# Tikai7/DiTTO-TTS

Hardware: NVIDIA B200
Metric: latent frames/sec per denoising step (higher is better)
Workload: dtype bf16

## Files before the change

ditto_tts_b200/csrc/cross_fused.cu:

```cuda
#include <algorithm>
#include <cstdlib>

#include "common.cuh"
#include "kernels.cuh"

namespace ditto {
namespace {

constexpr int XF_THREADS = 640;
constexpr int XF_EPI_WARP0 = 4;
constexpr int XF_EPI_WARPS = 16;
constexpr int XF_SM_WARPS = 8;
constexpr int XF_REGS_LAUNCH = 96, XF_REGS_CTRL = 56, XF_REGS_EPI = 104;
static_assert(128 * XF_REGS_CTRL + 32 * XF_EPI_WARPS * XF_REGS_EPI <= XF_THREADS * XF_REGS_LAUNCH, "register re-distribution exceeds the CTA pool");
constexpr int XF_BM = 128;
constexpr int XF_BK = 64;
constexpr int XF_NS = 64;
constexpr int XF_CH = 128;
constexpr int XF_HC = 64;
constexpr int XF_STAGES = 2;
constexpr int XF_A_BYTES = XF_BM * XF_BK * 2;
constexpr int XF_B_BYTES = XF_NS * XF_BK * 2;
constexpr int XF_STAGE_BYTES = XF_A_BYTES + XF_B_BYTES;
constexpr int XF_MAX_H = 768;
constexpr int XF_P_BYTES = XF_BM * XF_NS * 2;
constexpr int XF_VF_BOX = XF_NS * 64 * 2;
constexpr int XF_VF_RING = 3;
constexpr int XF_VF_BYTES = XF_VF_RING * XF_VF_BOX;
constexpr int XF_NB = 4;
constexpr int XF_SLAB_BYTES = XF_BM * 32 * 4;
constexpr int XF_HBUF_BYTES = 2 * XF_SLAB_BYTES;
constexpr int XF_OFF_P = XF_STAGES * XF_STAGE_BYTES;
constexpr int XF_OFF_VF = XF_OFF_P + XF_P_BYTES;
constexpr int XF_OFF_HB = XF_OFF_VF + XF_VF_BYTES;
constexpr int XF_OFF_BAR = XF_OFF_HB + XF_NB * XF_HBUF_BYTES;
constexpr int XF_BAR_BYTES = 512;
constexpr int XF_OFF_STAT = XF_OFF_BAR + XF_BAR_BYTES;
constexpr int XF_STAT_BYTES = 2 * XF_BM * 4 * 8;
constexpr int XF_SMEM_BYTES = XF_OFF_STAT + XF_STAT_BYTES + 1024 ;
static_assert(XF_SMEM_BYTES <= 232448, "exceeds the 227 KiB shared memory of an sm_100 CTA");
static_assert(XF_OFF_P % 1024 == 0 && XF_OFF_VF % 1024 == 0 && XF_OFF_HB % 1024 == 0 && XF_STAGE_BYTES % 1024 == 0,
              "swizzled operands need 1024-B alignment");
constexpr int XF_TMEM_COLS = 512;
constexpr int XF_O_BUFS = 3;
constexpr int XF_S_COL0 = XF_O_BUFS * XF_CH;

struct XfDev {
  int n_seq, T, S, H;
  int rt;
  int m_tiles, num_tiles, num_kb, num_ch, num_hc;
  int pf_dist;
  float alpha2;
  const float* sbias; long long sb_seq;
  const float* out_bias;
  const float* gamma; const float* beta;
  float inv_h;
  const float2* ln_stat; int ln_parts; const float* ln_c;
};

__device__ __forceinline__ void epi_bar_sync() { asm volatile("bar.sync 1, %0;" ::"n"(32 * XF_EPI_WARPS) : "memory"); }
__device__ __forceinline__ void quarter_bar_sync(int quarter) { asm volatile("bar.sync %0, 128;" ::"r"(2 + quarter) : "memory"); }
__device__ __forceinline__ void xf_regs_ctrl() { asm volatile("setmaxnreg.dec.sync.aligned.u32 %0;" ::"n"(XF_REGS_CTRL)); }
__device__ __forceinline__ void xf_regs_epi() { asm volatile("setmaxnreg.inc.sync.aligned.u32 %0;" ::"n"(XF_REGS_EPI)); }
__device__ __forceinline__ void tmem_ld_16x16(uint32_t taddr, uint32_t (&r)[8]) {
  asm volatile("tcgen05.ld.sync.aligned.16x256b.x2.b32 {%0, %1, %2, %3, %4, %5, %6, %7}, [%8];"
               : "=r"(r[0]), "=r"(r[1]), "=r"(r[2]), "=r"(r[3]), "=r"(r[4]), "=r"(r[5]), "=r"(r[6]), "=r"(r[7])
               : "r"(taddr)
               : "memory");
}
__device__ __forceinline__ void tma_store_4d(const CUtensorMap* m, const void* smem, int c0, int c1, int c2, int c3) {
  asm volatile("cp.async.bulk.tensor.4d.global.shared::cta.bulk_group [%0, {%2, %3, %4, %5}], [%1];" ::"l"(reinterpret_cast<uint64_t>(m)),
               "r"(smem_u32(smem)), "r"(c0), "r"(c1), "r"(c2), "r"(c3)
               : "memory");
}
__device__ __forceinline__ void tma_prefetch_4d(const CUtensorMap* m, int c0, int c1, int c2, int c3) {
  asm volatile("cp.async.bulk.prefetch.tensor.4d.L2.global.tile [%0, {%1, %2, %3, %4}];" ::"l"(reinterpret_cast<uint64_t>(m)), "r"(c0),
               "r"(c1), "r"(c2), "r"(c3)
               : "memory");
}
__device__ __forceinline__ void bulk_commit() { asm volatile("cp.async.bulk.commit_group;" ::: "memory"); }
template <int N>
__device__ __forceinline__ void bulk_wait() { asm volatile("cp.async.bulk.wait_group %0;" ::"n"(N) : "memory"); }
template <int N>
__device__ __forceinline__ void bulk_wait_read() { asm volatile("cp.async.bulk.wait_group.read %0;" ::"n"(N) : "memory"); }

__global__ void __launch_bounds__(XF_THREADS, 1)
    cross_fused_kernel(const __grid_constant__ CUtensorMap tmap_u, const __grid_constant__ CUtensorMap tmap_kf,
                       const __grid_constant__ CUtensorMap tmap_vf, const __grid_constant__ CUtensorMap tmap_h,
                       const __grid_constant__ CUtensorMap tmap_uo, const XfDev p) {
  extern __shared__ uint8_t smem_raw[];
  const uint32_t raw_addr = smem_u32(smem_raw);
  uint8_t* smem = smem_raw + ((1024u - (raw_addr & 1023u)) & 1023u);
  uint8_t* p_smem = smem + XF_OFF_P;
  uint8_t* vf_smem = smem + XF_OFF_VF;
  uint8_t* hbuf = smem + XF_OFF_HB;
  uint64_t* full_bar = reinterpret_cast<uint64_t*>(smem + XF_OFF_BAR);
  uint64_t* empty_bar = full_bar + XF_STAGES;
  uint64_t* s_full = empty_bar + XF_STAGES;
  uint64_t* s_empty = s_full + 2;
  uint64_t* p_full = s_empty + 2;
  uint64_t* vf_full = p_full + 1;
  uint64_t* vf_empty = vf_full + XF_VF_RING;
  uint64_t* o_full = vf_empty + XF_VF_RING;
  uint64_t* o_empty = o_full + XF_O_BUFS;
  uint64_t* hin_full = o_empty + XF_O_BUFS;
  uint64_t* hout_full = hin_full + XF_NB;
  uint64_t* hfree = hout_full + XF_NB;
  uint32_t* tmem_ptr = reinterpret_cast<uint32_t*>(hfree + XF_NB);
  float2* stat = reinterpret_cast<float2*>(smem + XF_OFF_STAT);
  static_assert((2 * XF_STAGES + 2 + 2 + 1 + 2 * XF_VF_RING + 2 * XF_O_BUFS + 3 * XF_NB) * 8 + 4 <= XF_BAR_BYTES, "barrier block too small");

  const int warp = warp_id_uniform();
  const int lane = threadIdx.x & 31;

  if (warp == 0 && lane == 0) {
    tma_prefetch_desc(&tmap_u);
    tma_prefetch_desc(&tmap_kf);
    tma_prefetch_desc(&tmap_vf);
    tma_prefetch_desc(&tmap_h);
    tma_prefetch_desc(&tmap_uo);
  }
  if (warp == 1 && lane == 0) {
    for (int s = 0; s < XF_STAGES; ++s) {
      mbar_init(&full_bar[s], 1);
      mbar_init(&empty_bar[s], 1);
    }
    for (int s = 0; s < 2; ++s) {
      mbar_init(&s_full[s], 1);
      mbar_init(&s_empty[s], XF_SM_WARPS);
    }
    mbar_init(p_full, XF_SM_WARPS);
    for (int s = 0; s < XF_VF_RING; ++s) {
      mbar_init(&vf_full[s], 1);
      mbar_init(&vf_empty[s], 1);
    }
    for (int s = 0; s < XF_O_BUFS; ++s) {
      mbar_init(&o_full[s], 1);
      mbar_init(&o_empty[s], XF_EPI_WARPS);
    }
    for (int s = 0; s < XF_NB; ++s) {
      mbar_init(&hin_full[s], 1);
      mbar_init(&hout_full[s], XF_EPI_WARPS);
      mbar_init(&hfree[s], 1);
    }
    fence_barrier_init();
  }
  if (warp == 2) tmem_alloc<XF_TMEM_COLS>(tmem_ptr);
  tcgen05_fence_before();
  __syncthreads();
  tcgen05_fence_after();
  const uint32_t tmem_base = *tmem_ptr;
  const int first = blockIdx.x, step = gridDim.x;

  if (warp == 0) {
    xf_regs_ctrl();
    {
      const bool leader = elect_one();
      int stage = 0;
      uint32_t phase = 0;
      uint32_t vc = 0;
      const uint32_t stage_tx = static_cast<uint32_t>(p.rt) * (XF_BK * 2) + XF_B_BYTES;
      auto load_scores_operands = [&](int tile) {
        const int seq = tile / p.m_tiles, mb = tile - seq * p.m_tiles;
        for (int kb = 0; kb < p.num_kb; ++kb) {
          mbar_wait(&empty_bar[stage], phase ^ 1u);
          if (leader) {
            uint8_t* sa = smem + stage * XF_STAGE_BYTES;
            mbar_expect_tx(&full_bar[stage], stage_tx);
            tma_load_4d(&tmap_u, &full_bar[stage], sa, kb * XF_BK, mb * p.rt, 0, seq);
            tma_load_4d(&tmap_kf, &full_bar[stage], sa + XF_A_BYTES, kb * XF_BK, 0, 0, seq);
          }
          __syncwarp();
          if (++stage == XF_STAGES) { stage = 0; phase ^= 1u; }
        }
      };
      if (first < p.num_tiles) load_scores_operands(first);
      for (int tile = first; tile < p.num_tiles; tile += step) {
        const int seq = tile / p.m_tiles;
        for (int hc = 0; hc < p.num_hc; ++hc, ++vc) {
          const uint32_t vs = vc % XF_VF_RING;
          mbar_wait(&vf_empty[vs], ((vc / XF_VF_RING) & 1u) ^ 1u);
          if (leader) {
            mbar_expect_tx(&vf_full[vs], XF_VF_BOX);
            tma_load_4d(&tmap_vf, &vf_full[vs], vf_smem + vs * XF_VF_BOX, hc * XF_HC, 0, 0, seq);
          }
          __syncwarp();
        }
        if (tile + step < p.num_tiles) load_scores_operands(tile + step);
      }
    }
  } else if (warp == 1) {
    xf_regs_ctrl();
    {
      const bool leader = elect_one();
      constexpr uint32_t idesc_s = umma_idesc_bf16(XF_BM, XF_NS, false, false);
      constexpr uint32_t idesc_o = umma_idesc_bf16(XF_BM, XF_HC, false, true);
      const uint64_t ds0 = umma_smem_desc(smem_u32(smem), 16, 1024);
      const uint64_t dp0 = umma_smem_desc(smem_u32(p_smem), 16, 1024);
      const uint64_t dv0 = umma_smem_desc(smem_u32(vf_smem), XF_VF_BOX, 1024);
      int stage = 0;
      uint32_t phase = 0;
      auto issue_scores = [&](uint32_t j) {
        const uint32_t sb = j & 1u;
        mbar_wait(&s_empty[sb], ((j >> 1) & 1u) ^ 1u);
        tcgen05_fence_after();
        const uint32_t d_tmem = tmem_base + XF_S_COL0 + sb * XF_NS;
        for (int kb = 0; kb < p.num_kb; ++kb) {
          mbar_wait(&full_bar[stage], phase);
          tcgen05_fence_after();
          if (leader) {
            const uint64_t da = ds0 + static_cast<uint64_t>((stage * XF_STAGE_BYTES) >> 4);
#pragma unroll
            for (int k = 0; k < XF_BK / 16; ++k)
              umma_bf16(d_tmem, da + ((k * 32) >> 4), da + ((XF_A_BYTES + k * 32) >> 4), idesc_s, (kb | k) != 0 ? 1u : 0u);
            umma_commit(&empty_bar[stage]);
          }
          __syncwarp();
          if (++stage == XF_STAGES) { stage = 0; phase ^= 1u; }
        }
        if (leader) umma_commit(&s_full[sb]);
        __syncwarp();
      };
      uint32_t it = 0, oc = 0, vc = 0;
      if (first < p.num_tiles) issue_scores(0);
      for (int tile = first; tile < p.num_tiles; tile += step, ++it) {
        mbar_wait(p_full, it & 1u);
        for (int hc = 0; hc < p.num_hc; ++hc, ++vc) {
          const uint32_t ob = oc % XF_O_BUFS, vs = vc % XF_VF_RING;
          mbar_wait(&vf_full[vs], (vc / XF_VF_RING) & 1u);
          if ((hc & 1) == 0) mbar_wait(&o_empty[ob], ((oc / XF_O_BUFS) & 1u) ^ 1u);
          tcgen05_fence_after();
          if (leader) {
            const uint32_t d_tmem = tmem_base + ob * XF_CH + (hc & 1) * XF_HC;
            const uint64_t dv = dv0 + static_cast<uint64_t>((vs * XF_VF_BOX) >> 4);
#pragma unroll
            for (int k = 0; k < XF_NS / 16; ++k)
              umma_bf16(d_tmem, dp0 + ((k * 32) >> 4), dv + ((k * (16 * 128)) >> 4), idesc_o, k != 0 ? 1u : 0u);
            umma_commit(&vf_empty[vs]);
            if (hc & 1) umma_commit(&o_full[ob]);
          }
          __syncwarp();
          if (hc & 1) ++oc;
        }
        if (tile + step < p.num_tiles) issue_scores(it + 1);
      }
    }
  } else if (warp == 2 || warp == 3) {
    xf_regs_ctrl();
    {
      const bool leader = elect_one();
      const int my_tiles = first < p.num_tiles ? (p.num_tiles - 1 - first) / step + 1 : 0;
      const int jobs_per_tile = 2 * p.num_hc;
      const int J = my_tiles * jobs_per_tile;
      auto job_coords = [&](int j, int& seq, int& row, int& pass, int& hc) {
        const int ti = j / jobs_per_tile, r = j - ti * jobs_per_tile;
        const int tile = first + ti * step;
        seq = tile / p.m_tiles;
        row = (tile - seq * p.m_tiles) * p.rt;
        pass = r / p.num_hc;
        hc = r - pass * p.num_hc;
      };
      if (warp == 2) {
        const int P0 = my_tiles * p.num_hc;
        int pf_next = 0;
        auto prefetch_upto = [&](int limit) {
          if (p.pf_dist <= 0) return;
          limit = limit < P0 ? limit : P0;
          for (; pf_next < limit; ++pf_next) {
            const int ti = pf_next / p.num_hc, hc = pf_next - ti * p.num_hc;
            const int tile = first + ti * step, seq = tile / p.m_tiles, row = (tile - seq * p.m_tiles) * p.rt;
            if (leader && pf_next >= XF_NB) {
              tma_prefetch_4d(&tmap_h, hc * XF_HC, row, 0, seq);
              tma_prefetch_4d(&tmap_h, hc * XF_HC + 32, row, 0, seq);
            }
          }
        };
        for (int j = 0; j < J; ++j) {
          int seq, row, pass, hc;
          job_coords(j, seq, row, pass, hc);
          const int b = j % XF_NB;
          const int ti = j / jobs_per_tile;
          prefetch_upto(pass == 0 ? ti * p.num_hc + hc + p.pf_dist + 1 : (ti + 1) * p.num_hc + p.pf_dist + (hc + 1) / 2 + 1);
          mbar_wait(&hfree[b], ((j / XF_NB) & 1u) ^ 1u);
          if (leader) {
            uint8_t* buf = hbuf + b * XF_HBUF_BYTES;
            mbar_expect_tx(&hin_full[b], static_cast<uint32_t>(p.rt) * 256);
            tma_load_4d(&tmap_h, &hin_full[b], buf, hc * XF_HC, row, 0, seq);
            tma_load_4d(&tmap_h, &hin_full[b], buf + XF_SLAB_BYTES, hc * XF_HC + 32, row, 0, seq);
          }
          __syncwarp();
        }
      } else {
        for (int j = 0; j < J; ++j) {
          const int b = j % XF_NB;
          mbar_wait(&hout_full[b], (j / XF_NB) & 1u);
          int seq, row, pass, hc;
          job_coords(j, seq, row, pass, hc);
          if (leader) {
            const uint8_t* buf = hbuf + b * XF_HBUF_BYTES;
            if (pass == 0) {
              tma_store_4d(&tmap_h, buf, hc * XF_HC, row, 0, seq);
              tma_store_4d(&tmap_h, buf + XF_SLAB_BYTES, hc * XF_HC + 32, row, 0, seq);
            } else {
              tma_store_4d(&tmap_uo, buf, hc * XF_HC, row, 0, seq);
            }
            bulk_commit();
            const int jn = j - 1 + XF_NB;
            if (j >= 1 && jn < J) {
              bulk_wait_read<1>();
              if ((jn % jobs_per_tile) >= p.num_hc) {
                if (p.num_hc - XF_NB + 1 > 8) bulk_wait<8>();
                else bulk_wait<1>();
              }
              mbar_arrive(&hfree[(j - 1) % XF_NB]);
            }
          }
          __syncwarp();
        }
        if (leader) bulk_wait<0>();
        __syncwarp();
      }
    }
  } else if (warp >= XF_EPI_WARP0) {
    xf_regs_epi();
    const int ew = warp - XF_EPI_WARP0;
    const int quarter = warp & 3;
    const int sub = ew >> 2;
    const int g = lane >> 2, q = lane & 3, q2 = q * 2;
    const bool writer = q == 0;
    uint32_t it = 0, oc = 0, job = 0;
    for (int tile = first; tile < p.num_tiles; tile += step, ++it) {
      const int seq = tile / p.m_tiles;
      const uint32_t sb = it & 1u;
      if (sub < 2) {
        const int trow = quarter * 32 + sub * 16;
        const float* bias = p.sbias + seq * p.sb_seq;
        float2 bb[8];
#pragma unroll
        for (int kb = 0; kb < 8; ++kb) {
          const int c = kb * 8 + q2;
          bb[kb].x = c < p.S ? __ldg(bias + c) * 1.4426950408889634f : 0.f;
          bb[kb].y = c + 1 < p.S ? __ldg(bias + c + 1) * 1.4426950408889634f : 0.f;
        }
        float aA = p.alpha2, nA = 0.f, aB = p.alpha2, nB = 0.f;
        float2 cc[8];
#pragma unroll
        for (int kb = 0; kb < 8; ++kb) cc[kb] = make_float2(0.f, 0.f);
        if (p.ln_stat != nullptr) {
          const float* lnc = p.ln_c + seq * p.sb_seq;
#pragma unroll
          for (int kb = 0; kb < 8; ++kb) {
            const int c = kb * 8 + q2;
            cc[kb].x = c < p.S ? __ldg(lnc + c) : 0.f;
            cc[kb].y = c + 1 < p.S ? __ldg(lnc + c + 1) : 0.f;
          }
          const int mbt = tile - seq * p.m_tiles;
          const int lrA = mbt * p.rt + trow + g;
#pragma unroll
          for (int half = 0; half < 2; ++half) {
            const int lr = lrA + half * 8;
            float sm = 0.f, sq = 0.f;
            if (lr < p.T) {
              const float2* sp2 = p.ln_stat + (static_cast<long long>(seq) * p.T + lr) * p.ln_parts;
              for (int c = 0; c < p.ln_parts; ++c) {
                const float2 v = __ldg(sp2 + c);
                sm += v.x; sq += v.y;
              }
            }
            const float mean = sm * p.inv_h;
            const float rstd = rsqrtf(fmaxf(fmaf(-mean, mean, sq * p.inv_h), 0.f) + 1e-5f);
            if (half == 0) { aA = rstd * p.alpha2; nA = -mean * aA; }
            else { aB = rstd * p.alpha2; nB = -mean * aB; }
          }
        }
        mbar_wait(&s_full[sb], (it >> 1) & 1u);
        tcgen05_fence_after();
        uint32_t r[32];
        tmem_ld_16x64(tmem_base + (static_cast<uint32_t>(trow) << 16) + XF_S_COL0 + sb * XF_NS, r);
        tmem_ld_wait();
        tcgen05_fence_before();
        __syncwarp();
        if (lane == 0) mbar_arrive(&s_empty[sb]);
        float mA = -INFINITY, mB = -INFINITY;
#pragma unroll
// ... 213 lines not shown
  }
  return 0;
}

}

bool cross_fused_supported(int64_t T, int64_t S, int H, int heads) {
  return heads == 1 && S >= 1 && S <= XF_NS && H % XF_CH == 0 && H >= XF_NB * XF_HC && H <= XF_MAX_H && T >= 1;
}

int launch_cross_fused(const CrossFusedParams& q, cudaStream_t st) {
  DITTO_TRY(tc_gemm_init());
  DITTO_REQUIRE(cross_fused_supported(q.T, q.S, q.H, 1), DITTO_E_UNSUPPORTED, "cross_fused: unsupported shape");
  DITTO_REQUIRE(q.u && q.kfold && q.vfold && q.sbias && q.out_bias && q.h && q.gamma && q.beta && q.u_out, DITTO_E_BADARG,
                "cross_fused: null argument");
  DITTO_REQUIRE(q.n_seq >= 1 && q.Sp >= q.S && q.Sp % 8 == 0, DITTO_E_BADARG, "cross_fused: bad sizes");
  DeviceState* ds = device_state();
  if (ds == nullptr) return DITTO_E_CUDA;
  if (!ds->xf_attr) {
    DITTO_CUDA(cudaFuncSetAttribute(cross_fused_kernel, cudaFuncAttributeMaxDynamicSharedMemorySize, XF_SMEM_BYTES));
    ds->xf_attr = true;
  }
  TcOperand U, Kf, Vf, Uo;
  U.ptr = q.u; U.rows = q.T; U.cols = q.H; U.ld = q.H; U.s_outer = q.T * q.H;
  Kf.ptr = q.kfold; Kf.rows = q.S; Kf.cols = q.H; Kf.ld = q.H; Kf.s_outer = q.kf_seq;
  Vf.ptr = q.vfold; Vf.rows = q.Sp; Vf.cols = q.H; Vf.ld = q.H; Vf.s_outer = q.vf_seq;
  Uo.ptr = q.u_out; Uo.rows = q.T; Uo.cols = q.H; Uo.ld = q.H; Uo.s_outer = q.T * q.H;
  const int sms = tc_num_sms();
  int rt = XF_BM;
  if (g_opt.xf_rows >= 8 && g_opt.xf_rows <= XF_BM && g_opt.xf_rows % 8 == 0) rt = g_opt.xf_rows;
  CUtensorMap mu, mk, mv, mh, mo;
  DITTO_TRY(tc_make_map(&mu, U, 1, q.n_seq, XF_BK, rt));
  DITTO_TRY(tc_make_map(&mk, Kf, 1, q.n_seq, XF_BK, XF_NS));
  DITTO_TRY(tc_make_map(&mv, Vf, 1, q.n_seq, 64, XF_NS));
  DITTO_TRY(tc_make_map(&mo, Uo, 1, q.n_seq, XF_HC, rt));
  DITTO_TRY(make_map_h(&mh, q.h, q.n_seq, q.T, q.H, rt));
  XfDev p;
  p.n_seq = static_cast<int>(q.n_seq); p.T = static_cast<int>(q.T); p.S = static_cast<int>(q.S); p.H = q.H;
  p.rt = rt;
  p.m_tiles = static_cast<int>(ceil_div(q.T, rt));
  const int64_t tiles = static_cast<int64_t>(p.m_tiles) * q.n_seq;
  DITTO_REQUIRE(tiles < (1ll << 31), DITTO_E_UNSUPPORTED, "cross_fused: too many tiles");
  p.num_tiles = static_cast<int>(tiles);
  p.num_kb = q.H / XF_BK;
  p.num_ch = q.H / XF_CH;
  p.num_hc = q.H / XF_HC;
  p.alpha2 = q.alpha * 1.4426950408889634f;
  p.sbias = q.sbias; p.sb_seq = q.sb_seq;
  p.out_bias = q.out_bias;
  p.gamma = q.gamma; p.beta = q.beta;
  p.inv_h = 1.0f / static_cast<float>(q.H);
  p.pf_dist = g_opt.xf_prefetch > 0 ? std::min(g_opt.xf_prefetch, 2 * p.num_hc) : 0;
  p.ln_stat = q.ln_stat; p.ln_parts = q.ln_parts; p.ln_c = q.ln_c;
  if (q.ln_stat != nullptr) DITTO_REQUIRE(q.ln_parts > 0 && q.ln_c != nullptr, DITTO_E_BADARG, "cross_fused: deferred LayerNorm arguments");
  const double rows = static_cast<double>(q.n_seq) * q.T;
  ProfScope prof(q.tag, st, 4.0 * rows * q.S * q.H, rows * q.H * 12.0);
  const int grid = static_cast<int>(std::min<int64_t>(sms, tiles));
  cross_fused_kernel<<<grid, XF_THREADS, XF_SMEM_BYTES, st>>>(mu, mk, mv, mh, mo, p);
  DITTO_LAUNCH_CHECK();
  return 0;
}

}
```

ditto_tts_b200/csrc/elementwise.cu:

```cuda
#include <vector>

#include "kernels.cuh"

namespace ditto {

__global__ void cast_bf16_kernel(const float* __restrict__ x, bf16* __restrict__ y, int64_t n) {
  int64_t i = (static_cast<int64_t>(blockIdx.x) * blockDim.x + threadIdx.x) * 4;
  const int64_t stride = static_cast<int64_t>(gridDim.x) * blockDim.x * 4;
  for (; i + 3 < n; i += stride) {
    float4 v = *reinterpret_cast<const float4*>(x + i);
    uint2 o;
    o.x = pack_bf16x2(v.x, v.y);
    o.y = pack_bf16x2(v.z, v.w);
    *reinterpret_cast<uint2*>(y + i) = o;
  }
  if (i < n) {
    for (int64_t j = i; j < n && j < i + 4; ++j) y[j] = __float2bfloat16_rn(x[j]);
  }
}

int launch_cast_bf16(const float* x, bf16* y, int64_t n, cudaStream_t st) {
  if (n <= 0) return 0;
  DITTO_REQUIRE((reinterpret_cast<uintptr_t>(x) & 15) == 0 && (reinterpret_cast<uintptr_t>(y) & 7) == 0,
                DITTO_E_BADARG, "cast_bf16: misaligned pointer");
// ... 456 lines not shown
  return 0;
}

__global__ void silu_kernel(float* __restrict__ x, int64_t n) {
  for (int64_t i = static_cast<int64_t>(blockIdx.x) * blockDim.x + threadIdx.x; i < n;
       i += static_cast<int64_t>(gridDim.x) * blockDim.x) {
    const float v = x[i];
    x[i] = v / (1.0f + expf(-v));
  }
}
int launch_silu(float* x, int64_t n, cudaStream_t st) {
  silu_kernel<<<static_cast<unsigned>(std::min<int64_t>(ceil_div(n, 256), 148 * 8)), 256, 0, st>>>(x, n);
  DITTO_LAUNCH_CHECK();
  return 0;
}

__global__ void mean_silu_kernel(const float* __restrict__ text, float* __restrict__ out, int S, int D) {
  const int seq = blockIdx.y;
  const int c = blockIdx.x * blockDim.x + threadIdx.x;
  if (c >= D) return;
  const float* p = text + static_cast<int64_t>(seq) * S * D + c;
  float acc = 0.f;
  for (int s = 0; s < S; ++s) acc += p[static_cast<int64_t>(s) * D];
  const float m = acc / static_cast<float>(S);
  out[static_cast<int64_t>(seq) * D + c] = m / (1.0f + expf(-m));
}
int launch_mean_silu(const float* text, float* out, int64_t n, int S, int D, cudaStream_t st) {
  dim3 grid(static_cast<unsigned>(ceil_div(D, 128)), static_cast<unsigned>(n));
  mean_silu_kernel<<<grid, 128, 0, st>>>(text, out, S, D);
  DITTO_LAUNCH_CHECK();
  return 0;
}

__global__ void fold_bias_kernel(const bf16* __restrict__ kv, int64_t ld, const float* __restrict__ bq, float* __restrict__ sb,
                                 int64_t total, int S, int Sp, int heads, int d, float scale) {
  const int lane = threadIdx.x & 31;
  const int64_t o = static_cast<int64_t>(blockIdx.x) * (blockDim.x >> 5) + (threadIdx.x >> 5);
  if (o >= total) return;
  const int s_idx = static_cast<int>(o % Sp);
  const int head = static_cast<int>((o / Sp) % heads);
  const int64_t seq = o / (static_cast<int64_t>(Sp) * heads);
  float acc = 0.f;
  if (s_idx < S) {
    const bf16* row = kv + (seq * S + s_idx) * ld + head * d;
    for (int i = lane; i < d; i += 32) acc += __bfloat162float(row[i]) * bq[head * d + i];
  }
  acc = warp_sum(acc);
  if (lane == 0) sb[o] = s_idx < S ? scale * acc : 0.f;
}
int launch_fold_bias(const bf16* kv, int64_t ld, const float* bq, float* sb, int64_t n, int S, int Sp, int heads, int d, float scale,
                     cudaStream_t st) {
  const int64_t total = n * heads * Sp;
  fold_bias_kernel<<<static_cast<unsigned>(ceil_div(total, 8)), 256, 0, st>>>(kv, ld, bq, sb, total, S, Sp, heads, d, scale);
  DITTO_LAUNCH_CHECK();
  return 0;
}

__global__ void transpose_v_kernel(const bf16* __restrict__ v, int64_t ld, bf16* __restrict__ vt, int T, int Tp, int heads,
                                   int d) {
  __shared__ bf16 tile[32][33];
  const int b = blockIdx.z;
  const int seq = b / heads, head = b % heads;
  const bf16* src = v + (static_cast<int64_t>(seq) * T) * ld + head * d;
  bf16* dst = vt + static_cast<int64_t>(b) * d * Tp;
  const int t0 = blockIdx.x * 32, c0 = blockIdx.y * 32;
  for (int i = threadIdx.y; i < 32; i += blockDim.y) {
    const int tt = t0 + i, c = c0 + threadIdx.x;
    tile[i][threadIdx.x] = (tt < T && c < d) ? src[static_cast<int64_t>(tt) * ld + c] : __float2bfloat16(0.f);
  }
  __syncthreads();
  for (int i = threadIdx.y; i < 32; i += blockDim.y) {
    const int c = c0 + i, tt = t0 + threadIdx.x;
    if (c < d && tt < Tp) dst[static_cast<int64_t>(c) * Tp + tt] = tile[threadIdx.x][i];
  }
}
int launch_transpose_v(const bf16* v, int64_t ld, bf16* vt, int64_t n_seq, int T, int Tp, int heads, int d, cudaStream_t st) {
  dim3 grid(static_cast<unsigned>(ceil_div(Tp, 32)), static_cast<unsigned>(ceil_div(d, 32)), static_cast<unsigned>(n_seq * heads));
  transpose_v_kernel<<<grid, dim3(32, 8), 0, st>>>(v, ld, vt, T, Tp, heads, d);
  DITTO_LAUNCH_CHECK();
  return 0;
}

__device__ __forceinline__ float cfg_combine(float ec, float eu, float w) { return __fmaf_rn(w, __fsub_rn(ec, eu), eu); }
__device__ __forceinline__ float ddpm_update(float x, float e, float z, float c1, float c2, float c3) {
  return __fmaf_rn(c3, z, __fmul_rn(c1, __fmaf_rn(-c2, e, x)));
}

__global__ void __launch_bounds__(256)
    cfg_ddpm_update_kernel(const float4* __restrict__ eps_c, const float4* __restrict__ eps_u, const float4* __restrict__ x,
                           const float4* __restrict__ z, const int64_t* __restrict__ t, const float* __restrict__ coef,
                           int steps, float w, float4* __restrict__ out, int64_t vec_per_seq, int64_t total_vec) {
  for (int64_t i = static_cast<int64_t>(blockIdx.x) * blockDim.x + threadIdx.x; i < total_vec;
       i += static_cast<int64_t>(gridDim.x) * blockDim.x) {
    const int64_t seq = i / vec_per_seq;
    int64_t tt = t[seq];
    tt = tt < 0 ? 0 : (tt >= steps ? steps - 1 : tt);
    const float c1 = coef[tt * 3 + 0], c2 = coef[tt * 3 + 1], c3 = coef[tt * 3 + 2];
    float4 e = eps_c[i];
    if (eps_u != nullptr) {
      const float4 u = eps_u[i];
      e = make_float4(cfg_combine(e.x, u.x, w), cfg_combine(e.y, u.y, w), cfg_combine(e.z, u.z, w), cfg_combine(e.w, u.w, w));
    }
    const float4 xv = x[i];
    const float4 zv = z != nullptr ? z[i] : make_float4(0.f, 0.f, 0.f, 0.f);
    out[i] = make_float4(ddpm_update(xv.x, e.x, zv.x, c1, c2, c3), ddpm_update(xv.y, e.y, zv.y, c1, c2, c3),
                         ddpm_update(xv.z, e.z, zv.z, c1, c2, c3), ddpm_update(xv.w, e.w, zv.w, c1, c2, c3));
// ... 208 lines not shown
__global__ void __launch_bounds__(256)
    cfg_update_known_kernel(const float4* __restrict__ eps_c, const float4* __restrict__ eps_u, const float4* __restrict__ x,
                            const float4* __restrict__ z, unsigned long long* rng, int64_t* t, int64_t n_t,
                            const float* __restrict__ coef, const float* __restrict__ coef_known, int steps, float w,
                            float4* __restrict__ out, float4* __restrict__ hist, const float4* __restrict__ known,
                            const uint8_t* __restrict__ mask, int64_t vec_per_seq, int64_t vec_per_frame, int64_t total_vec,
                            int64_t vec_offset, int advance) {
  unsigned long long seed = 0ull, draw = 0ull;
  if (RNG) {
    seed = rng[0];
    draw = rng[1];
  }
  for (int64_t i = static_cast<int64_t>(blockIdx.x) * blockDim.x + threadIdx.x; i < total_vec;
       i += static_cast<int64_t>(gridDim.x) * blockDim.x) {
    const int64_t seq = i / vec_per_seq;
    if (mask[i / vec_per_frame] != 0) {
      int64_t tt = t[seq];
      tt = tt < 0 ? 0 : (tt >= steps ? steps - 1 : tt);
      const float a = coef_known[tt * 2 + 0], s = coef_known[tt * 2 + 1];
      const float4 pv = known[i];
      const float4 zv = RNG ? philox_normal4(seed, draw, static_cast<unsigned long long>(vec_offset + i)) : z[i];
      out[i] = make_float4(known_value(pv.x, zv.x, a, s), known_value(pv.y, zv.y, a, s), known_value(pv.z, zv.z, a, s),
                           known_value(pv.w, zv.w, a, s));
      continue;
    }
    if (MULTISTEP) {
      const MultistepRow c = multistep_row(coef, t, seq, steps);
      float4 e = eps_c[i];
      if (eps_u != nullptr) {
        const float4 u = eps_u[i];
        e = make_float4(cfg_combine(e.x, u.x, w), cfg_combine(e.y, u.y, w), cfg_combine(e.z, u.z, w), cfg_combine(e.w, u.w, w));
      }
      const float4 xv = x[i];
      float4 zv = RNG ? make_float4(0.f, 0.f, 0.f, 0.f) : z[i];
      const float4 h = multistep_hist(hist, i, c.c4);
      if (RNG) zv = philox_normal4(seed, draw, static_cast<unsigned long long>(vec_offset + i));
      multistep_store(c, xv, e, zv, h, out, hist, i);
    } else {
      int64_t tt = t[seq];
      tt = tt < 0 ? 0 : (tt >= steps ? steps - 1 : tt);
      const float c1 = coef[tt * 3 + 0], c2 = coef[tt * 3 + 1], c3 = coef[tt * 3 + 2];
      float4 e = eps_c[i];
      if (eps_u != nullptr) {
        const float4 u = eps_u[i];
        e = make_float4(cfg_combine(e.x, u.x, w), cfg_combine(e.y, u.y, w), cfg_combine(e.z, u.z, w), cfg_combine(e.w, u.w, w));
      }
      const float4 xv = x[i];
      const float4 zv = RNG ? philox_normal4(seed, draw, static_cast<unsigned long long>(vec_offset + i)) : z[i];
      out[i] = make_float4(ddpm_update(xv.x, e.x, zv.x, c1, c2, c3), ddpm_update(xv.y, e.y, zv.y, c1, c2, c3),
                           ddpm_update(xv.z, e.z, zv.z, c1, c2, c3), ddpm_update(xv.w, e.w, zv.w, c1, c2, c3));
    }
  }
  if (RNG && advance) last_block_advances(rng, t, n_t, draw);
}

static int64_t profiled_known_frames(const uint8_t* mask, int64_t n, cudaStream_t st) {
  cudaStreamCaptureStatus cs = cudaStreamCaptureStatusNone;
  if (!g_prof_enabled || cudaStreamIsCapturing(st, &cs) != cudaSuccess || cs != cudaStreamCaptureStatusNone) return 0;
  std::vector<uint8_t> h(static_cast<size_t>(n));
  if (cudaMemcpyAsync(h.data(), mask, static_cast<size_t>(n), cudaMemcpyDeviceToHost, st) != cudaSuccess ||
      cudaStreamSynchronize(st) != cudaSuccess)
    return 0;
  int64_t k = 0;
  for (uint8_t v : h) k += v != 0;
  return k;
}

int launch_cfg_update_known(const float* eps_c, const float* eps_u, const float* x, const float* z, unsigned long long* rng, int64_t* t,
                            int64_t n_t, const float* coef, const float* coef_known, int steps, float w, float* out, float* hist,
                            const float* known, const uint8_t* mask, int64_t B, int64_t T, int64_t H, int64_t elem_offset, bool advance,
                            cudaStream_t st) {
  DITTO_REQUIRE(H % 4 == 0 && elem_offset % 4 == 0, DITTO_E_UNSUPPORTED, "cfg_update_known: H % 4 and element offset % 4");
  const bool draw = rng != nullptr, ms = hist != nullptr;
  const int64_t vec_per_frame = H / 4, total_vec = B * T * vec_per_frame;
  if (total_vec == 0) return (draw && advance) ? launch_step_advance(rng, t, n_t, st) : 0;
  const int64_t want = ceil_div(total_vec, 256 * 4);
  const unsigned blocks = static_cast<unsigned>(std::min<int64_t>(round_up(want, 148), 148 * 32));
  const int64_t known_vec = profiled_known_frames(mask, B * T, st) * vec_per_frame;
  const double unknown_streams = (ms ? 5 : 3) + (eps_u ? 1 : 0) + (draw ? 0 : 1), known_streams = 2 + (draw ? 0 : 1);
  ProfScope prof(PC_CFG_UPDATE, st, 0.0,
                 16.0 * (static_cast<double>(total_vec - known_vec) * unknown_streams + static_cast<double>(known_vec) * known_streams) +
                     static_cast<double>(B * T));
  const float4 *ec = reinterpret_cast<const float4*>(eps_c), *eu = reinterpret_cast<const float4*>(eps_u);
  const float4 *xv = reinterpret_cast<const float4*>(x), *zv = reinterpret_cast<const float4*>(z);
  const float4* kv = reinterpret_cast<const float4*>(known);
  float4 *o = reinterpret_cast<float4*>(out), *h = reinterpret_cast<float4*>(hist);
  const int64_t vps = T * vec_per_frame, voff = elem_offset / 4;
  const int adv = advance ? 1 : 0;
  if (ms && draw)
    cfg_update_known_kernel<true, true><<<blocks, 256, 0, st>>>(ec, eu, xv, zv, rng, t, n_t, coef, coef_known, steps, w, o, h, kv, mask,
                                                                vps, vec_per_frame, total_vec, voff, adv);
  else if (ms)
    cfg_update_known_kernel<true, false><<<blocks, 256, 0, st>>>(ec, eu, xv, zv, rng, t, n_t, coef, coef_known, steps, w, o, h, kv, mask,
                                                                 vps, vec_per_frame, total_vec, voff, adv);
  else if (draw)
    cfg_update_known_kernel<false, true><<<blocks, 256, 0, st>>>(ec, eu, xv, zv, rng, t, n_t, coef, coef_known, steps, w, o, h, kv, mask,
                                                                 vps, vec_per_frame, total_vec, voff, adv);
  else
    cfg_update_known_kernel<false, false><<<blocks, 256, 0, st>>>(ec, eu, xv, zv, rng, t, n_t, coef, coef_known, steps, w, o, h, kv,
                                                                  mask, vps, vec_per_frame, total_vec, voff, adv);
  DITTO_LAUNCH_CHECK();
  return 0;
}

__global__ void step_advance_kernel(unsigned long long* rng, int64_t* t, int64_t n_t) {
  for (int64_t i = threadIdx.x; i < n_t; i += blockDim.x) t[i] -= 1;
// ... 94 lines not shown
```

ditto_tts_b200/csrc/engine.cu:

```cuda
#include <cmath>
#include <cstdio>
#include <cstdlib>
#include <cstring>
#include <map>
#include <mutex>
#include <vector>

#include "kernels.cuh"

namespace ditto {

static thread_local std::string t_last_error;
std::atomic<long long> g_launches{0};
DebugOptions g_opt;
void set_error(const std::string& msg) { t_last_error = msg; }
int cuda_fail(cudaError_t err, const char* what, const char* file, int line) {
  t_last_error = std::string("CUDA error ") + std::to_string(static_cast<int>(err)) + " (" + cudaGetErrorString(err) + ") at " +
                 what + " [" + file + ":" + std::to_string(line) + "]";
  return DITTO_E_CUDA;
}

bool g_prof_enabled = false;
namespace {
struct ProfRec { int cls; cudaEvent_t a, b; double flops, bytes; };
// ... 13 lines not shown
  if (cudaEventCreate(&r.a) != cudaSuccess || cudaEventCreate(&r.b) != cudaSuccess) return;
  cudaEventRecord(r.a, st);
  g_prof_recs.push_back(r);
  slot = static_cast<int>(g_prof_recs.size()) - 1;
}
ProfScope::~ProfScope() {
  if (slot >= 0) cudaEventRecord(g_prof_recs[slot].b, st);
}

struct Arena {
  char* base;
  size_t off = 0;
  explicit Arena(void* b) : base(static_cast<char*>(b)) {}
  template <typename T>
  T* take(int64_t n) {
    off = (off + 255) & ~static_cast<size_t>(255);
    T* p = base ? reinterpret_cast<T*>(base + off) : nullptr;
    off += static_cast<size_t>(n) * sizeof(T);
    return p;
  }
};

struct LayerPack {
  bf16 *w_qkv = nullptr, *wc_in = nullptr, *wc_o = nullptr, *w_glu = nullptr, *w_fc2 = nullptr;
  bf16* wc_o_p4 = nullptr;
  float *b_qkv = nullptr, *b_glu = nullptr;
  float *c_qkv = nullptr, *c_glu = nullptr, *bq_g = nullptr;
  bf16* wq_g = nullptr;
};

}

using namespace ditto;

struct ditto_engine {
  ditto_config_t cfg;
  int H = 0, L = 0, heads = 0, d = 0, half = 0, Td = 0, Xd = 0, steps = 0, maxT = 0;
  bool bf16_mode = false, fused_rope = false, finalized = false, have_schedule = false;
  bool blocks_only = false;
  int device = -1;
  int rope_pd = 0;
  bool glu_perm16 = false;
  bool pv_perm4 = false;
  bool qkv_perm16 = false;
  bool cross_flash = false;
  bool fc2_ln = false;
  bool flash768 = false;
  bool flash_attn = true;
  bool defer_ln2 = false;
  bool fused_cross = true;
  bool fused_attn = false;
  bool fold_cross = false;
  bool defer_ln = false;
  int pv_transpose = 0;
  bool rope_table_in_epilogue = false;
  std::map<std::string, int64_t> expected;
  std::map<std::string, float*> w;
  std::vector<void*> owned;
  float *time_table = nullptr, *rope_cos = nullptr, *rope_sin = nullptr, *rope_freq = nullptr, *coef = nullptr, *qs_buf = nullptr;
  float* coef_ms = nullptr;
  float* coef_known = nullptr;
  bf16 *w_in16 = nullptr, *w_out16 = nullptr;
  bf16* w_out_p4 = nullptr;
  std::vector<LayerPack> layers;
  static constexpr int kSide = 8;
  cudaStream_t side[kSide] = {};
  cudaEvent_t ev_fork = nullptr, ev_join[kSide] = {};
  int n_side = 0;
  std::recursive_mutex fork_mutex;

  const float* W(const std::string& k) const {
    auto it = w.find(k);
    return it == w.end() ? nullptr : it->second;
  }
  const float* LW(int i, const char* name) const { return W("blocks." + std::to_string(i) + "." + name); }
};

namespace ditto {

static int dev_alloc(ditto_engine* e, void** p, size_t bytes) {
  DITTO_CUDA(cudaMalloc(p, bytes ? bytes : 16));
  e->owned.push_back(*p);
  return 0;
}

static void build_expected(ditto_engine* e) {
  const int64_t H = e->H, Td = e->Td, Xd = e->Xd, St = e->steps;
  auto& m = e->expected;
  if (!e->blocks_only) {
    m["t_embedding.weight"] = St * Td;
    m["time_embed.0.weight"] = Td * Td; m["time_embed.0.bias"] = Td;
    m["time_embed.2.weight"] = Td * Td; m["time_embed.2.bias"] = Td;
    m["ada_ln.time_mlp.1.weight"] = 2 * H * Td; m["ada_ln.time_mlp.1.bias"] = 2 * H;
    m["ada_ln.text_mlp.1.weight"] = 2 * H * Xd; m["ada_ln.text_mlp.1.bias"] = 2 * H;
    m["proj_in.weight"] = H * H; m["proj_in.bias"] = H;
    m["proj_out.weight"] = H * H; m["proj_out.bias"] = H;
  }
  for (int i = 0; i < e->L; ++i) {
    const std::string p = "blocks." + std::to_string(i) + ".";
    for (const char* n : {"norm1", "norm2", "norm3"}) { m[p + n + ".weight"] = H; m[p + n + ".bias"] = H; }
    m[p + "attn.in_proj_weight"] = 3 * H * H; m[p + "attn.in_proj_bias"] = 3 * H;
    m[p + "cross_attn.in_proj_weight"] = 3 * H * H; m[p + "cross_attn.in_proj_bias"] = 3 * H;
    m[p + "cross_attn.out_proj.weight"] = H * H; m[p + "cross_attn.out_proj.bias"] = H;
    m[p + "mlp_fc1.weight"] = 4 * H * H; m[p + "mlp_fc1.bias"] = 4 * H;
    m[p + "gate.weight"] = 4 * H * H; m[p + "gate.bias"] = 4 * H;
    m[p + "mlp_fc2.weight"] = 4 * H * H; m[p + "mlp_fc2.bias"] = H;
  }
  m["rotary.inv_freq"] = e->half;
}

static bool ignorable_key(const std::string& k) {
  if (k.rfind("nac.", 0) == 0) return true;
  if (k == "alphas_cumprod") return true;
  if (k.size() > 9 && k.compare(k.size() - 9, 9, ".inv_freq") == 0 && k != "rotary.inv_freq") return true;
  if (k.find(".attn.out_proj.") != std::string::npos) return true;
  return false;
}

static int sgemm_nt(const float* A, int64_t lda, const float* Wt, int64_t ldw, float* C, int64_t ldc, const float* bias,
                    const float* resid, int64_t ldr, float alpha, int M, int N, int K, cudaStream_t st) {
  SgemmParams p;
  p.A = A; p.lda = lda; p.B = Wt; p.ldb = ldw; p.C = C; p.ldc = ldc; p.bias = bias; p.resid = resid; p.ldr = ldr;
  p.alpha = alpha; p.M = M; p.N = N; p.K = K; p.b_is_nk = true;
  return launch_sgemm(p, st);
}

static int tc_nt(const bf16* A, int64_t lda, const bf16* Wt, int64_t ldw, void* out, bool out_bf16, int64_t ldo,
                 const float* bias, const float* resid, int64_t ldr, int64_t resid_row_mod, bf16* out2, int64_t ldo2,
                 int M, int N, int K, cudaStream_t st, int tag = PC_TC_OTHER, float2* stat_out = nullptr, int stat_parts = 0) {
  TcGemmParams p;
  p.tag = tag;
  p.stat_out = stat_out; p.stat_parts = stat_parts;
  p.A.ptr = A; p.A.rows = M; p.A.cols = K; p.A.ld = lda;
  p.B.ptr = Wt; p.B.rows = N; p.B.cols = K; p.B.ld = ldw;
  p.M = M; p.N = N; p.K = K;
  p.bias = bias; p.out = out; p.out_bf16 = out_bf16; p.ldo = ldo;
  p.resid = resid; p.ldr = ldr; p.resid_row_mod = resid_row_mod; p.out2 = out2; p.ldo2 = ldo2;
  return launch_tc_gemm(p, st);
}

struct CtxLayout {
  float* text_mod = nullptr;
  void* kv0 = nullptr;
  size_t kv_stride = 0;
  bf16 *kfold0 = nullptr, *vfold0 = nullptr;
  float *sbias0 = nullptr, *cvec0 = nullptr;
  size_t kfold_stride = 0, vfold_stride = 0, sbias_stride = 0;
  size_t total = 0;
};
static bool fold_active(const ditto_engine* e, int64_t S) {
  return e->bf16_mode && e->fold_cross && e->heads * round_up(S, 8) * 2 <= e->H;
}
static bool fold_ln_active(const ditto_engine* e, int64_t S) {
  const bool want = e->defer_ln || (e->defer_ln2 && cross_fused_supported(1, S, e->H, e->heads));
  return want && fold_active(e, S) && tc_scores_softmax_csize(static_cast<int>(S)) == 1;
}
static bool cross_flash_active(const ditto_engine* e, int64_t S) {
  return e->cross_flash && e->fused_cross && e->heads == 1 && S <= 256 && fold_active(e, S) && !cross_fused_supported(1, S, e->H, e->heads);
}
static CtxLayout ctx_layout(const ditto_engine* e, void* base, int64_t n, int64_t S) {
  Arena a(base);
  CtxLayout c;
  c.text_mod = a.take<float>(n * 2 * e->H);
  const int64_t kv_elems = n * S * 2 * e->H;
  a.take<char>(0);
  const size_t kv_bytes = ((static_cast<size_t>(kv_elems) * (e->bf16_mode ? 2 : 4)) + 255) & ~static_cast<size_t>(255);
  c.kv0 = a.take<char>(static_cast<int64_t>(kv_bytes) * e->L);
  c.kv_stride = kv_bytes;
  if (fold_active(e, S)) {
    const int64_t Sp = round_up(S, 8);
    c.kfold_stride = static_cast<size_t>(n * e->heads * S * e->H);
    c.vfold_stride = static_cast<size_t>(n * e->heads * Sp * e->H);
    c.sbias_stride = static_cast<size_t>(n * e->heads * Sp);
    c.kfold0 = a.take<bf16>(static_cast<int64_t>(c.kfold_stride) * e->L);
    c.vfold0 = a.take<bf16>(static_cast<int64_t>(c.vfold_stride) * e->L);
    c.sbias0 = a.take<float>(static_cast<int64_t>(c.sbias_stride) * e->L);
    if (e->defer_ln || e->defer_ln2) c.cvec0 = a.take<float>(static_cast<int64_t>(c.sbias_stride) * e->L);
  }
  c.total = a.off + 256;
  return c;
}

struct SeqGroup {
  int64_t n = 0, n_x = 0, T = 0, S = 0;
  const void* ctx = nullptr;
  int64_t row0 = 0;
  int64_t xrow0 = 0;
  int64_t seq0 = 0;
  int64_t p_off = 0;
  int64_t l_off = 0;
  int64_t vt_off = 0;
};

struct Workspace {
  float *h = nullptr, *xskip = nullptr, *scores = nullptr;
  void *u = nullptr, *qkv = nullptr, *P = nullptr, *qc = nullptr, *oc = nullptr, *hid = nullptr, *xb16 = nullptr;
  float *fc1 = nullptr, *gate = nullptr;
  bf16* vt = nullptr;
  float* lpart = nullptr;
  float2* lnstat = nullptr;
  int ln_parts_h = 0, ln_parts_attn = 0;
  float* tmp_small = nullptr;
  bf16* text16 = nullptr;
  int* row_pos = nullptr;
  int64_t M = 0;
  size_t total = 0;
};
static Workspace ws_layout(const ditto_engine* e, void* base, SeqGroup* gs, int ng) {
  Arena a(base);
  Workspace w;
  const int64_t H = e->H;
  const int es = e->bf16_mode ? 2 : 4;
  int64_t M = 0, Mx = 0, seqs = 0, p_el = 0, l_el = 0, vt_el = 0, n_tot = 0, text_el = 0;
  for (int i = 0; i < ng; ++i) {
    SeqGroup& g = gs[i];
    const int64_t ldp = std::max(round_up(g.T, 8), round_up(g.S, 8));
    g.row0 = M; g.xrow0 = Mx; g.seq0 = seqs; g.p_off = p_el; g.l_off = l_el; g.vt_off = vt_el;
    M += g.n * g.T; Mx += g.n_x * g.T; seqs += g.n;
    p_el += round_up(g.n * e->heads * g.T * ldp, 128);
    l_el += round_up(g.n * e->heads * g.T * ceil_div(ldp, 256), 64);
    vt_el += round_up(g.n * e->heads * e->d * ldp, 128);
    n_tot = std::max(n_tot, g.n);
    text_el = std::max(text_el, g.n * g.S);
  }
  w.M = M;
  w.h = a.take<float>(M * H);
  w.xskip = a.take<float>(M * H);
  w.u = a.take<char>(M * H * es);
  w.xb16 = a.take<char>(M * H * 2);
  w.qkv = a.take<char>(M * 3 * H * es);
// ... 193 lines not shown
  if (block_only) {
  } else if (b16) {
    const int Mp = static_cast<int>(ragged ? M : g0.n_x * g0.T);
    DITTO_TRY(tc_nt(static_cast<bf16*>(w.xb16), H, e->w_in16, H, w.xskip, false, H, e->W("proj_in.bias"), nullptr, 0, 0, nullptr, 0, Mp, H,
                    H, st, PC_TC_PROJ_IN));
  } else {
    for (int gi = 0; gi < ng; ++gi)
      DITTO_TRY(sgemm_nt(x + gs[gi].xrow0 * H, H, e->W("proj_in.weight"), H, w.xskip + gs[gi].xrow0 * H, H, e->W("proj_in.bias"), nullptr, 0,
                         1.f, static_cast<int>(gs[gi].n_x * gs[gi].T), H, H, st));
  }

  const bool fuse_cross_any = b16 && e->fused_cross && !dln;
  auto fuse_cross_group = [&](const SeqGroup& g) {
    return fuse_cross_any && fold_active(e, g.S) && cross_fused_supported(g.T, g.S, H, e->heads);
  };
  for (int i = l_begin; i < l_end; ++i) {
    const LayerPack& lp = e->layers[i];
    const bool last = (i == l_end - 1);
    if (b16) {
      bf16* u = static_cast<bf16*>(w.u);
      bf16* qkv = static_cast<bf16*>(w.qkv);
      if (do_self) {
        TcGemmParams g;
        g.A.ptr = u; g.A.rows = M; g.A.cols = H; g.A.ld = H;
        g.B.ptr = lp.w_qkv; g.B.rows = 3 * H; g.B.cols = H; g.B.ld = H;
        g.M = static_cast<int>(M); g.N = 3 * H; g.K = H; g.bias = lp.b_qkv; g.out = qkv; g.out_bf16 = true; g.ldo = 3 * H;
        g.tag = PC_TC_QKV;
        if (e->fused_rope) {
          g.epilogue = TC_EPI_QKV_ROPE; g.rope_cos = e->rope_cos; g.rope_sin = e->rope_sin; g.rope_half = e->half;
          g.rope_freq = e->rope_table_in_epilogue ? nullptr : e->rope_freq;
          g.rope_pd = e->rope_pd; g.seq_T = static_cast<int>(g0.T); g.hidden = H;
          g.rope_pos = ragged ? w.row_pos : nullptr;
          g.rope_perm16 = e->qkv_perm16;
        }
        if (dln) { g.ln_stat = w.lnstat; g.ln_parts = ln1_parts; g.ln_width = H; g.ln_c = lp.c_qkv; }
        DITTO_TRY(launch_tc_gemm(g, st));
        if (!e->fused_rope)
          for (int gi = 0; gi < ng; ++gi)
            DITTO_TRY(launch_rope(qkv + gs[gi].row0 * 3 * H, true, 3 * H, e->rope_cos, e->rope_sin, gs[gi].n * gs[gi].T,
                                  static_cast<int>(gs[gi].T), H, d, st));
      }
      DITTO_TRY(fork.begin(ng));
      for (int gi = 0; gi < ng; ++gi) {
        const SeqGroup& grp = gs[gi];
        const Workspace wg = group_view(e, w, grp);
        const CtxLayout c = ctx_layout(e, const_cast<void*>(grp.ctx), grp.n, grp.S);
        const int64_t n = grp.n, T = grp.T, S = grp.S, Mg = n * T;
        cudaStream_t st = fork.stream(gi);
        bf16* q = qkv + grp.row0 * 3 * H;
        bf16* ug = u + grp.row0 * H;
        float* hg = w.h + grp.row0 * H;
        const bool dln2 = dln ? dln2_all : fold_ln_active(e, S) && do_self;
        float2* lnstat_g = w.lnstat ? w.lnstat + grp.row0 * std::max(w.ln_parts_h, w.ln_parts_attn) : nullptr;
        if (!do_self) {
        } else if (e->flash768 && !dln2 && flash768_supported(H, e->heads, static_cast<int>(T))) {
          Flash768Params f;
          f.qkv = q; f.ld = 3 * H; f.n_seq = n; f.T = static_cast<int>(T); f.H = H; f.alpha = inv_sqrt_d; f.h = hg;
          f.gamma = e->LW(i, "norm2.weight"); f.beta = e->LW(i, "norm2.bias"); f.u_out = ug; f.tag = PC_FLASH768;
          DITTO_TRY(launch_flash768(f, st));
        } else {
          DITTO_TRY(attention_bf16(e, wg, q, 3 * H, T * 3 * H, q + H, 3 * H, T * 3 * H, q + 2 * H, 3 * H, T * 3 * H, n, static_cast<int>(T),
                                   static_cast<int>(T), inv_sqrt_d, hg, false, H, T * H, hg, st, false, dln2 ? ug : nullptr,
                                   dln2 ? lnstat_g : nullptr));
          if (!dln2) DITTO_TRY(launch_layernorm(hg, e->LW(i, "norm2.weight"), e->LW(i, "norm2.bias"), ug, true, Mg, H, st));
        }
        if (!do_cross) continue;
        void* kv = static_cast<char*>(c.kv0) + c.kv_stride * i;
        bool norm3_done = false;
        if (fold_active(e, S)) {
          const int heads = e->heads;
          const int64_t Sp = round_up(S, 8);
          if (!dln && cross_flash_active(e, S)) {
            Flash768Params f;
            f.qkv = ug; f.ld = H; f.n_seq = n; f.T = static_cast<int>(T); f.H = H; f.alpha = sqrt_inv_d; f.h = hg;
            f.kfold = c.kfold0 + c.kfold_stride * i; f.kf_seq = S * H; f.vfold = c.vfold0 + c.vfold_stride * i; f.vf_seq = Sp * H;
            f.vf_rows = static_cast<int>(Sp); f.Tk = static_cast<int>(S); f.kbias = c.sbias0 + c.sbias_stride * i; f.kb_seq = Sp;
            f.out_bias = e->LW(i, "cross_attn.out_proj.bias");
            f.gamma = e->LW(i, "norm3.weight"); f.beta = e->LW(i, "norm3.bias"); f.u_out = ug; f.tag = PC_CROSS_FLASH;
            DITTO_TRY(launch_flash768_quad(f, st));
            continue;
          }
          if (fuse_cross_group(grp)) {
            CrossFusedParams f;
            f.u = ug; f.kfold = c.kfold0 + c.kfold_stride * i; f.kf_seq = S * H; f.vfold = c.vfold0 + c.vfold_stride * i; f.vf_seq = Sp * H;
            f.sbias = c.sbias0 + c.sbias_stride * i; f.sb_seq = Sp; f.out_bias = e->LW(i, "cross_attn.out_proj.bias");
            f.h = hg; f.gamma = e->LW(i, "norm3.weight"); f.beta = e->LW(i, "norm3.bias"); f.u_out = ug;
            f.n_seq = n; f.T = T; f.S = S; f.Sp = Sp; f.H = H; f.alpha = sqrt_inv_d; f.tag = PC_TC_CROSS_FUSED;
            if (dln2) { f.ln_stat = lnstat_g; f.ln_parts = w.ln_parts_attn; f.ln_c = c.cvec0 + c.sbias_stride * i; }
            DITTO_TRY(launch_cross_fused(f, st));
            continue;
          }
          if (e->fused_attn && tc_scores_softmax_csize(static_cast<int>(S)) == 1) {
            TcScoresSoftmaxParams f;
            f.Q.ptr = ug; f.Q.rows = T; f.Q.cols = H; f.Q.ld = H; f.Q.s_inner = 0; f.Q.s_outer = T * H;
            f.Km.ptr = c.kfold0 + c.kfold_stride * i; f.Km.rows = S; f.Km.cols = H; f.Km.ld = H; f.Km.s_inner = S * H;
            f.Km.s_outer = static_cast<int64_t>(heads) * S * H;
            f.M = static_cast<int>(T); f.N = static_cast<int>(S); f.K = H; f.batch_inner = heads; f.batch_outer = static_cast<int>(n);
            f.alpha = sqrt_inv_d; f.bias = c.sbias0 + c.sbias_stride * i; f.sb_inner = Sp; f.sb_outer = heads * Sp;
            f.P = static_cast<bf16*>(wg.P); f.ldp = heads * Sp; f.sp_inner = Sp; f.sp_outer = T * heads * Sp; f.npad = static_cast<int>(Sp);
            f.tag = PC_TC_CROSS_SCORES;
            if (dln2) { f.ln_stat = lnstat_g; f.ln_parts = w.ln_parts_attn; f.ln_width = H; f.ln_c = c.cvec0 + c.sbias_stride * i; }
            DITTO_TRY(launch_tc_scores_softmax(f, st));
          } else {
            DITTO_REQUIRE(!dln2, DITTO_E_UNSUPPORTED, "forward: deferred LayerNorm needs the fused scores kernel on the folded cross path");
            TcGemmParams g;
            g.A.ptr = ug; g.A.rows = T; g.A.cols = H; g.A.ld = H; g.A.s_inner = 0; g.A.s_outer = T * H;
            g.B.ptr = c.kfold0 + c.kfold_stride * i; g.B.rows = S; g.B.cols = H; g.B.ld = H; g.B.s_inner = S * H;
            g.B.s_outer = static_cast<int64_t>(heads) * S * H;
            g.M = static_cast<int>(T); g.N = static_cast<int>(S); g.K = H; g.batch_inner = heads; g.batch_outer = static_cast<int>(n);
            g.alpha = sqrt_inv_d; g.bias = c.sbias0 + c.sbias_stride * i; g.sb_inner = Sp; g.sb_outer = heads * Sp;
            g.out = wg.scores; g.out_bf16 = false; g.ldo = heads * Sp; g.so_inner = Sp; g.so_outer = T * heads * Sp;
            g.tag = PC_TC_CROSS_SCORES;
            DITTO_TRY(launch_tc_gemm(g, st));
            DITTO_TRY(launch_softmax(wg.scores, Sp, wg.P, true, Sp, n * T * heads, static_cast<int>(S), st));
          }
          TcGemmParams o;
          o.A.ptr = static_cast<const bf16*>(wg.P); o.A.rows = T; o.A.cols = heads * Sp; o.A.ld = heads * Sp; o.A.s_outer = T * heads * Sp;
          o.B.ptr = c.vfold0 + c.vfold_stride * i; o.B.rows = heads * Sp; o.B.cols = H; o.B.ld = H; o.B.s_outer = heads * Sp * H;
          o.b_kn = true;
          o.M = static_cast<int>(T); o.N = H; o.K = static_cast<int>(heads * Sp); o.batch_inner = 1; o.batch_outer = static_cast<int>(n);
          o.bias = e->LW(i, "cross_attn.out_proj.bias");
          o.out = hg; o.out_bf16 = false; o.ldo = H; o.so_outer = T * H; o.resid = hg; o.ldr = H; o.sr_outer = T * H;
          o.tag = PC_TC_CROSS_PV;
          if (dln) { o.out2 = u; o.ldo2 = H; o.stat_out = w.lnstat; o.stat_parts = w.ln_parts_h; o.stat_rows_outer = T; }
          DITTO_TRY(launch_tc_gemm(o, st));
        } else {
          bf16* qc = static_cast<bf16*>(w.qc) + grp.row0 * H;
          bf16* oc = static_cast<bf16*>(w.oc) + grp.row0 * H;
          DITTO_TRY(tc_nt(ug, H, lp.wc_in, H, qc, true, H, e->LW(i, "cross_attn.in_proj_bias"), nullptr, 0, 0, nullptr, 0, static_cast<int>(Mg),
                          H, H, st, PC_TC_CROSS_Q));
          const bf16* kc = static_cast<const bf16*>(kv);
          DITTO_TRY(attention_bf16(e, wg, qc, H, T * H, kc, 2 * H, S * 2 * H, kc + H, 2 * H, S * 2 * H, n, static_cast<int>(T),
                                   static_cast<int>(S), sqrt_inv_d, oc, true, H, T * H, nullptr, st, true));
          if (e->fc2_ln && !dln) {
            GemmResidLnParams f;
            f.A = oc; f.lda = H; f.W = lp.wc_o_p4; f.ldw = H; f.bias = e->LW(i, "cross_attn.out_proj.bias"); f.h = hg; f.ldh = H;
            f.gamma = e->LW(i, "norm3.weight"); f.beta = e->LW(i, "norm3.bias"); f.u = ug; f.ldu = H;
            f.M = static_cast<int>(Mg); f.N = H; f.K = H; f.tag = PC_TC_CROSS_OUT;
            DITTO_TRY(launch_gemm_resid_ln(f, st));
            norm3_done = true;
          } else {
// ... 146 lines not shown
int32_t ditto_profile_get(int32_t i, int64_t* launches, double* total_ms, double* flops, double* bytes) {
  DITTO_REQUIRE(i >= 0 && i < PC_COUNT && launches && total_ms && flops && bytes, DITTO_E_BADARG, "profile_get: bad argument");
  *launches = g_prof_acc[i].launches; *total_ms = g_prof_acc[i].ms; *flops = g_prof_acc[i].flops; *bytes = g_prof_acc[i].bytes;
  return 0;
}

int32_t ditto_debug_set_counters(uint64_t* counters) {
  tc_gemm_set_debug_counters(reinterpret_cast<unsigned long long*>(counters));
  return 0;
}

int32_t ditto_engine_create(const ditto_config_t* cfg, ditto_engine_t** out) {
  DITTO_REQUIRE(cfg && out, DITTO_E_BADARG, "engine_create: null argument");
  DITTO_REQUIRE(cfg->hidden_dim > 0 && cfg->num_layers > 0 && cfg->num_heads > 0 && cfg->time_dim > 0 && cfg->diffusion_steps > 0,
                DITTO_E_BADARG, "engine_create: non-positive dimension");
  DITTO_REQUIRE(cfg->hidden_dim % cfg->num_heads == 0 && (cfg->hidden_dim / cfg->num_heads) % 2 == 0, DITTO_E_BADARG,
                "engine_create: hidden_dim must split into heads of even size");
  DITTO_REQUIRE(cfg->text_dim == cfg->hidden_dim, DITTO_E_UNSUPPORTED,
                "engine_create: text_dim must equal hidden_dim (nn.MultiheadAttention without kdim, DiT.py:90-91)");
  DITTO_REQUIRE(cfg->hidden_dim % 8 == 0 && cfg->hidden_dim <= 1024 && cfg->time_dim % 4 == 0, DITTO_E_UNSUPPORTED,
                "engine_create: need hidden_dim % 8 == 0, hidden_dim <= 1024, time_dim % 4 == 0");
  DITTO_REQUIRE(cfg->precision == DITTO_PREC_FP32 || cfg->precision == DITTO_PREC_BF16, DITTO_E_BADARG, "engine_create: precision");
  int ndev = 0;
  DITTO_CUDA(cudaGetDeviceCount(&ndev));
  DITTO_REQUIRE(ndev > 0, DITTO_E_CUDA, "engine_create: no CUDA device (there is no CPU fallback)");
  ditto_engine* e = new ditto_engine();
  e->cfg = *cfg;
  e->H = cfg->hidden_dim; e->L = cfg->num_layers; e->heads = cfg->num_heads; e->d = e->H / e->heads; e->half = e->d / 2;
  e->Td = cfg->time_dim; e->Xd = cfg->text_dim; e->steps = cfg->diffusion_steps;
  e->maxT = cfg->max_seq_len > 0 ? cfg->max_seq_len : 4096;
  e->bf16_mode = cfg->precision == DITTO_PREC_BF16;
  e->blocks_only = (cfg->flags & DITTO_F_BLOCKS_ONLY) != 0;
  if (cudaGetDevice(&e->device) != cudaSuccess) e->device = -1;
  if (e->bf16_mode) {
    if (e->bf16_mode && e->d % 8 != 0) {
      delete e;
      set_error("engine_create: bf16 path needs head_dim % 8 == 0 (16-byte TMA rows)");
      return DITTO_E_UNSUPPORTED;
    }
    int rc = tc_gemm_init();
    if (rc != 0) { delete e; return rc; }
    for (int pd : {128, 64, 32})
      if (e->half % pd == 0 && e->H % (2 * pd) == 0) { e->rope_pd = pd; break; }
    e->fused_rope = (cfg->flags & DITTO_F_FUSED_ROPE) && e->rope_pd != 0;
    e->fold_cross = (cfg->flags & DITTO_F_FOLD_CROSS) != 0;
    e->fused_attn = (cfg->flags & DITTO_F_FUSED_ATTN) != 0;
    e->defer_ln = (cfg->flags & DITTO_F_DEFER_LN) != 0 && e->fused_rope && e->fused_attn;
    if (g_opt.no_defer_ln) e->defer_ln = false;
    if (g_opt.no_fused_attn) e->fused_attn = false;
    e->fused_cross = e->fused_attn;
    e->flash_attn = e->fused_attn;
    if (g_opt.no_flash) e->flash_attn = false;
    if (g_opt.no_fused_cross) e->fused_cross = false;
    e->defer_ln2 = !e->defer_ln && e->fused_cross && e->bf16_mode && e->heads == 1 && g_opt.defer_ln2 != 0;
    e->pv_transpose = g_opt.pv_transpose != 0;
    e->rope_table_in_epilogue = g_opt.rope_table != 0;
    e->glu_perm16 = !e->defer_ln && e->H % 32 == 0 && !g_opt.glu_generic;
    const bool pd_ok = e->rope_pd == 128 || (e->rope_pd == 32 && !g_opt.no_rope_fast32);
    e->qkv_perm16 = e->fused_rope && pd_ok && !e->defer_ln && !e->rope_table_in_epilogue && e->H % 256 == 0 && !g_opt.rope_generic;
    e->pv_perm4 = e->qkv_perm16 && !e->pv_transpose && !e->defer_ln2 && e->d % 128 == 0 && !g_opt.no_pv_perm4;
    e->flash768 = e->fused_attn && e->pv_perm4 && !e->defer_ln && flash768_supported(e->H, e->heads, 1) && !g_opt.no_flash768;
    e->fc2_ln = !e->defer_ln && gemm_resid_ln_supported(e->H, 4 * e->H) && !g_opt.no_fc2_ln && gemm_resid_ln_schedulable(e->H);
    e->cross_flash = e->flash768 && e->fc2_ln && e->fold_cross && !e->defer_ln2 && !g_opt.no_cross_flash && flash768_quad_schedulable();
  }
  build_expected(e);
  e->layers.resize(e->L);
  int want_side = ditto_engine::kSide;
  if (g_opt.side_streams >= 0) want_side = std::min(ditto_engine::kSide, g_opt.side_streams);
  if (want_side > 0 && cudaEventCreateWithFlags(&e->ev_fork, cudaEventDisableTiming) == cudaSuccess) {
    for (int k = 0; k < want_side; ++k) {
      if (cudaStreamCreateWithFlags(&e->side[k], cudaStreamNonBlocking) != cudaSuccess ||
          cudaEventCreateWithFlags(&e->ev_join[k], cudaEventDisableTiming) != cudaSuccess)
        break;
      e->n_side = k + 1;
    }
  }
  *out = e;
  return 0;
}

int32_t ditto_engine_destroy(ditto_engine_t* e) {
  if (!e) return 0;
  for (int k = 0; k < ditto_engine::kSide; ++k) {
    if (e->side[k]) cudaStreamDestroy(e->side[k]);
    if (e->ev_join[k]) cudaEventDestroy(e->ev_join[k]);
  }
  if (e->ev_fork) cudaEventDestroy(e->ev_fork);
  for (auto& kv : e->w) cudaFree(kv.second);
  for (void* p : e->owned) cudaFree(p);
  delete e;
  return 0;
}

int32_t ditto_engine_load_weight(ditto_engine_t* e, const char* key, const float* data, int64_t numel, void* stream) {
  DITTO_REQUIRE(e && key && data, DITTO_E_BADARG, "load_weight: null argument");
  const std::string k(key);
  if (ignorable_key(k)) return 0;
  auto it = e->expected.find(k);
  if (it == e->expected.end()) {
    set_error("load_weight: unknown state_dict key '" + k + "'");
    return DITTO_E_BADARG;
  }
  if (it->second != numel) {
    set_error("load_weight: '" + k + "' has " + std::to_string(numel) + " elements, expected " + std::to_string(it->second));
    return DITTO_E_BADARG;
  }
// ... 222 lines not shown

int32_t ditto_text_context(ditto_engine_t* e, const float* text_emb, int64_t n, int64_t S, void* ctx, void* workspace,
                           int64_t workspace_bytes, void* stream) {
  DITTO_REQUIRE(e && text_emb && ctx && workspace, DITTO_E_BADARG, "text_context: null argument");
  DITTO_REQUIRE(e->finalized, DITTO_E_STATE, "text_context: engine not finalized");
  DITTO_REQUIRE(n > 0 && S > 0, DITTO_E_BADARG, "text_context: empty input");
  cudaStream_t st = static_cast<cudaStream_t>(stream);
  const int H = e->H, Xd = e->Xd;
  Workspace w = ws_layout(e, workspace, n, 1, S);
  DITTO_REQUIRE(static_cast<int64_t>(w.total) <= workspace_bytes, DITTO_E_WORKSPACE, "text_context: workspace too small");
  CtxLayout c = ctx_layout(e, ctx, n, S);
  if (!e->blocks_only) {
    DITTO_TRY(launch_mean_silu(text_emb, w.tmp_small, n, static_cast<int>(S), Xd, st));
    DITTO_TRY(sgemm_nt(w.tmp_small, Xd, e->W("ada_ln.text_mlp.1.weight"), Xd, c.text_mod, 2 * H, e->W("ada_ln.text_mlp.1.bias"), nullptr,
                       0, 1.f, static_cast<int>(n), 2 * H, Xd, st));
  }
  if (e->bf16_mode) DITTO_TRY(launch_cast_bf16(text_emb, w.text16, n * S * Xd, st));
  for (int i = 0; i < e->L; ++i) {
    void* kv = static_cast<char*>(c.kv0) + c.kv_stride * i;
    const float* bias = e->LW(i, "cross_attn.in_proj_bias") + H;
    if (e->bf16_mode) {
      DITTO_TRY(tc_nt(w.text16, Xd, e->layers[i].wc_in + static_cast<int64_t>(H) * H, H, kv, true, 2 * H, bias, nullptr, 0, 0, nullptr, 0,
                      static_cast<int>(n * S), 2 * H, Xd, st, PC_TC_TEXT_KV));
      if (fold_active(e, S)) {
        const int d = e->d, heads = e->heads;
        const int64_t Sp = round_up(S, 8);
        const bf16* kvb = static_cast<const bf16*>(kv);
        bf16* kf = c.kfold0 + c.kfold_stride * i;
        bf16* vf = c.vfold0 + c.vfold_stride * i;
        float* sb = c.sbias0 + c.sbias_stride * i;
        DITTO_CUDA(cudaMemsetAsync(vf, 0, c.vfold_stride * sizeof(bf16), st));
        TcGemmParams g;
        g.A.ptr = kvb; g.A.rows = S; g.A.cols = d; g.A.ld = 2 * H; g.A.s_inner = d; g.A.s_outer = S * 2 * H;
        const bool fln = fold_ln_active(e, S);
        g.B.ptr = fln ? e->layers[i].wq_g : e->layers[i].wc_in;
        g.B.rows = d; g.B.cols = H; g.B.ld = H; g.B.s_inner = static_cast<int64_t>(d) * H; g.B.s_outer = 0;
        g.b_kn = true;
        g.M = static_cast<int>(S); g.N = H; g.K = d; g.batch_inner = heads; g.batch_outer = static_cast<int>(n);
        g.out = kf; g.out_bf16 = true; g.ldo = H; g.so_inner = S * H; g.so_outer = static_cast<int64_t>(heads) * S * H;
        g.tag = PC_TC_TEXT_KV;
        DITTO_TRY(launch_tc_gemm(g, st));
        TcGemmParams v;
        v.A.ptr = kvb + H; v.A.rows = S; v.A.cols = d; v.A.ld = 2 * H; v.A.s_inner = d; v.A.s_outer = S * 2 * H;
        v.B.ptr = cross_flash_active(e, S) ? e->layers[i].wc_o_p4 : e->layers[i].wc_o;
        v.B.rows = H; v.B.cols = d; v.B.ld = H; v.B.s_inner = d; v.B.s_outer = 0;
        v.M = static_cast<int>(S); v.N = H; v.K = d; v.batch_inner = heads; v.batch_outer = static_cast<int>(n);
        v.out = vf; v.out_bf16 = true; v.ldo = H; v.so_inner = Sp * H; v.so_outer = static_cast<int64_t>(heads) * Sp * H;
        v.tag = PC_TC_TEXT_KV;
        DITTO_TRY(launch_tc_gemm(v, st));
        DITTO_TRY(launch_fold_bias(kvb, 2 * H, fln ? e->layers[i].bq_g : e->LW(i, "cross_attn.in_proj_bias"), sb, n,
                                   static_cast<int>(S), static_cast<int>(Sp), heads, d, sqrtf(1.0f / static_cast<float>(d)), st));
        if (fln)
          DITTO_TRY(launch_rowsum_bf16(kf, c.cvec0 + c.sbias_stride * i, n * heads, static_cast<int>(S), static_cast<int>(Sp), H, st));
      }
    } else {
      DITTO_TRY(sgemm_nt(text_emb, Xd, e->LW(i, "cross_attn.in_proj_weight") + static_cast<int64_t>(H) * H, H, static_cast<float*>(kv),
                         2 * H, bias, nullptr, 0, 1.f, static_cast<int>(n * S), 2 * H, Xd, st));
    }
  }
  return 0;
}

int32_t ditto_forward(ditto_engine_t* e, const float* x, int64_t n_x, const void* ctx, const int64_t* t, int64_t n_seq, int64_t T,
                      int64_t S, float* out, void* workspace, int64_t workspace_bytes, void* stream) {
  DITTO_REQUIRE(e && x && ctx && t && out && workspace, DITTO_E_BADARG, "forward: null argument");
  DITTO_REQUIRE(e->finalized && !e->blocks_only, DITTO_E_STATE, "forward: engine not finalized (or a blocks-only engine)");
  DITTO_REQUIRE(n_seq > 0 && T > 0 && S > 0 && n_x > 0 && n_seq % n_x == 0, DITTO_E_BADARG, "forward: bad batch sizes");
  DITTO_REQUIRE(T <= e->maxT, DITTO_E_UNSUPPORTED, "forward: T exceeds max_seq_len of the engine");
  return forward_impl(e, x, n_x, ctx, t, n_seq, T, S, out, workspace, workspace_bytes, static_cast<cudaStream_t>(stream));
}

int32_t ditto_cfg_ddpm_update(ditto_engine_t* e, const float* eps_c, const float* eps_u, const float* x, const float* z,
                              const int64_t* t, float guidance_scale, float* x_out, int64_t B, int64_t elems_per_seq, void* stream) {
  DITTO_REQUIRE(e && eps_c && x && t && x_out, DITTO_E_BADARG, "cfg_ddpm_update: null argument");
  DITTO_REQUIRE(e->have_schedule, DITTO_E_STATE, "cfg_ddpm_update: schedule not loaded");
  DITTO_REQUIRE(B >= 0 && elems_per_seq >= 0, DITTO_E_BADARG, "cfg_ddpm_update: negative size");
  return launch_cfg_ddpm_update(eps_c, eps_u, x, z, t, e->coef, e->steps, guidance_scale, x_out, B, elems_per_seq,
                                static_cast<cudaStream_t>(stream));
}

static int launch_update(const ditto_engine* e, const float* eps_c, const float* eps_u, const float* x, const float* z, const int64_t* t,
                         float w, float* x_out, float* hist, int64_t B, int64_t per, cudaStream_t st) {
  if (hist) return launch_cfg_multistep_update(eps_c, eps_u, x, z, t, e->coef_ms, e->steps, w, x_out, hist, B, per, st);
  return launch_cfg_ddpm_update(eps_c, eps_u, x, z, t, e->coef, e->steps, w, x_out, B, per, st);
}
static int launch_update_rng(const ditto_engine* e, const float* eps_c, const float* eps_u, const float* x, uint64_t* rng, int64_t* t,
                             int64_t n_t, float w, float* x_out, float* hist, int64_t B, int64_t per, int64_t elem_offset, bool advance,
                             cudaStream_t st) {
  unsigned long long* r = reinterpret_cast<unsigned long long*>(rng);
  if (hist)
    return launch_cfg_multistep_update_rng(eps_c, eps_u, x, r, t, n_t, e->coef_ms, e->steps, w, x_out, hist, B, per, elem_offset, advance, st);
  return launch_cfg_ddpm_update_rng(eps_c, eps_u, x, r, t, n_t, e->coef, e->steps, w, x_out, B, per, elem_offset, advance, st);
}
static int require_multistep(const ditto_engine* e, const float* hist, const char* what) {
  DITTO_REQUIRE(e && hist, DITTO_E_BADARG, std::string(what) + ": null argument (hist)");
  DITTO_REQUIRE(e->coef_ms, DITTO_E_STATE, std::string(what) + ": no multistep table loaded (ditto_engine_load_multistep_table)");
  return 0;
}

static int32_t p_sample_impl(ditto_engine_t* e, const float* x, const void* ctx, const int64_t* t, const float* z, int32_t guided,
                             float guidance_scale, int64_t B, int64_t T, int64_t S, float* eps_scratch, float* x_out, float* hist,
                             void* workspace, int64_t workspace_bytes, void* stream) {
  DITTO_REQUIRE(e && x && ctx && t && eps_scratch && x_out && workspace, DITTO_E_BADARG, "p_sample: null argument");
  DITTO_REQUIRE(e->finalized && e->have_schedule && !e->blocks_only, DITTO_E_STATE, "p_sample: engine not finalized / schedule not loaded");
  DITTO_REQUIRE(B > 0 && T > 0 && S > 0 && T <= e->maxT, DITTO_E_BADARG, "p_sample: bad sizes");
  const int64_t n = guided ? 2 * B : B;
// ... 327 lines not shown
  return static_cast<int64_t>(a.off + 256);
}

int32_t ditto_adaln(const float* x, const float* time_emb, const float* text_emb, const float* w_time, const float* b_time,
                    const float* w_text, const float* b_text, float* out, int64_t n_seq, int64_t T, int64_t S, int64_t H, int64_t time_dim,
                    int64_t text_dim, void* workspace, int64_t workspace_bytes, void* stream) {
  DITTO_REQUIRE(x && time_emb && text_emb && w_time && b_time && w_text && b_text && out && workspace, DITTO_E_BADARG, "adaln: null argument");
  DITTO_REQUIRE(n_seq > 0 && T > 0 && S > 0 && H > 0 && H % 4 == 0 && H <= 1024 && time_dim % 4 == 0 && text_dim > 0, DITTO_E_UNSUPPORTED,
                "adaln: need H % 4 == 0, H <= 1024, time_dim % 4 == 0");
  DITTO_REQUIRE(ditto_adaln_workspace_bytes(n_seq, H, time_dim, text_dim) <= workspace_bytes, DITTO_E_WORKSPACE, "adaln: workspace too small");
  cudaStream_t st = static_cast<cudaStream_t>(stream);
  Arena a(workspace);
  float* ts = a.take<float>(n_seq * time_dim);
  float* tm = a.take<float>(n_seq * 2 * H);
  float* pooled = a.take<float>(n_seq * text_dim);
  float* xm = a.take<float>(n_seq * 2 * H);
  DITTO_CUDA(cudaMemcpyAsync(ts, time_emb, sizeof(float) * n_seq * time_dim, cudaMemcpyDeviceToDevice, st));
  DITTO_TRY(launch_silu(ts, n_seq * time_dim, st));
  DITTO_TRY(sgemm_nt(ts, time_dim, w_time, time_dim, tm, 2 * H, b_time, nullptr, 0, 1.f, static_cast<int>(n_seq), static_cast<int>(2 * H),
                     static_cast<int>(time_dim), st));
  DITTO_TRY(launch_mean_silu(text_emb, pooled, n_seq, static_cast<int>(S), static_cast<int>(text_dim), st));
  DITTO_TRY(sgemm_nt(pooled, text_dim, w_text, text_dim, xm, 2 * H, b_text, nullptr, 0, 1.f, static_cast<int>(n_seq), static_cast<int>(2 * H),
                     static_cast<int>(text_dim), st));
  return launch_adaln_ln(x, n_seq, tm, xm, nullptr, static_cast<int>(n_seq), nullptr, nullptr, out, nullptr, false, nullptr, n_seq,
                         static_cast<int>(T), static_cast<int>(H), st);
}

int32_t ditto_rope(const float* t, const float* pos, float* out, int64_t batch, int64_t T, int64_t heads, int64_t head_dim, void* stream) {
  DITTO_REQUIRE(t && pos && out, DITTO_E_BADARG, "rope: null argument");
  DITTO_REQUIRE(batch >= 0 && T > 0 && heads > 0 && head_dim > 0 && head_dim % 2 == 0, DITTO_E_BADARG, "rope: bad sizes (head_dim must be even)");
  return launch_rope_angles(t, pos, out, batch, static_cast<int>(T), static_cast<int>(heads), static_cast<int>(head_dim),
                            static_cast<cudaStream_t>(stream));
}

int32_t ditto_attn_self768(const void* qkv, int64_t ld, int64_t n_seq, int64_t T, float alpha, float* h, const float* gamma,
                           const float* beta, void* u_out, int32_t flags, void* stream) {
  DITTO_REQUIRE(qkv && h && n_seq > 0 && T > 0 && T < (1ll << 30), DITTO_E_BADARG, "attn_self768: bad argument");
  Flash768Params f;
  f.qkv = static_cast<const bf16*>(qkv); f.ld = ld; f.n_seq = n_seq; f.T = static_cast<int>(T); f.H = 768; f.alpha = alpha; f.h = h;
  f.gamma = gamma; f.beta = beta; f.u_out = static_cast<bf16*>(u_out); f.force_rescale = (flags & 1) != 0; f.dbg = flags >> 8; f.tag = PC_FLASH768;
  return launch_flash768(f, static_cast<cudaStream_t>(stream));
}

int32_t ditto_debug_option(const char* name, int32_t value) {
  DITTO_REQUIRE(name != nullptr, DITTO_E_BADARG, "debug_option: null name");
  struct Opt { const char* n; int* p; };
  const Opt opts[] = {
      {"no_pair", &g_opt.no_pair}, {"cluster_m", &g_opt.cluster_m}, {"cluster_n", &g_opt.cluster_n}, {"generic_epi", &g_opt.generic_epi},
      {"stages_1cta", &g_opt.stages_1cta}, {"stages_pair", &g_opt.stages_pair}, {"no_mcast", &g_opt.no_mcast}, {"xf_rows", &g_opt.xf_rows}, {"xf_prefetch", &g_opt.xf_prefetch},
      {"no_defer_ln", &g_opt.no_defer_ln}, {"no_fused_attn", &g_opt.no_fused_attn}, {"no_flash", &g_opt.no_flash},
      {"no_flash768", &g_opt.no_flash768}, {"no_fused_cross", &g_opt.no_fused_cross}, {"defer_ln2", &g_opt.defer_ln2},
      {"pv_transpose", &g_opt.pv_transpose}, {"rope_table", &g_opt.rope_table}, {"rope_generic", &g_opt.rope_generic},
      {"glu_generic", &g_opt.glu_generic}, {"no_rope_fast32", &g_opt.no_rope_fast32}, {"no_pv_perm4", &g_opt.no_pv_perm4},
      {"side_streams", &g_opt.side_streams}, {"no_fused_ln", &g_opt.no_fused_ln}, {"flash768_quad", &g_opt.flash768_quad},
      {"no_fc2_ln", &g_opt.no_fc2_ln}, {"no_cross_flash", &g_opt.no_cross_flash}, {"dbg_nostore", &g_opt.dbg_nostore}};
  if (strcmp(name, "reset") == 0) { g_opt = DebugOptions(); return 0; }
  for (const Opt& o : opts)
    if (strcmp(name, o.n) == 0) { *o.p = value; return 0; }
  set_error(std::string("debug_option: unknown option '") + name + "'");
  return DITTO_E_BADARG;
}

int32_t ditto_layernorm(const float* x, const float* gamma, const float* beta, void* y, int32_t out_bf16, int64_t rows, int64_t H,
                        void* stream) {
  DITTO_REQUIRE(x && y && rows >= 0 && H > 0, DITTO_E_BADARG, "layernorm: bad argument");
  return launch_layernorm(x, gamma, beta, y, out_bf16 != 0, rows, static_cast<int>(H), static_cast<cudaStream_t>(stream));
}

int32_t ditto_gemm_f32(const float* A, int64_t lda, int64_t strideA, const float* B, int64_t ldb, int64_t strideB, int32_t b_is_nk,
                       float* C, int64_t ldc, int64_t strideC, const float* bias, const float* resid, float alpha, int64_t M, int64_t N,
                       int64_t K, int64_t batch, void* stream) {
  DITTO_REQUIRE(A && B && C && batch >= 1, DITTO_E_BADARG, "gemm_f32: bad argument");
  SgemmParams p;
  p.A = A; p.lda = lda; p.sA_outer = strideA; p.B = B; p.ldb = ldb; p.sB_outer = strideB; p.b_is_nk = b_is_nk != 0;
  p.C = C; p.ldc = ldc; p.sC_outer = strideC; p.bias = bias; p.resid = resid; p.ldr = ldc; p.sR_outer = strideC; p.alpha = alpha;
  p.M = static_cast<int>(M); p.N = static_cast<int>(N); p.K = static_cast<int>(K); p.batch_outer = static_cast<int>(batch);
  return launch_sgemm(p, static_cast<cudaStream_t>(stream));
}

int32_t ditto_gemm_resid_ln_weight_row(int32_t packed_row) { return packed_row >= 0 ? gemm_resid_ln_weight_row(packed_row) : -1; }
int32_t ditto_gemm_resid_ln(const void* A, int64_t lda, const void* W, int64_t ldw, const float* bias, float* h, int64_t ldh,
                            const float* gamma, const float* beta, void* u, int64_t ldu, int64_t M, int64_t N, int64_t K, void* stream) {
  DITTO_REQUIRE(A && W && bias && h && M > 0 && M < (1ll << 31) && N > 0 && K > 0 && N < (1 << 20) && K < (1 << 24), DITTO_E_BADARG,
                "gemm_resid_ln: bad argument");
  GemmResidLnParams f;
  f.A = static_cast<const bf16*>(A); f.lda = lda; f.W = static_cast<const bf16*>(W); f.ldw = ldw; f.bias = bias;
  f.h = h; f.ldh = ldh; f.gamma = gamma; f.beta = beta; f.u = static_cast<bf16*>(u); f.ldu = ldu;
  f.M = static_cast<int>(M); f.N = static_cast<int>(N); f.K = static_cast<int>(K);
  return launch_gemm_resid_ln(f, static_cast<cudaStream_t>(stream));
}

int32_t ditto_gemm_bf16(const void* A, int64_t lda, const void* W, int64_t ldw, void* C, int64_t ldc, int32_t out_bf16,
                        const float* bias, const float* resid, int64_t ldr, float alpha, int64_t M, int64_t N, int64_t K, void* stream) {
  DITTO_REQUIRE(A && W && C, DITTO_E_BADARG, "gemm_bf16: null argument");
  TcGemmParams p;
  p.A.ptr = static_cast<const bf16*>(A); p.A.rows = M; p.A.cols = K; p.A.ld = lda;
  p.B.ptr = static_cast<const bf16*>(W); p.B.rows = N; p.B.cols = K; p.B.ld = ldw;
  p.M = static_cast<int>(M); p.N = static_cast<int>(N); p.K = static_cast<int>(K);
  p.alpha = alpha; p.bias = bias; p.out = C; p.out_bf16 = out_bf16 != 0; p.ldo = ldc; p.resid = resid; p.ldr = ldr;
  return launch_tc_gemm(p, static_cast<cudaStream_t>(stream));
}

int32_t ditto_cast_bf16(const float* x, void* y, int64_t n, void* stream) {
  DITTO_REQUIRE(x && y && n >= 0, DITTO_E_BADARG, "cast_bf16: bad argument");
  return launch_cast_bf16(x, static_cast<bf16*>(y), n, static_cast<cudaStream_t>(stream));
}

// ... 3 lines not shown
```

ditto_tts_b200/csrc/flash_attn768.cu:

```cuda
#include <algorithm>

#include "common.cuh"
#include "kernels.cuh"

namespace ditto {
namespace {

constexpr int F7_THREADS = 384;
constexpr int F7_EPI_WARP0 = 4;
constexpr int F7_EPI_WARPS = 8;
constexpr int F7_BM = 128, F7_BN = 128, F7_BK = 64;
constexpr int F7_D = 768;
constexpr int F7_DH = F7_D / 2;
constexpr int F7_KCH = F7_D / F7_BK;
constexpr int F7_VKEYS = 32;
constexpr int F7_VST = F7_BN / F7_VKEYS;
constexpr int F7_VBOX = F7_VKEYS * 128;
constexpr int F7_STAGES = 4;
constexpr int F7_STAGE_BYTES = 32768;
constexpr int F7_QK_BYTES = F7_BM * F7_BK * 2;
constexpr int F7_V_BYTES = (F7_DH / 64) * F7_VBOX;
constexpr int F7_P_BYTES = F7_BM * F7_BN * 2;
constexpr int F7_OFF_POWN = F7_STAGES * F7_STAGE_BYTES;
constexpr int F7_OFF_PLAND = F7_OFF_POWN + F7_P_BYTES;
constexpr int F7_OFF_BAR = F7_OFF_PLAND + F7_P_BYTES;
constexpr int F7_BAR_BYTES = 256;
constexpr int F7_OFF_XCH = F7_OFF_BAR + F7_BAR_BYTES;
constexpr int F7_XCH_HDR = 0, F7_XCH_L = 2 * F7_BM * 4, F7_XCH_STAT = 4 * F7_BM * 4;
constexpr int F7_XCH_BYTES = 4 * F7_BM * 4 + 2 * F7_BM * 8;
constexpr int F7_SMEM_BYTES = F7_OFF_XCH + F7_XCH_BYTES + 1024;
static_assert(F7_SMEM_BYTES <= 232448, "exceeds the 227 KiB shared memory of an sm_100 CTA");
static_assert(F7_V_BYTES <= F7_STAGE_BYTES && 2 * F7_QK_BYTES == F7_STAGE_BYTES, "ring slot too small");
static_assert(F7_KCH % F7_STAGES == 0 && F7_VST == F7_STAGES, "every tile must start at ring slot 0");
constexpr int F7_TMEM_COLS = 512;
constexpr int F7_S_COL = F7_DH;
constexpr float F7_TAU = 8.0f;

#ifndef DITTO_F7_TRACE
#define DITTO_F7_TRACE 0
#endif
constexpr int F7_TR_MAX = 512;
constexpr int F7_TR_ROLES = 3;
struct F7Tr {
  unsigned long long* b; int n; long long t0;
  __device__ __forceinline__ void init(unsigned long long* buf, int rank, int role, bool on, long long t_sync) {
    b = (DITTO_F7_TRACE && buf != nullptr && on) ? buf + (rank * F7_TR_ROLES + role) * F7_TR_MAX : nullptr; n = 0; t0 = t_sync;
  }
  __device__ __forceinline__ void ev(int kind, int j) {
    if (DITTO_F7_TRACE && b != nullptr && n < F7_TR_MAX)
      b[n++] = (static_cast<unsigned long long>(kind * 256 + (j & 255)) << 40) | (static_cast<unsigned long long>(clock64() - t0) & 0xFFFFFFFFFFull);
  }
  __device__ __forceinline__ void val(int kind, int j, long long v) {
    if (DITTO_F7_TRACE && b != nullptr && n < F7_TR_MAX)
      b[n++] = (static_cast<unsigned long long>(kind * 256 + (j & 255)) << 40) | (static_cast<unsigned long long>(v) & 0xFFFFFFFFFFull);
  }
};

struct F7Dev {
  unsigned long long* trace;
  int n_seq, T;
  int m_tiles, k_tiles, num_items;
  float alpha2;
  float* h;
  const float* gamma; const float* beta;
  bf16* u_out;
  int force_rescale;
  int dbg;
};

__device__ __forceinline__ void tmem_st_16x64(uint32_t taddr, const uint32_t (&r)[32]) {
  asm volatile(
      "tcgen05.st.sync.aligned.16x256b.x8.b32 [%0], "
      "{%1, %2, %3, %4, %5, %6, %7, %8, %9, %10, %11, %12, %13, %14, %15, %16, "
      "%17, %18, %19, %20, %21, %22, %23, %24, %25, %26, %27, %28, %29, %30, %31, %32};"
      ::"r"(taddr), "r"(r[0]), "r"(r[1]), "r"(r[2]), "r"(r[3]), "r"(r[4]), "r"(r[5]), "r"(r[6]), "r"(r[7]), "r"(r[8]), "r"(r[9]),
        "r"(r[10]), "r"(r[11]), "r"(r[12]), "r"(r[13]), "r"(r[14]), "r"(r[15]), "r"(r[16]), "r"(r[17]), "r"(r[18]), "r"(r[19]),
        "r"(r[20]), "r"(r[21]), "r"(r[22]), "r"(r[23]), "r"(r[24]), "r"(r[25]), "r"(r[26]), "r"(r[27]), "r"(r[28]), "r"(r[29]),
        "r"(r[30]), "r"(r[31])
      : "memory");
}
__device__ __forceinline__ void tmem_st_wait() { asm volatile("tcgen05.wait::st.sync.aligned;" ::: "memory"); }
__device__ __forceinline__ uint32_t f7_ctarank() {
  uint32_t r;
  asm volatile("mov.u32 %0, %%cluster_ctarank;" : "=r"(r));
  return r;
}
__device__ __forceinline__ void f7_cluster_sync() {
  asm volatile("barrier.cluster.arrive.release.aligned;\n\tbarrier.cluster.wait.acquire.aligned;" ::: "memory");
}
__device__ __forceinline__ uint32_t f7_mapa(uint32_t addr, uint32_t rank) {
  uint32_t r;
  asm volatile("mapa.shared::cluster.u32 %0, %1, %2;" : "=r"(r) : "r"(addr), "r"(rank));
  return r;
}
__device__ __forceinline__ void f7_st_async(uint32_t remote_addr, float v, uint32_t remote_bar) {
  asm volatile("st.async.weak.shared::cluster.mbarrier::complete_tx::bytes.b32 [%0], %1, [%2];" ::"r"(remote_addr),
               "r"(__float_as_uint(v)), "r"(remote_bar)
               : "memory");
}
__device__ __forceinline__ void f7_bulk_copy_to_peer(uint32_t remote_dst, uint32_t local_src, uint32_t bytes, uint32_t remote_bar) {
  asm volatile("cp.async.bulk.shared::cluster.shared::cta.mbarrier::complete_tx::bytes [%0], [%1], %2, [%3];" ::"r"(remote_dst),
               "r"(local_src), "r"(bytes), "r"(remote_bar)
               : "memory");
}
__device__ __forceinline__ void f7_commit_mc(uint64_t* bar, uint16_t mask) {
  asm volatile("tcgen05.commit.cta_group::1.mbarrier::arrive::one.shared::cluster.multicast::cluster.b64 [%0], %1;" ::"r"(smem_u32(bar)),
               "h"(mask)
               : "memory");
}
__device__ __forceinline__ void f7_prefetch_l2(const void* p) { asm volatile("prefetch.global.L2 [%0];" ::"l"(p)); }

__global__ void __cluster_dims__(2, 1, 1) __launch_bounds__(F7_THREADS, 1)
    flash_attn768_kernel(const __grid_constant__ CUtensorMap tmap_q, const __grid_constant__ CUtensorMap tmap_k,
                         const __grid_constant__ CUtensorMap tmap_v, const F7Dev p) {
  extern __shared__ uint8_t smem_raw[];
  const uint32_t raw_addr = smem_u32(smem_raw);
  uint8_t* smem = smem_raw + ((1024u - (raw_addr & 1023u)) & 1023u);
  uint8_t* p_own = smem + F7_OFF_POWN;
// ... 386 lines not shown
#pragma unroll
        for (int jj = 0; jj < 4; ++jj) {
          f[jj] = (okA && !(p.dbg & 2)) ? *reinterpret_cast<const float4*>(hA + cb * 64 + jj * 16) : make_float4(0.f, 0.f, 0.f, 0.f);
          f[4 + jj] = (okB && !(p.dbg & 2)) ? *reinterpret_cast<const float4*>(hB + cb * 64 + jj * 16) : make_float4(0.f, 0.f, 0.f, 0.f);
        }
      };
      load_res(0, f0);
      load_res(1, f1);
      mbar_wait(&l_bar[par], (it >> 1) & 1u);
      tr.ev(15, it);
      lA += l_x[par * F7_BM + rA];
      lB += l_x[par * F7_BM + rB];
      const float iA = 1.0f / lA, iB = 1.0f / lB;
      mbar_wait(o_full, it & 1u);
      tcgen05_fence_after();
      tr.ev(16, it);
      float smA = 0.f, sqA = 0.f, smB = 0.f, sqB = 0.f;
      auto sweep1 = [&](int cb, const float4(&f)[8]) {
        uint32_t o[32];
        tmem_ld_16x64(t_lane + cb * 64, o);
        tmem_ld_wait();
#pragma unroll
        for (int jj = 0; jj < 4; ++jj) {
          const int k0 = 2 * jj, k1 = 2 * jj + 1;
          float4 vA, vB;
          vA.x = fmaf(iA, __uint_as_float(o[4 * k0]), f[jj].x);
          vA.y = fmaf(iA, __uint_as_float(o[4 * k0 + 1]), f[jj].y);
          vA.z = fmaf(iA, __uint_as_float(o[4 * k1]), f[jj].z);
          vA.w = fmaf(iA, __uint_as_float(o[4 * k1 + 1]), f[jj].w);
          vB.x = fmaf(iB, __uint_as_float(o[4 * k0 + 2]), f[4 + jj].x);
          vB.y = fmaf(iB, __uint_as_float(o[4 * k0 + 3]), f[4 + jj].y);
          vB.z = fmaf(iB, __uint_as_float(o[4 * k1 + 2]), f[4 + jj].z);
          vB.w = fmaf(iB, __uint_as_float(o[4 * k1 + 3]), f[4 + jj].w);
          if (okA && !(p.dbg & 4)) *reinterpret_cast<float4*>(hA + cb * 64 + jj * 16) = vA;
          if (okB && !(p.dbg & 4)) *reinterpret_cast<float4*>(hB + cb * 64 + jj * 16) = vB;
          smA += (vA.x + vA.y) + (vA.z + vA.w);
          sqA = fmaf(vA.x, vA.x, fmaf(vA.y, vA.y, fmaf(vA.z, vA.z, fmaf(vA.w, vA.w, sqA))));
          smB += (vB.x + vB.y) + (vB.z + vB.w);
          sqB = fmaf(vB.x, vB.x, fmaf(vB.y, vB.y, fmaf(vB.z, vB.z, fmaf(vB.w, vB.w, sqB))));
          o[4 * k0] = __float_as_uint(vA.x); o[4 * k0 + 1] = __float_as_uint(vA.y);
          o[4 * k1] = __float_as_uint(vA.z); o[4 * k1 + 1] = __float_as_uint(vA.w);
          o[4 * k0 + 2] = __float_as_uint(vB.x); o[4 * k0 + 3] = __float_as_uint(vB.y);
          o[4 * k1 + 2] = __float_as_uint(vB.z); o[4 * k1 + 3] = __float_as_uint(vB.w);
        }
        if (p.u_out != nullptr) tmem_st_16x64(t_lane + cb * 64, o);
      };
#pragma unroll 1
      for (int cb = 0; cb < F7_DH / 64; cb += 2) {
        sweep1(cb, f0);
        if (cb + 2 < F7_DH / 64) load_res(cb + 2, f0);
        sweep1(cb + 1, f1);
        if (cb + 3 < F7_DH / 64) load_res(cb + 3, f1);
      }
      tr.ev(17, it);
      if (p.u_out != nullptr) {
        tmem_st_wait();
        smA = quad_sum(smA); sqA = quad_sum(sqA); smB = quad_sum(smB); sqB = quad_sum(sqB);
        if (ew == 0 && lane == 0) mbar_expect_tx(&stat_bar[par], F7_BM * 8);
        if (writer) {
          const uint32_t slot = f7_mapa(smem_u32(stat_x + (par * F7_BM + rA) * 2), peer);
          const uint32_t bar = f7_mapa(smem_u32(&stat_bar[par]), peer);
          f7_st_async(slot, smA, bar);
          f7_st_async(slot + 4, sqA, bar);
          f7_st_async(slot + 8 * 8, smB, bar);
          f7_st_async(slot + 8 * 8 + 4, sqB, bar);
        }
        mbar_wait(&stat_bar[par], (it >> 1) & 1u);
        tr.ev(18, it);
        const float2 xA = *reinterpret_cast<const float2*>(stat_x + (par * F7_BM + rA) * 2);
        const float2 xB = *reinterpret_cast<const float2*>(stat_x + (par * F7_BM + rB) * 2);
        const float inv_h = 1.0f / static_cast<float>(F7_D);
        const float meanA = (smA + xA.x) * inv_h, meanB = (smB + xB.x) * inv_h;
        const float rsA = rsqrtf(fmaxf(fmaf(-meanA, meanA, (sqA + xA.y) * inv_h), 0.f) + 1e-5f);
        const float rsB = rsqrtf(fmaxf(fmaf(-meanB, meanB, (sqB + xB.y) * inv_h), 0.f) + 1e-5f);
        bf16* uA = p.u_out + growA * F7_D + col_half + q * 4;
        bf16* uB = uA + 8 * F7_D;
        const float* gp = p.gamma + col_half + q * 4;
        const float* bp = p.beta + col_half + q * 4;
#pragma unroll 1
        for (int cb = 0; cb < F7_DH / 64; ++cb) {
          uint32_t o[32];
          tmem_ld_16x64(t_lane + cb * 64, o);
          float4 gm[4], bt[4];
#pragma unroll
          for (int jj = 0; jj < 4; ++jj) {
            gm[jj] = __ldg(reinterpret_cast<const float4*>(gp + cb * 64 + jj * 16));
            bt[jj] = __ldg(reinterpret_cast<const float4*>(bp + cb * 64 + jj * 16));
          }
          tmem_ld_wait();
#pragma unroll
          for (int jj = 0; jj < 4; ++jj) {
            const int k0 = 2 * jj, k1 = 2 * jj + 1;
            uint2 wA, wB;
            wA.x = pack_bf16x2(fmaf((__uint_as_float(o[4 * k0]) - meanA) * rsA, gm[jj].x, bt[jj].x),
                               fmaf((__uint_as_float(o[4 * k0 + 1]) - meanA) * rsA, gm[jj].y, bt[jj].y));
            wA.y = pack_bf16x2(fmaf((__uint_as_float(o[4 * k1]) - meanA) * rsA, gm[jj].z, bt[jj].z),
                               fmaf((__uint_as_float(o[4 * k1 + 1]) - meanA) * rsA, gm[jj].w, bt[jj].w));
            wB.x = pack_bf16x2(fmaf((__uint_as_float(o[4 * k0 + 2]) - meanB) * rsB, gm[jj].x, bt[jj].x),
                               fmaf((__uint_as_float(o[4 * k0 + 3]) - meanB) * rsB, gm[jj].y, bt[jj].y));
            wB.y = pack_bf16x2(fmaf((__uint_as_float(o[4 * k1 + 2]) - meanB) * rsB, gm[jj].z, bt[jj].z),
                               fmaf((__uint_as_float(o[4 * k1 + 3]) - meanB) * rsB, gm[jj].w, bt[jj].w));
            if (okA && !(p.dbg & 8)) *reinterpret_cast<uint2*>(uA + cb * 64 + jj * 16) = wA;
            if (okB && !(p.dbg & 8)) *reinterpret_cast<uint2*>(uB + cb * 64 + jj * 16) = wB;
          }
        }
      }
      tcgen05_fence_before();
      __syncwarp();
      if (lane == 0) mbar_arrive(o_empty);
      tr.ev(19, it);
    }
  } else {
    regs_shrink_ctrl();
  }

  __syncwarp();
  tcgen05_fence_before();
  __syncthreads();
  f7_cluster_sync();
  if (warp == 2) {
    tcgen05_fence_after();
    tmem_dealloc<F7_TMEM_COLS>(tmem_base);
  }
}

}

bool flash768_supported(int H, int heads, int T) { return heads == 1 && H == F7_D && T >= 1; }

int launch_flash768(const Flash768Params& q, cudaStream_t st) {
  if (g_opt.flash768_quad != 1 && q.T >= 1 && (g_opt.flash768_quad == 2 || flash768_quad_preferred(q.T)) && flash768_quad_schedulable())
    return launch_flash768_quad(q, st);
  DITTO_TRY(tc_gemm_init());
  DITTO_REQUIRE(flash768_supported(q.H, 1, q.T), DITTO_E_UNSUPPORTED, "flash768: single head of 768 only");
  DITTO_REQUIRE(q.qkv && q.h && q.n_seq >= 1 && q.ld % 8 == 0 && q.ld >= 3 * F7_D, DITTO_E_BADARG, "flash768: bad argument");
  DITTO_REQUIRE(q.u_out == nullptr || (q.gamma && q.beta), DITTO_E_BADARG, "flash768: LayerNorm output needs gamma and beta");
  DITTO_REQUIRE((reinterpret_cast<uintptr_t>(q.h) & 15) == 0 && (reinterpret_cast<uintptr_t>(q.u_out) & 7) == 0, DITTO_E_BADARG,
                "flash768: h must be 16-byte, u 8-byte aligned");
  DeviceState* ds = device_state();
  if (ds == nullptr) return DITTO_E_CUDA;
  DITTO_REQUIRE(ds->num_sms >= 2, DITTO_E_UNSUPPORTED, "flash768: needs an SM pair");
  if (!ds->f768_attr) {
    DITTO_CUDA(cudaFuncSetAttribute(flash_attn768_kernel, cudaFuncAttributeMaxDynamicSharedMemorySize, F7_SMEM_BYTES));
    ds->f768_attr = true;
  }
  TcOperand Q, K, V;
  Q.ptr = q.qkv; Q.rows = q.T; Q.cols = F7_D; Q.ld = q.ld; Q.s_outer = static_cast<int64_t>(q.T) * q.ld;
  K = Q; K.ptr = q.qkv + F7_D;
  V = Q; V.ptr = q.qkv + 2 * F7_D;
  CUtensorMap mq, mk, mv;
  DITTO_TRY(tc_make_map(&mq, Q, 1, q.n_seq, F7_BK, F7_BM));
  DITTO_TRY(tc_make_map(&mk, K, 1, q.n_seq, F7_BK, F7_BN));
  DITTO_TRY(tc_make_map(&mv, V, 1, q.n_seq, 64, F7_VKEYS));
  F7Dev p;
  p.n_seq = static_cast<int>(q.n_seq); p.T = q.T;
  p.m_tiles = static_cast<int>(ceil_div(q.T, F7_BM));
  p.k_tiles = static_cast<int>(ceil_div(q.T, F7_BN));
  const int64_t items = static_cast<int64_t>(p.m_tiles) * q.n_seq;
  DITTO_REQUIRE(items < (1ll << 31), DITTO_E_UNSUPPORTED, "flash768: too many work items");
  p.num_items = static_cast<int>(items);
  p.alpha2 = q.alpha * 1.4426950408889634f;
  p.h = q.h; p.gamma = q.gamma; p.beta = q.beta; p.u_out = q.u_out;
  p.force_rescale = q.force_rescale ? 1 : 0;
  p.dbg = q.dbg;
  p.trace = DITTO_F7_TRACE ? tc_gemm_debug_counters() : nullptr;
  const double rows = static_cast<double>(q.n_seq) * q.T;
  ProfScope prof(q.tag, st, 4.0 * q.T * static_cast<double>(q.T) * F7_D * q.n_seq, rows * F7_D * (6.0 + 8.0 + (q.u_out ? 2.0 : 0.0)));
  const int clusters = static_cast<int>(std::min<int64_t>(ds->num_sms / 2, items));
  flash_attn768_kernel<<<2 * clusters, F7_THREADS, F7_SMEM_BYTES, st>>>(mq, mk, mv, p);
  DITTO_LAUNCH_CHECK();
  return 0;
}

}
```

ditto_tts_b200/csrc/flash_attn768q.cu:

```cuda
#include <algorithm>
#include <mutex>

#include "common.cuh"
#include "kernels.cuh"

namespace ditto {
namespace {

constexpr int Q7_THREADS = 384;
constexpr int Q7_EPI_WARP0 = 4;
constexpr int Q7_EPI_WARPS = 8;
constexpr int Q7_BM = 128, Q7_BN = 128, Q7_BK = 64;
constexpr int Q7_D = 768;
constexpr int Q7_DH = Q7_D / 2;
constexpr int Q7_KCH = Q7_D / Q7_BK;
constexpr int Q7_VKEYS = 64;
constexpr int Q7_VST = Q7_BN / Q7_VKEYS;
constexpr int Q7_VBOX = Q7_VKEYS * 128;
constexpr int Q7_STAGES = 6;
constexpr int Q7_Q_BYTES = Q7_BM * Q7_BK * 2;
constexpr int Q7_K_BYTES = (Q7_BN / 2) * Q7_BK * 2;
constexpr int Q7_V_BYTES = 3 * Q7_VBOX;
constexpr int Q7_STAGE_BYTES = 24576;
static_assert(Q7_Q_BYTES + Q7_K_BYTES == Q7_STAGE_BYTES && Q7_V_BYTES == Q7_STAGE_BYTES, "both stage kinds fill a ring slot");
constexpr int Q7_P_BYTES = Q7_BM * Q7_BN * 2;
constexpr int Q7_OFF_POWN = Q7_STAGES * Q7_STAGE_BYTES;
constexpr int Q7_OFF_PLAND = Q7_OFF_POWN + Q7_P_BYTES;
constexpr int Q7_OFF_BAR = Q7_OFF_PLAND + Q7_P_BYTES;
constexpr int Q7_BAR_BYTES = 512;
constexpr int Q7_OFF_XCH = Q7_OFF_BAR + Q7_BAR_BYTES;
constexpr int Q7_XCH_HDR = 0, Q7_XCH_L = 2 * Q7_BM * 4, Q7_XCH_STAT = 4 * Q7_BM * 4;
constexpr int Q7_XCH_BYTES = 4 * Q7_BM * 4 + 2 * Q7_BM * 8;
constexpr int Q7_SMEM_BYTES = Q7_OFF_XCH + Q7_XCH_BYTES + 1024;
static_assert(Q7_SMEM_BYTES <= 232448, "exceeds the 227 KiB shared memory of an sm_100 CTA");
static_assert(Q7_OFF_POWN % 1024 == 0, "operand buffers must be 1024-byte aligned (128-B swizzle atoms)");
constexpr int Q7_TMEM_COLS = 512;
constexpr int Q7_S_COL = Q7_DH;
constexpr float Q7_TAU = 8.0f;

#ifndef DITTO_F7_TRACE
#define DITTO_F7_TRACE 0
#endif
constexpr int Q7_TR_MAX = 512, Q7_TR_ROLES = 3;
struct Q7Tr {
  unsigned long long* b; int n; long long t0;
  __device__ __forceinline__ void init(unsigned long long* buf, int rank, int role, bool on, long long t_sync) {
    b = (DITTO_F7_TRACE && buf != nullptr && on) ? buf + (rank * Q7_TR_ROLES + role) * Q7_TR_MAX : nullptr; n = 0; t0 = t_sync;
  }
  __device__ __forceinline__ void ev(int kind, int j) {
    if (DITTO_F7_TRACE && b != nullptr && n < Q7_TR_MAX)
      b[n++] = (static_cast<unsigned long long>(kind * 256 + (j & 255)) << 40) | (static_cast<unsigned long long>(clock64() - t0) & 0xFFFFFFFFFFull);
  }
  __device__ __forceinline__ void val(int kind, int j, long long v) {
    if (DITTO_F7_TRACE && b != nullptr && n < Q7_TR_MAX)
      b[n++] = (static_cast<unsigned long long>(kind * 256 + (j & 255)) << 40) | (static_cast<unsigned long long>(v) & 0xFFFFFFFFFFull);
  }
};

struct Q7Dev {
  unsigned long long* trace;
  int n_seq, T;
  int Tk;
  int m_tiles, k_tiles, num_items;
  const float* kbias; long long kb_seq;
  const float* obias;
  float alpha2;
  float* h;
  const float* gamma; const float* beta;
  bf16* u_out;
  int force_rescale;
  int dbg;
};

__device__ __forceinline__ void q7_tmem_st_16x64(uint32_t taddr, const uint32_t (&r)[32]) {
  asm volatile(
      "tcgen05.st.sync.aligned.16x256b.x8.b32 [%0], "
      "{%1, %2, %3, %4, %5, %6, %7, %8, %9, %10, %11, %12, %13, %14, %15, %16, "
      "%17, %18, %19, %20, %21, %22, %23, %24, %25, %26, %27, %28, %29, %30, %31, %32};"
      ::"r"(taddr), "r"(r[0]), "r"(r[1]), "r"(r[2]), "r"(r[3]), "r"(r[4]), "r"(r[5]), "r"(r[6]), "r"(r[7]), "r"(r[8]), "r"(r[9]),
        "r"(r[10]), "r"(r[11]), "r"(r[12]), "r"(r[13]), "r"(r[14]), "r"(r[15]), "r"(r[16]), "r"(r[17]), "r"(r[18]), "r"(r[19]),
        "r"(r[20]), "r"(r[21]), "r"(r[22]), "r"(r[23]), "r"(r[24]), "r"(r[25]), "r"(r[26]), "r"(r[27]), "r"(r[28]), "r"(r[29]),
        "r"(r[30]), "r"(r[31])
      : "memory");
}
__device__ __forceinline__ void q7_tmem_st_wait() { asm volatile("tcgen05.wait::st.sync.aligned;" ::: "memory"); }
__device__ __forceinline__ uint32_t q7_mapa(uint32_t addr, uint32_t rank) {
  uint32_t r;
  asm volatile("mapa.shared::cluster.u32 %0, %1, %2;" : "=r"(r) : "r"(addr), "r"(rank));
  return r;
}
__device__ __forceinline__ void q7_st_async(uint32_t remote_addr, float v, uint32_t remote_bar) {
  asm volatile("st.async.weak.shared::cluster.mbarrier::complete_tx::bytes.b32 [%0], %1, [%2];" ::"r"(remote_addr),
               "r"(__float_as_uint(v)), "r"(remote_bar)
               : "memory");
}
__device__ __forceinline__ void q7_bulk_copy_to_peer(uint32_t remote_dst, uint32_t local_src, uint32_t bytes, uint32_t remote_bar) {
  asm volatile("cp.async.bulk.shared::cluster.shared::cta.mbarrier::complete_tx::bytes [%0], [%1], %2, [%3];" ::"r"(remote_dst),
               "r"(local_src), "r"(bytes), "r"(remote_bar)
               : "memory");
}
__device__ __forceinline__ void q7_prefetch_l2(const void* p) { asm volatile("prefetch.global.L2 [%0];" ::"l"(p)); }

template <bool CROSS>
__global__ void __launch_bounds__(Q7_THREADS, 1)
    flash_attn768q_kernel(const __grid_constant__ CUtensorMap tmap_q, const __grid_constant__ CUtensorMap tmap_k,
                          const __grid_constant__ CUtensorMap tmap_v, const Q7Dev p) {
  extern __shared__ uint8_t smem_raw[];
  const uint32_t raw_addr = smem_u32(smem_raw);
  uint8_t* smem = smem_raw + ((1024u - (raw_addr & 1023u)) & 1023u);
  uint8_t* p_own = smem + Q7_OFF_POWN;
  uint8_t* p_land = smem + Q7_OFF_PLAND;
  uint64_t* ring_full = reinterpret_cast<uint64_t*>(smem + Q7_OFF_BAR);
  uint64_t* ring_empty = ring_full + Q7_STAGES;
  uint64_t* s_full = ring_empty + Q7_STAGES;
  uint64_t* s_empty = s_full + 1;
  uint64_t* p_full = s_empty + 1;
  uint64_t* p_ready = p_full + 1;
  uint64_t* p_free = p_ready + 1;
  uint64_t* land_full = p_free + 1;
  uint64_t* land_ready = land_full + 1;
  uint64_t* accept = land_ready + 1;
  uint64_t* pv_done = accept + 2;
  uint64_t* o_full = pv_done + 4;
  uint64_t* o_empty = o_full + 1;
  uint64_t* hdr_bar = o_empty + 1;
  uint64_t* l_bar = hdr_bar + 2;
  uint64_t* stat_bar = l_bar + 2;
  uint32_t* tmem_ptr = reinterpret_cast<uint32_t*>(stat_bar + 2);
  static_assert((2 * Q7_STAGES + 21) * 8 + 4 <= Q7_BAR_BYTES, "barrier block too small");
  float* hdr_x = reinterpret_cast<float*>(smem + Q7_OFF_XCH + Q7_XCH_HDR);
  float* l_x = reinterpret_cast<float*>(smem + Q7_OFF_XCH + Q7_XCH_L);
  float* stat_x = reinterpret_cast<float*>(smem + Q7_OFF_XCH + Q7_XCH_STAT);

  const int warp = warp_id_uniform();
  const int lane = threadIdx.x & 31;
  const uint32_t rank = __shfl_sync(0xffffffffu, cluster_ctarank(), 0);
  const int a = static_cast<int>(rank & 1u);
  const int c = static_cast<int>(rank >> 1);
  const uint32_t peer = rank ^ 2u;
  const int num_clusters = gridDim.x >> 2;
  const int first = blockIdx.x >> 2;
  const int KT = p.k_tiles;

  if (warp == 0 && lane == 0) {
    tma_prefetch_desc(&tmap_q);
    tma_prefetch_desc(&tmap_k);
    tma_prefetch_desc(&tmap_v);
  }
  if (warp == 1 && lane == 0) {
    for (int s = 0; s < Q7_STAGES; ++s) { mbar_init(&ring_full[s], 1); mbar_init(&ring_empty[s], 1); }
    mbar_init(s_full, 1);
    mbar_init(s_empty, 2 * Q7_EPI_WARPS);
    mbar_init(p_full, 2 * Q7_EPI_WARPS);
    mbar_init(p_ready, Q7_EPI_WARPS);
    mbar_init(p_free, 2);
    mbar_init(land_full, 1);
    mbar_init(land_ready, 2);
    mbar_init(&accept[0], 2 * Q7_EPI_WARPS);
    mbar_init(&accept[1], 2 * Q7_EPI_WARPS);
    for (int s = 0; s < 4; ++s) mbar_init(&pv_done[s], 1);
    mbar_init(o_full, 1);
    mbar_init(o_empty, 2 * Q7_EPI_WARPS);
    for (int s = 0; s < 2; ++s) { mbar_init(&hdr_bar[s], 1); mbar_init(&l_bar[s], 1); mbar_init(&stat_bar[s], 1); }
    fence_barrier_init();
  }
  if (warp == 2) {
    asm volatile("tcgen05.alloc.cta_group::2.sync.aligned.shared::cta.b32 [%0], %1;" ::"r"(smem_u32(tmem_ptr)), "n"(Q7_TMEM_COLS) : "memory");
    asm volatile("tcgen05.relinquish_alloc_permit.cta_group::2.sync.aligned;" ::: "memory");
  }
  __syncwarp();
  tcgen05_fence_before();
  __syncthreads();
  cluster_sync_all();
  tcgen05_fence_after();
  const uint32_t tmem_base = *tmem_ptr;
  if ((p.dbg >> 8) != 0 && (first & 1)) {
    const long long t_go = clock64() + (static_cast<long long>(p.dbg >> 8) << 11);
    while (clock64() < t_go) {}
  }
  const long long t_sync = DITTO_F7_TRACE ? clock64() : 0;

  if (warp == 0) {
    regs_shrink_ctrl();
    const bool leader = elect_one();
    Q7Tr tr; tr.init(p.trace, rank, 2, first == 0 && leader, t_sync);
    int stage = 0;
    uint32_t phase = 0;
    for (int item = first; item < p.num_items; item += num_clusters) {
      const int qt = item % p.m_tiles, seq = item / p.m_tiles;
      const int q_row0 = qt * (2 * Q7_BM) + a * Q7_BM;
      auto load_s = [&](int j) {
#pragma unroll 1
        for (int ch = 0; ch < Q7_KCH; ++ch) {
          mbar_wait(&ring_empty[stage], phase ^ 1u);
          if (leader) {
            uint8_t* sb = smem + stage * Q7_STAGE_BYTES;
            if (a == 0) mbar_expect_tx(&ring_full[stage], 2 * Q7_STAGE_BYTES);
            tma_load_4d_2sm(&tmap_q, &ring_full[stage], sb, ch * Q7_BK, q_row0, 0, seq);
            tma_load_4d_2sm(&tmap_k, &ring_full[stage], sb + Q7_Q_BYTES, ch * Q7_BK, j * Q7_BN + a * (Q7_BN / 2), 0, seq);
          }
          __syncwarp();
          if (++stage == Q7_STAGES) { stage = 0; phase ^= 1u; }
        }
        tr.ev(30, j);
      };
      auto load_v = [&](int j) {
#pragma unroll 1
        for (int s = 0; s < Q7_VST; ++s) {
          mbar_wait(&ring_empty[stage], phase ^ 1u);
          if (leader) {
            uint8_t* sb = smem + stage * Q7_STAGE_BYTES;
            const int key0 = j * Q7_BN + s * Q7_VKEYS;
            if (a == 0) mbar_expect_tx(&ring_full[stage], 2 * Q7_STAGE_BYTES);
            tma_load_4d_2sm(&tmap_v, &ring_full[stage], sb, c * Q7_DH + a * 128, key0, 0, seq);
            tma_load_4d_2sm(&tmap_v, &ring_full[stage], sb + Q7_VBOX, c * Q7_DH + a * 128 + 64, key0, 0, seq);
            tma_load_4d_2sm(&tmap_v, &ring_full[stage], sb + 2 * Q7_VBOX, c * Q7_DH + 256 + a * 64, key0, 0, seq);
          }
          __syncwarp();
          if (++stage == Q7_STAGES) { stage = 0; phase ^= 1u; }
        }
        tr.ev(31, j);
      };
      if (c < KT) load_s(c);
      for (int j = 0; j < KT; ++j) {
        if ((j & 1) == c && j + 2 < KT) load_s(j + 2);
        load_v(j);
      }
    }
  } else if (warp == 1) {
    regs_shrink_ctrl();
    if (a == 0) {
      const bool leader = elect_one();
      constexpr uint32_t idesc_s = umma_idesc_bf16(2 * Q7_BM, Q7_BN, false, false);
      constexpr uint32_t idesc_o256 = umma_idesc_bf16(2 * Q7_BM, 256, false, true);
      constexpr uint32_t idesc_o128 = umma_idesc_bf16(2 * Q7_BM, 128, false, true);
      const uint64_t dk0 = umma_smem_desc(smem_u32(smem), 16, 1024);
      const uint64_t dv0 = umma_smem_desc(smem_u32(smem), Q7_VBOX, 1024);
      constexpr uint64_t kToPOwn = Q7_OFF_POWN >> 4, kToPLand = Q7_OFF_PLAND >> 4;
      const uint16_t own_mask = static_cast<uint16_t>(3u << (2 * c)), peer_mask = static_cast<uint16_t>(3u << (2 * (c ^ 1)));
      int stage = 0;
      uint32_t phase = 0;
// ... 20 lines not shown
          __syncwarp();
          if (++stage == Q7_STAGES) { stage = 0; phase ^= 1u; }
        }
        if (leader) umma_commit_2sm_mc(s_full, own_mask);
        __syncwarp();
        tr.ev(2, sc);
        tr.val(6, sc, fw);
        ++sc;
      };
      auto issue_pv = [&](int j) {
        const bool own = (j & 1) == c;
        if (own) {
          mbar_wait(p_full, oc & 1u);
        } else {
          mbar_wait(land_ready, rc & 1u);
          mbar_wait(&accept[rc & 1u], (rc >> 1) & 1u);
        }
        if (j == 0) mbar_wait(o_empty, (it & 1u) ^ 1u);
        tcgen05_fence_after();
        tr.ev(3, j);
        long long fw = 0;
        const uint64_t dp = dk0 + (own ? kToPOwn : kToPLand);
#pragma unroll 1
        for (int s = 0; s < Q7_VST; ++s) {
          if (DITTO_F7_TRACE && tr.b) { const long long w0 = clock64(); mbar_wait(&ring_full[stage], phase); fw += clock64() - w0; }
          else mbar_wait(&ring_full[stage], phase);
          tcgen05_fence_after();
          if (leader) {
            const uint64_t so = static_cast<uint64_t>((stage * Q7_STAGE_BYTES) >> 4);
#pragma unroll
            for (int k = 0; k < Q7_VKEYS / 16; ++k) {
              const int key16 = s * (Q7_VKEYS / 16) + k;
              const uint64_t da = dp + (((key16 >> 2) * (Q7_BM * 128) + (key16 & 3) * 32) >> 4);
              const uint32_t acc = (j | s | k) != 0 ? 1u : 0u;
              umma_bf16_2sm(tmem_base, da, dv0 + so + ((k * (16 * 128)) >> 4), idesc_o256, acc);
              umma_bf16_2sm(tmem_base + 256, da, dv0 + so + ((2 * Q7_VBOX + k * (16 * 128)) >> 4), idesc_o128, acc);
            }
            umma_commit_2sm_mc(&ring_empty[stage], own_mask);
          }
          __syncwarp();
          tr.ev(8 + s, j);
          if (++stage == Q7_STAGES) { stage = 0; phase ^= 1u; }
        }
        if (leader) {
          umma_commit_2sm_mc(&pv_done[pvi & 3u], own_mask);
          umma_commit_2sm_mc(p_free, own ? own_mask : peer_mask);
        }
        __syncwarp();
        tr.ev(4, j);
        tr.val(7, j, fw);
        if (own) ++oc; else ++rc;
        ++pvi;
      };
      for (int item = first; item < p.num_items; item += num_clusters, ++it) {
        if (c < KT) issue_s();
        for (int j = 0; j < KT; ++j) {
          if ((j & 1) == c && j + 2 < KT) issue_s();
          issue_pv(j);
        }
        if (leader) umma_commit_2sm_mc(o_full, own_mask);
        __syncwarp();
        tr.ev(5, it);
      }
    }
  } else if (warp == 2) {
    regs_shrink_ctrl();
    const bool leader = elect_one();
    const uint32_t dst = q7_mapa(smem_u32(p_land), peer), src = smem_u32(p_own), bar = q7_mapa(smem_u32(land_full), peer);
    uint32_t oc = 0;
    for (int item = first; item < p.num_items; item += num_clusters)
      for (int j = c; j < KT; j += 2, ++oc) {
        mbar_wait(p_ready, oc & 1u);
        if (leader) q7_bulk_copy_to_peer(dst, src, Q7_P_BYTES, bar);
        __syncwarp();
      }
  } else if (warp == 3) {
    regs_shrink_ctrl();
    uint32_t rc = 0;
    for (int item = first; item < p.num_items; item += num_clusters)
      for (int j = c ^ 1; j < KT; j += 2, ++rc) {
        if (lane == 0) {
          mbar_expect_tx(land_full, Q7_P_BYTES);
          mbar_wait(land_full, rc & 1u);
          mbar_arrive_leader(land_ready);
        }
        __syncwarp();
      }
  } else {
    regs_grow_epi();
    const int ew = warp - Q7_EPI_WARP0;
    const int quarter = warp & 3, hsel = ew >> 2;
    const int g = lane >> 2, q = lane & 3, q2 = q * 2;
    const int trow = quarter * 32 + hsel * 16;
    const int rA = trow + g, rB = rA + 8;
    const uint32_t t_lane = tmem_base + (static_cast<uint32_t>(trow) << 16);
    const bool writer = q == 0;
    const int col_half = c * Q7_DH;
    uint32_t it = 0, sc = 0, oc = 0, rc = 0, pvc = 0;
    Q7Tr tr; tr.init(p.trace, rank, 1, first == 0 && ew == 0 && lane == 0, t_sync);
    auto rescale_o = [&](float fA, float fB) {
      tr.ev(25, static_cast<int>(pvc));
      mbar_wait(&pv_done[(pvc - 1) & 3u], ((pvc - 1) >> 2) & 1u);
      tcgen05_fence_after();
#pragma unroll 1
      for (int cb = 0; cb < Q7_DH / 64; ++cb) {
        uint32_t o[32];
        tmem_ld_16x64(t_lane + cb * 64, o);
        tmem_ld_wait();
#pragma unroll
        for (int kb = 0; kb < 8; ++kb) {
          o[4 * kb] = __float_as_uint(__uint_as_float(o[4 * kb]) * fA);
          o[4 * kb + 1] = __float_as_uint(__uint_as_float(o[4 * kb + 1]) * fA);
          o[4 * kb + 2] = __float_as_uint(__uint_as_float(o[4 * kb + 2]) * fB);
          o[4 * kb + 3] = __float_as_uint(__uint_as_float(o[4 * kb + 3]) * fB);
        }
        q7_tmem_st_16x64(t_lane + cb * 64, o);
      }
      q7_tmem_st_wait();
      tcgen05_fence_before();
    };
    for (int item = first; item < p.num_items; item += num_clusters, ++it) {
      const int qt = item % p.m_tiles, seq = item / p.m_tiles;
      const int row0 = qt * (2 * Q7_BM) + a * Q7_BM;
      const int lrowA = row0 + rA;
      const bool okA = lrowA < p.T, okB = lrowA + 8 < p.T;
      const long long growA = static_cast<long long>(seq) * p.T + lrowA;
      float* hA = p.h + growA * Q7_D + col_half + q * 4;
      float* hB = hA + 8 * Q7_D;
      auto prefetch_residual = [&]() {
        if (p.dbg & 16) return;
        for (int i = lane; i < 16 * (Q7_DH * 4 / 128); i += 32) {
          const int r = i / (Q7_DH * 4 / 128), l = i - r * (Q7_DH * 4 / 128);
          if (row0 + trow + r < p.T)
            q7_prefetch_l2(p.h + (static_cast<long long>(seq) * p.T + row0 + trow + r) * Q7_D + col_half + l * 32);
        }
      };
      if (c >= KT) prefetch_residual();
      tr.ev(24, it);
      float refA = 0.f, refB = 0.f;
      float2 lA2 = make_float2(0.f, 0.f), lB2 = make_float2(0.f, 0.f);
      uint32_t s0[32], s1[32];
      bool have_s = false;
      auto load_scores = [&]() {
        mbar_wait(s_full, sc & 1u);
        tcgen05_fence_after();
        tmem_ld_16x64(t_lane + Q7_S_COL, s0);
        tmem_ld_16x64(t_lane + Q7_S_COL + 64, s1);
        tmem_ld_wait();
        tcgen05_fence_before();
        __syncwarp();
        if (lane == 0) mbar_arrive_leader(s_empty);
        tr.ev(10, sc);
        ++sc;
        have_s = true;
      };
      for (int j = 0; j < KT; ++j, ++pvc) {
        if (pvc >= 4) mbar_wait(&pv_done[pvc & 3u], ((pvc >> 2) - 1) & 1u);
        tr.ev(20, j);
        if ((j & 1) != c) {
          if (j + 1 < KT && !have_s) load_scores();
          const uint32_t slot = rc & 1u;
          if (ew == 0 && lane == 0) mbar_expect_tx(&hdr_bar[slot], Q7_BM * 4);
          if (!(p.dbg & 1)) mbar_wait(&hdr_bar[slot], (rc >> 1) & 1u);
          tr.ev(11, j);
          const float nA = hdr_x[slot * Q7_BM + rA], nB = hdr_x[slot * Q7_BM + rB];
          if (j > 0) {
            const bool upA = nA != refA, upB = nB != refB;
            if (__any_sync(0xffffffffu, upA || upB)) {
              const float fA = upA ? ex2_approx(refA - nA) : 1.0f, fB = upB ? ex2_approx(refB - nB) : 1.0f;
              lA2.x *= fA; lA2.y *= fA; lB2.x *= fB; lB2.y *= fB;
              rescale_o(fA, fB);
            }
          }
          refA = nA; refB = nB;
// ... 126 lines not shown
      lB += l_x[par * Q7_BM + rB];
      const float iA = 1.0f / lA, iB = 1.0f / lB;
      mbar_wait(o_full, it & 1u);
      tcgen05_fence_after();
      tr.ev(16, it);
      float smA = 0.f, sqA = 0.f, smB = 0.f, sqB = 0.f;
      auto sweep1 = [&](int cb, const float4(&f)[8]) {
        uint32_t o[32];
        tmem_ld_16x64(t_lane + cb * 64, o);
        float4 ob[4];
        if (CROSS) {
#pragma unroll
          for (int jj = 0; jj < 4; ++jj) ob[jj] = __ldg(reinterpret_cast<const float4*>(p.obias + col_half + q * 4 + cb * 64 + jj * 16));
        }
        tmem_ld_wait();
        tr.ev(21, cb);
#pragma unroll
        for (int jj = 0; jj < 4; ++jj) {
          const int k0 = 2 * jj, k1 = 2 * jj + 1;
          float4 vA, vB;
          vA.x = fmaf(iA, __uint_as_float(o[4 * k0]), f[jj].x);
          vA.y = fmaf(iA, __uint_as_float(o[4 * k0 + 1]), f[jj].y);
          vA.z = fmaf(iA, __uint_as_float(o[4 * k1]), f[jj].z);
          vA.w = fmaf(iA, __uint_as_float(o[4 * k1 + 1]), f[jj].w);
          vB.x = fmaf(iB, __uint_as_float(o[4 * k0 + 2]), f[4 + jj].x);
          vB.y = fmaf(iB, __uint_as_float(o[4 * k0 + 3]), f[4 + jj].y);
          vB.z = fmaf(iB, __uint_as_float(o[4 * k1 + 2]), f[4 + jj].z);
          vB.w = fmaf(iB, __uint_as_float(o[4 * k1 + 3]), f[4 + jj].w);
          if (CROSS) {
            vA.x += ob[jj].x; vA.y += ob[jj].y; vA.z += ob[jj].z; vA.w += ob[jj].w;
            vB.x += ob[jj].x; vB.y += ob[jj].y; vB.z += ob[jj].z; vB.w += ob[jj].w;
          }
          if (okA && !(p.dbg & 4)) *reinterpret_cast<float4*>(hA + cb * 64 + jj * 16) = vA;
          if (okB && !(p.dbg & 4)) *reinterpret_cast<float4*>(hB + cb * 64 + jj * 16) = vB;
          smA += (vA.x + vA.y) + (vA.z + vA.w);
          sqA = fmaf(vA.x, vA.x, fmaf(vA.y, vA.y, fmaf(vA.z, vA.z, fmaf(vA.w, vA.w, sqA))));
          smB += (vB.x + vB.y) + (vB.z + vB.w);
          sqB = fmaf(vB.x, vB.x, fmaf(vB.y, vB.y, fmaf(vB.z, vB.z, fmaf(vB.w, vB.w, sqB))));
          o[4 * k0] = __float_as_uint(vA.x); o[4 * k0 + 1] = __float_as_uint(vA.y);
          o[4 * k1] = __float_as_uint(vA.z); o[4 * k1 + 1] = __float_as_uint(vA.w);
          o[4 * k0 + 2] = __float_as_uint(vB.x); o[4 * k0 + 3] = __float_as_uint(vB.y);
          o[4 * k1 + 2] = __float_as_uint(vB.z); o[4 * k1 + 3] = __float_as_uint(vB.w);
        }
        if (p.u_out != nullptr) q7_tmem_st_16x64(t_lane + cb * 64, o);
        tr.ev(22, cb);
      };
      static_assert(Q7_DH / 64 == 6, "two rounds of three chunks");
      sweep1(0, f0); load_res(3, f0);
      sweep1(1, f1); load_res(4, f1);
      sweep1(2, f2); load_res(5, f2);
      sweep1(3, f0);
      sweep1(4, f1);
      sweep1(5, f2);
      tr.ev(17, it);
      if (p.u_out != nullptr) {
        q7_tmem_st_wait();
        smA = quad_sum(smA); sqA = quad_sum(sqA); smB = quad_sum(smB); sqB = quad_sum(sqB);
        if (ew == 0 && lane == 0) mbar_expect_tx(&stat_bar[par], Q7_BM * 8);
        if (writer) {
          const uint32_t slot = q7_mapa(smem_u32(stat_x + (par * Q7_BM + rA) * 2), peer);
          const uint32_t bar = q7_mapa(smem_u32(&stat_bar[par]), peer);
          q7_st_async(slot, smA, bar);
          q7_st_async(slot + 4, sqA, bar);
          q7_st_async(slot + 8 * 8, smB, bar);
          q7_st_async(slot + 8 * 8 + 4, sqB, bar);
        }
        mbar_wait(&stat_bar[par], (it >> 1) & 1u);
        tr.ev(18, it);
        const float2 xA = *reinterpret_cast<const float2*>(stat_x + (par * Q7_BM + rA) * 2);
        const float2 xB = *reinterpret_cast<const float2*>(stat_x + (par * Q7_BM + rB) * 2);
        const float inv_h = 1.0f / static_cast<float>(Q7_D);
        const float meanA = (smA + xA.x) * inv_h, meanB = (smB + xB.x) * inv_h;
        const float rsA = rsqrtf(fmaxf(fmaf(-meanA, meanA, (sqA + xA.y) * inv_h), 0.f) + 1e-5f);
        const float rsB = rsqrtf(fmaxf(fmaf(-meanB, meanB, (sqB + xB.y) * inv_h), 0.f) + 1e-5f);
        const float2 aA2 = make_float2(rsA, rsA), cA2 = make_float2(-meanA * rsA, -meanA * rsA);
        const float2 aB2 = make_float2(rsB, rsB), cB2 = make_float2(-meanB * rsB, -meanB * rsB);
        bf16* uA = p.u_out + growA * Q7_D + col_half + q * 4;
        bf16* uB = uA + 8 * Q7_D;
        const float* gp = p.gamma + col_half + q * 4;
        const float* bp = p.beta + col_half + q * 4;
        auto sweep2 = [&](int cb, const uint32_t(&o)[32]) {
          float4 gm[4], bt[4];
#pragma unroll
          for (int jj = 0; jj < 4; ++jj) {
            gm[jj] = __ldg(reinterpret_cast<const float4*>(gp + cb * 64 + jj * 16));
            bt[jj] = __ldg(reinterpret_cast<const float4*>(bp + cb * 64 + jj * 16));
          }
          tr.ev(23, cb);
#pragma unroll
          for (int jj = 0; jj < 4; ++jj) {
            const int k0 = 2 * jj, k1 = 2 * jj + 1;
            const float2 g01 = make_float2(gm[jj].x, gm[jj].y), g23 = make_float2(gm[jj].z, gm[jj].w);
            const float2 b01 = make_float2(bt[jj].x, bt[jj].y), b23 = make_float2(bt[jj].z, bt[jj].w);
            const float2 yA0 = __ffma2_rn(__ffma2_rn(make_float2(__uint_as_float(o[4 * k0]), __uint_as_float(o[4 * k0 + 1])), aA2, cA2), g01, b01);
            const float2 yA1 = __ffma2_rn(__ffma2_rn(make_float2(__uint_as_float(o[4 * k1]), __uint_as_float(o[4 * k1 + 1])), aA2, cA2), g23, b23);
            const float2 yB0 = __ffma2_rn(__ffma2_rn(make_float2(__uint_as_float(o[4 * k0 + 2]), __uint_as_float(o[4 * k0 + 3])), aB2, cB2), g01, b01);
            const float2 yB1 = __ffma2_rn(__ffma2_rn(make_float2(__uint_as_float(o[4 * k1 + 2]), __uint_as_float(o[4 * k1 + 3])), aB2, cB2), g23, b23);
            uint2 wA, wB;
            wA.x = pack_bf16x2(yA0.x, yA0.y);
            wA.y = pack_bf16x2(yA1.x, yA1.y);
            wB.x = pack_bf16x2(yB0.x, yB0.y);
            wB.y = pack_bf16x2(yB1.x, yB1.y);
            if (okA && !(p.dbg & 8)) *reinterpret_cast<uint2*>(uA + cb * 64 + jj * 16) = wA;
            if (okB && !(p.dbg & 8)) *reinterpret_cast<uint2*>(uB + cb * 64 + jj * 16) = wB;
          }
        };
        {
          uint32_t o0[32], o1[32];
          tmem_ld_16x64(t_lane, o0);
          tmem_ld_wait();
#pragma unroll 1
          for (int cb = 0; cb < Q7_DH / 64; cb += 2) {
            tmem_ld_16x64(t_lane + (cb + 1) * 64, o1);
            sweep2(cb, o0);
            tmem_ld_wait();
            if (cb + 2 < Q7_DH / 64) tmem_ld_16x64(t_lane + (cb + 2) * 64, o0);
            sweep2(cb + 1, o1);
            tmem_ld_wait();
          }
        }
      }
      tcgen05_fence_before();
      __syncwarp();
      if (lane == 0) mbar_arrive_leader(o_empty);
      tr.ev(19, it);
    }
  }

  __syncwarp();
  tcgen05_fence_before();
  __syncthreads();
  cluster_sync_all();
  if (warp == 2) {
    tcgen05_fence_after();
    asm volatile("tcgen05.dealloc.cta_group::2.sync.aligned.b32 %0, %1;" ::"r"(tmem_base), "n"(Q7_TMEM_COLS) : "memory");
  }
}

std::mutex g_q7_mutex;

}

bool flash768_quad_preferred(int T) { return round_up(T, 2 * Q7_BM) * 100 <= round_up(T, Q7_BM) * 120; }

static int q7_clusters(DeviceState* ds) {
  std::lock_guard<std::mutex> lock(g_q7_mutex);
  if (ds->f768q_clusters == 0) {
    int n = 0;
    if (cudaFuncSetAttribute(flash_attn768q_kernel<false>, cudaFuncAttributeMaxDynamicSharedMemorySize, Q7_SMEM_BYTES) == cudaSuccess &&
        cudaFuncSetAttribute(flash_attn768q_kernel<true>, cudaFuncAttributeMaxDynamicSharedMemorySize, Q7_SMEM_BYTES) == cudaSuccess) {
      cudaLaunchConfig_t cfg = {};
      cudaLaunchAttribute attr[1];
      attr[0].id = cudaLaunchAttributeClusterDimension;
      attr[0].val.clusterDim.x = 4;
      attr[0].val.clusterDim.y = 1;
      attr[0].val.clusterDim.z = 1;
      cfg.blockDim = dim3(Q7_THREADS, 1, 1);
      cfg.dynamicSmemBytes = Q7_SMEM_BYTES;
      cfg.attrs = attr;
      cfg.numAttrs = 1;
      cfg.gridDim = dim3(static_cast<unsigned>(4 * std::max(ds->num_sms, 4)), 1, 1);
      if (cudaOccupancyMaxActiveClusters(&n, flash_attn768q_kernel<false>, &cfg) != cudaSuccess) n = 0;
    }
    (void)cudaGetLastError();
    ds->f768q_clusters = n > 0 ? n : -1;
  }
  return ds->f768q_clusters;
}

bool flash768_quad_schedulable() {
  if (tc_gemm_init() != 0) return false;
  DeviceState* ds = device_state();
  return ds != nullptr && q7_clusters(ds) > 0;
}

int launch_flash768_quad(const Flash768Params& q, cudaStream_t st) {
  DITTO_TRY(tc_gemm_init());
  DITTO_REQUIRE(flash768_supported(q.H, 1, q.T), DITTO_E_UNSUPPORTED, "flash768: single head of 768 only");
  const bool cross = q.kfold != nullptr;
  DITTO_REQUIRE(q.qkv && q.h && q.n_seq >= 1 && q.ld % 8 == 0 && q.ld >= (cross ? 1 : 3) * Q7_D, DITTO_E_BADARG, "flash768: bad argument");
  DITTO_REQUIRE(!cross || (q.vfold && q.kbias && q.out_bias && q.Tk >= 1 && q.Tk <= 256 && q.vf_rows >= q.Tk && q.kb_seq >= q.Tk &&
                           q.kf_seq % 8 == 0 && q.vf_seq % 8 == 0 && (reinterpret_cast<uintptr_t>(q.out_bias) & 15) == 0),
                DITTO_E_BADARG, "flash768 (cross-attention): folded keys / values, score bias and output bias for 1..256 text tokens");
  DITTO_REQUIRE(q.u_out == nullptr || (q.gamma && q.beta), DITTO_E_BADARG, "flash768: LayerNorm output needs gamma and beta");
  DITTO_REQUIRE((reinterpret_cast<uintptr_t>(q.h) & 15) == 0 && (reinterpret_cast<uintptr_t>(q.u_out) & 7) == 0, DITTO_E_BADARG,
                "flash768: h must be 16-byte, u 8-byte aligned");
  DeviceState* ds = device_state();
  if (ds == nullptr) return DITTO_E_CUDA;
  cudaLaunchConfig_t cfg = {};
  cudaLaunchAttribute attr[1];
  attr[0].id = cudaLaunchAttributeClusterDimension;
  attr[0].val.clusterDim.x = 4;
  attr[0].val.clusterDim.y = 1;
  attr[0].val.clusterDim.z = 1;
  cfg.blockDim = dim3(Q7_THREADS, 1, 1);
  cfg.dynamicSmemBytes = Q7_SMEM_BYTES;
  cfg.stream = st;
  cfg.attrs = attr;
  cfg.numAttrs = 1;
  const int max_clusters = q7_clusters(ds);
  DITTO_REQUIRE(max_clusters > 0, DITTO_E_UNSUPPORTED, "flash768: four-CTA clusters cannot be scheduled on this device");
  TcOperand Q, K, V;
  Q.ptr = q.qkv; Q.rows = q.T; Q.cols = Q7_D; Q.ld = q.ld; Q.s_outer = static_cast<int64_t>(q.T) * q.ld;
  K = Q; K.ptr = q.qkv + Q7_D;
  V = Q; V.ptr = q.qkv + 2 * Q7_D;
  if (cross) {
    K.ptr = q.kfold; K.rows = q.Tk; K.ld = Q7_D; K.s_outer = q.kf_seq;
    V.ptr = q.vfold; V.rows = q.Tk; V.ld = Q7_D; V.s_outer = q.vf_seq;
  }
  CUtensorMap mq, mk, mv;
  DITTO_TRY(tc_make_map(&mq, Q, 1, q.n_seq, Q7_BK, Q7_BM));
  DITTO_TRY(tc_make_map(&mk, K, 1, q.n_seq, Q7_BK, Q7_BN / 2));
  DITTO_TRY(tc_make_map(&mv, V, 1, q.n_seq, 64, Q7_VKEYS));
  Q7Dev p;
  p.n_seq = static_cast<int>(q.n_seq); p.T = q.T;
  p.Tk = cross ? q.Tk : q.T;
  p.kbias = q.kbias; p.kb_seq = q.kb_seq; p.obias = q.out_bias;
  p.m_tiles = static_cast<int>(ceil_div(q.T, 2 * Q7_BM));
  p.k_tiles = static_cast<int>(ceil_div(p.Tk, Q7_BN));
  const int64_t items = static_cast<int64_t>(p.m_tiles) * q.n_seq;
  DITTO_REQUIRE(items < (1ll << 31), DITTO_E_UNSUPPORTED, "flash768: too many work items");
  p.num_items = static_cast<int>(items);
  p.alpha2 = q.alpha * 1.4426950408889634f;
  p.h = q.h; p.gamma = q.gamma; p.beta = q.beta; p.u_out = q.u_out;
  p.force_rescale = q.force_rescale ? 1 : 0;
  p.dbg = q.dbg;
  p.trace = DITTO_F7_TRACE ? tc_gemm_debug_counters() : nullptr;
  const double rows = static_cast<double>(q.n_seq) * q.T;
  ProfScope prof(q.tag, st, 4.0 * q.T * static_cast<double>(p.Tk) * Q7_D * q.n_seq,
                 rows * Q7_D * ((cross ? 2.0 : 6.0) + 8.0 + (q.u_out ? 2.0 : 0.0)) + (cross ? 4.0 * q.n_seq * static_cast<double>(p.Tk) * Q7_D : 0.0));
  const int clusters = static_cast<int>(std::min<int64_t>(max_clusters, items));
  cfg.gridDim = dim3(static_cast<unsigned>(4 * clusters), 1, 1);
  void* args[4] = {&mq, &mk, &mv, &p};
  DITTO_CUDA(cudaLaunchKernelExC(&cfg, cross ? reinterpret_cast<const void*>(flash_attn768q_kernel<true>)
                                             : reinterpret_cast<const void*>(flash_attn768q_kernel<false>), args));
  count_launch();
  return 0;
}

}
```

ditto_tts_b200/csrc/kernels.cuh:

```cuda
#pragma once
#include <algorithm>

#include "common.cuh"

namespace ditto {

struct DebugOptions {
  int no_pair = 0, cluster_m = 0, cluster_n = 0, generic_epi = 0, stages_1cta = 0, stages_pair = 0, no_mcast = 0, dbg_nostore = 0;
  int xf_rows = 0;
  int xf_prefetch = 0;
  int no_defer_ln = 0, no_fused_attn = 0, no_flash = 0, no_flash768 = 0, no_fused_cross = 0, defer_ln2 = 0, pv_transpose = 0,
      rope_table = 0, rope_generic = 0, glu_generic = 0, no_rope_fast32 = 0, no_pv_perm4 = 0, side_streams = -1, no_fused_ln = 0;
  int flash768_quad = 0;
  int no_fc2_ln = 0;
  int no_cross_flash = 0;
};
extern DebugOptions g_opt;

struct DeviceState {
  bool tc_init = false, xf_attr = false, fa_attr = false, f768_attr = false;
  int num_sms = 0;
  int f768q_clusters = 0;
};
DeviceState* device_state();

int launch_cast_bf16(const float* x, bf16* y, int64_t n, cudaStream_t st);
int launch_pack_rows(const float* x, bf16* y, float* bias_out, const float* bias_in, const int* perm, int rows, int K,
                     cudaStream_t st, const float* gamma = nullptr, const float* beta = nullptr, float* csum = nullptr);
int launch_rowsum_bf16(const bf16* x, float* out, int64_t groups, int S, int Sp, int K, cudaStream_t st);
int launch_layernorm(const float* x, const float* gamma, const float* beta, void* y, bool out_bf16, int64_t rows, int H,
                     cudaStream_t st);
int launch_adaln_ln(const float* x, int64_t n_x, const float* time_table, const float* text_mod, const int64_t* t,
                    int steps, const float* gamma, const float* beta, float* h, void* u, bool u_bf16, bf16* xcast,
                    int64_t n_seq, int T, int H, cudaStream_t st, float2* stat = nullptr, bool xcast_all = false,
                    int* row_pos = nullptr);
int launch_rope_table(const float* inv_freq, float* cos_t, float* sin_t, float* freq_out, int max_T, int half, int head_dim,
                      cudaStream_t st);
int launch_rope(void* qkv, bool is_bf16, int64_t ld, const float* cos_t, const float* sin_t, int64_t rows, int seq_T,
                int H, int head_dim, cudaStream_t st);
int launch_softmax(const float* s, int64_t lds, void* p, bool p_bf16, int64_t ldp, int64_t rows, int cols, cudaStream_t st);
int launch_geglu_f32(const float* a, const float* g, float* out, int64_t n, cudaStream_t st);
int launch_silu(float* x, int64_t n, cudaStream_t st);
int launch_mean_silu(const float* text, float* out, int64_t n, int S, int D, cudaStream_t st);
int launch_fold_bias(const bf16* kv, int64_t ld, const float* bq, float* sb, int64_t n, int S, int Sp, int heads, int d, float scale,
                     cudaStream_t st);
int launch_transpose_v(const bf16* v, int64_t ld, bf16* vt, int64_t n_seq, int T, int Tp, int heads, int d, cudaStream_t st);
int launch_cfg_ddpm_update(const float* eps_c, const float* eps_u, const float* x, const float* z, const int64_t* t,
                           const float* coef, int steps, float w, float* out, int64_t B, int64_t elems_per_seq,
                           cudaStream_t st);
int launch_cfg_ddpm_update_rng(const float* eps_c, const float* eps_u, const float* x, unsigned long long* rng, int64_t* t, int64_t n_t,
                               const float* coef, int steps, float w, float* out, int64_t B, int64_t elems_per_seq,
                               int64_t elem_offset, bool advance, cudaStream_t st);
int launch_cfg_multistep_update(const float* eps_c, const float* eps_u, const float* x, const float* z, const int64_t* t,
                                const float* coef, int steps, float w, float* out, float* hist, int64_t B, int64_t elems_per_seq,
                                cudaStream_t st);
int launch_cfg_multistep_update_rng(const float* eps_c, const float* eps_u, const float* x, unsigned long long* rng, int64_t* t,
                                    int64_t n_t, const float* coef, int steps, float w, float* out, float* hist, int64_t B,
                                    int64_t elems_per_seq, int64_t elem_offset, bool advance, cudaStream_t st);
int launch_cfg_update_known(const float* eps_c, const float* eps_u, const float* x, const float* z, unsigned long long* rng, int64_t* t,
                            int64_t n_t, const float* coef, const float* coef_known, int steps, float w, float* out, float* hist,
                            const float* known, const uint8_t* mask, int64_t B, int64_t T, int64_t H, int64_t elem_offset, bool advance,
                            cudaStream_t st);
int launch_step_advance(unsigned long long* rng, int64_t* t, int64_t n_t, cudaStream_t st);
int launch_randn(const unsigned long long* rng, int64_t elem_offset, float* out, int64_t n, cudaStream_t st);
int launch_rope_angles(const float* t, const float* pos, float* out, int64_t batch, int T, int heads, int d, cudaStream_t st);
int launch_schedule_coef(const float* betas, const float* alphas, const float* acp, float* coef, int steps, cudaStream_t st);
int launch_q_sample(const float* x0, const float* noise, const int64_t* t, const float* buf, int steps, float* out, int64_t B,
                    int64_t elems_per_seq, cudaStream_t st);

struct SgemmParams {
  const float* A = nullptr; int64_t lda = 0, sA_inner = 0, sA_outer = 0;
  const float* B = nullptr; int64_t ldb = 0, sB_inner = 0, sB_outer = 0;
  float* C = nullptr;       int64_t ldc = 0, sC_inner = 0, sC_outer = 0;
  const float* resid = nullptr; int64_t ldr = 0, sR_inner = 0, sR_outer = 0;
  const float* bias = nullptr;
  float alpha = 1.f;
  int M = 0, N = 0, K = 0;
  int batch_inner = 1, batch_outer = 1;
  bool b_is_nk = true;
};
int launch_sgemm(const SgemmParams& p, cudaStream_t st);

enum TcEpilogue { TC_EPI_STORE = 0, TC_EPI_GEGLU = 1, TC_EPI_QKV_ROPE = 2 };

struct TcOperand {
  const bf16* ptr = nullptr;
  int64_t rows = 0, cols = 0, ld = 0;
  int64_t s_inner = 0, s_outer = 0;
};

struct TcGemmParams {
  TcOperand A, B;
  bool b_kn = false;
  int M = 0, N = 0, K = 0;
  int batch_inner = 1, batch_outer = 1;
  int epilogue = TC_EPI_STORE;
  int tag = PC_TC_OTHER;
  float alpha = 1.f;
  const float* bias = nullptr;
  int64_t sb_inner = 0, sb_outer = 0;
  void* out = nullptr; bool out_bf16 = false;
  int64_t ldo = 0, so_inner = 0, so_outer = 0;
  const float* resid = nullptr;
  int64_t ldr = 0, sr_inner = 0, sr_outer = 0;
  int64_t resid_row_mod = 0;
  bf16* out2 = nullptr; int64_t ldo2 = 0;
  const float* rope_cos = nullptr; const float* rope_sin = nullptr;
  const float* rope_freq = nullptr;
  int rope_half = 0, rope_pd = 0, seq_T = 0, hidden = 0;
  const int* rope_pos = nullptr;
  bool rope_perm16 = false;
  bool glu_perm16 = false;
  bool out_perm4 = false;
  const float* row_lsum = nullptr; int row_lparts = 0; int64_t sl_inner = 0, sl_outer = 0;
  int cluster_m = 0, cluster_n = 0;
  float2* stat_out = nullptr; int stat_parts = 0; int64_t stat_rows_outer = 0;
  const float2* ln_stat = nullptr; int ln_parts = 0; int ln_width = 0; const float* ln_c = nullptr;
};
int launch_tc_gemm(const TcGemmParams& p, cudaStream_t st);

struct TcScoresSoftmaxParams {
  TcOperand Q, Km;
  int M = 0, N = 0, K = 0;
  int batch_inner = 1, batch_outer = 1;
  float alpha = 1.f;
  const float* bias = nullptr; int64_t sb_inner = 0, sb_outer = 0;
  bf16* P = nullptr; int64_t ldp = 0, sp_inner = 0, sp_outer = 0;
  int npad = 0;
  float* lpart = nullptr; int64_t sl_inner = 0, sl_outer = 0;
  int cluster_m = 0;
  const float2* ln_stat = nullptr; int ln_parts = 0; int ln_width = 0; const float* ln_c = nullptr;
  int tag = PC_TC_OTHER;
};
int tc_scores_softmax_csize(int N);
int launch_tc_scores_softmax(const TcScoresSoftmaxParams& p, cudaStream_t st);
struct CrossFusedParams {
  const bf16* u = nullptr;
  const bf16* kfold = nullptr; int64_t kf_seq = 0;
  const bf16* vfold = nullptr; int64_t vf_seq = 0;
  const float* sbias = nullptr; int64_t sb_seq = 0;
  const float* out_bias = nullptr;
  float* h = nullptr;
  const float* gamma = nullptr; const float* beta = nullptr;
  bf16* u_out = nullptr;
  const float2* ln_stat = nullptr; int ln_parts = 0; const float* ln_c = nullptr;
  int64_t n_seq = 0, T = 0, S = 0, Sp = 0; int H = 0;
  float alpha = 1.f;
  int tag = PC_TC_OTHER;
};
bool cross_fused_supported(int64_t T, int64_t S, int H, int heads);
int launch_cross_fused(const CrossFusedParams& p, cudaStream_t st);

struct FlashAttnParams {
  TcOperand Q, Km, V;
  int64_t n_seq = 0; int heads = 0, d = 0, Tq = 0, Tk = 0;
  float alpha = 1.f;
  float* out = nullptr; const float* resid = nullptr;
  int64_t ldo = 0, o_seq = 0, ldr = 0, r_seq = 0;
  int tag = PC_TC_OTHER;
};
bool flash_attn_supported(int d, int Tq, int Tk);
int launch_flash_attn(const FlashAttnParams& p, cudaStream_t st);

struct Flash768Params {
  const bf16* qkv = nullptr; int64_t ld = 0;
  int64_t n_seq = 0; int T = 0; int H = 0;
  float alpha = 1.f;
  float* h = nullptr;
  const float* gamma = nullptr; const float* beta = nullptr;
  bf16* u_out = nullptr;
  const bf16* kfold = nullptr; int64_t kf_seq = 0;
  const bf16* vfold = nullptr; int64_t vf_seq = 0; int vf_rows = 0;
  int Tk = 0;
  const float* kbias = nullptr; int64_t kb_seq = 0;
  const float* out_bias = nullptr;
  bool force_rescale = false;
  int dbg = 0;
  int tag = PC_TC_OTHER;
};
bool flash768_supported(int H, int heads, int T);
int launch_flash768(const Flash768Params& p, cudaStream_t st);
bool flash768_quad_preferred(int T);
bool flash768_quad_schedulable();
int launch_flash768_quad(const Flash768Params& p, cudaStream_t st);

struct GemmResidLnParams {
  const bf16* A = nullptr; int64_t lda = 0;
  const bf16* W = nullptr; int64_t ldw = 0;
  const float* bias = nullptr;
  float* h = nullptr; int64_t ldh = 0;
  const float* resid = nullptr; int64_t ldr = 0; int64_t resid_mod = 0;
  const float* gamma = nullptr; const float* beta = nullptr;
  bf16* u = nullptr; int64_t ldu = 0;
  int M = 0, N = 0, K = 0;
  int tag = PC_TC_OTHER;
};
bool gemm_resid_ln_supported(int N, int K);
bool gemm_resid_ln_schedulable(int N);
int gemm_resid_ln_weight_row(int packed_row);
int launch_gemm_resid_ln(const GemmResidLnParams& p, cudaStream_t st);

int tc_gemm_init();
int tc_make_map(CUtensorMap* m, const TcOperand& op, int64_t n_inner, int64_t n_outer, int box_cols, int box_rows);
int tc_num_sms();
void tc_gemm_set_debug_counters(unsigned long long* dev_ptr);
unsigned long long* tc_gemm_debug_counters();

}
```

Baseline: 4.485 million.

## Skip cross-attention for sequences whose text embedding rows are identical

A new kernel flags each sequence whose text embedding has identical rows. For those sequences, single-head cross-attention reduces exactly to a constant vector: the folded V row plus the output bias. That constant is precomputed per layer and added in the self-attention flash768 epilogue, which then applies norm3 instead of norm2. The fused cross kernels skip flagged tiles through a new tile iterator, so cross-attention work is removed for uniform-text sequences such as the null-text classifier-free-guidance branch. The cost is extra per-tile skip checks, serial tile walking in some warps, and added register pressure and complexity in the epilogue.

Measured after the change: 4.617 million (median of 6 runs). +2.9%, better.

```diff
diff --git a/ditto_tts_b200/csrc/cross_fused.cu b/ditto_tts_b200/csrc/cross_fused.cu
--- a/ditto_tts_b200/csrc/cross_fused.cu
+++ b/ditto_tts_b200/csrc/cross_fused.cu
@@ -56,7 +56,17 @@
   const float* gamma; const float* beta;
   float inv_h;
   const float2* ln_stat; int ln_parts; const float* ln_c;
+  const int* uni;
 };
+
+__device__ __forceinline__ bool xf_skip(const XfDev& p, int tile) { return p.uni != nullptr && __ldg(p.uni + tile / p.m_tiles) != 0; }
+__device__ __forceinline__ int xf_next(const XfDev& p, int tile, int step) {
+  for (tile += step; tile < p.num_tiles && xf_skip(p, tile); tile += step) {}
+  return tile;
+}
+__device__ __forceinline__ int xf_first(const XfDev& p, int first, int step) {
+  return first < p.num_tiles && xf_skip(p, first) ? xf_next(p, first, step) : first;
+}
 
 __device__ __forceinline__ void epi_bar_sync() { asm volatile("bar.sync 1, %0;" ::"n"(32 * XF_EPI_WARPS) : "memory"); }
 __device__ __forceinline__ void quarter_bar_sync(int quarter) { asm volatile("bar.sync %0, 128;" ::"r"(2 + quarter) : "memory"); }
@@ -150,7 +160,8 @@
   __syncthreads();
   tcgen05_fence_after();
   const uint32_t tmem_base = *tmem_ptr;
-  const int first = blockIdx.x, step = gridDim.x;
+  const int step = gridDim.x;
+  const int first = xf_first(p, blockIdx.x, step);
 
   if (warp == 0) {
     xf_regs_ctrl();
@@ -175,7 +186,7 @@
         }
       };
       if (first < p.num_tiles) load_scores_operands(first);
-      for (int tile = first; tile < p.num_tiles; tile += step) {
+      for (int tile = first; tile < p.num_tiles; tile = xf_next(p, tile, step)) {
         const int seq = tile / p.m_tiles;
         for (int hc = 0; hc < p.num_hc; ++hc, ++vc) {
           const uint32_t vs = vc % XF_VF_RING;
@@ -186,7 +197,8 @@
           }
           __syncwarp();
         }
-        if (tile + step < p.num_tiles) load_scores_operands(tile + step);
+        const int next = xf_next(p, tile, step);
+        if (next < p.num_tiles) load_scores_operands(next);
       }
     }
   } else if (warp == 1) {
@@ -223,7 +235,7 @@
       };
       uint32_t it = 0, oc = 0, vc = 0;
       if (first < p.num_tiles) issue_scores(0);
-      for (int tile = first; tile < p.num_tiles; tile += step, ++it) {
+      for (int tile = first; tile < p.num_tiles; tile = xf_next(p, tile, step), ++it) {
         mbar_wait(p_full, it & 1u);
         for (int hc = 0; hc < p.num_hc; ++hc, ++vc) {
           const uint32_t ob = oc % XF_O_BUFS, vs = vc % XF_VF_RING;
@@ -242,19 +254,25 @@
           __syncwarp();
           if (hc & 1) ++oc;
         }
-        if (tile + step < p.num_tiles) issue_scores(it + 1);
+        if (xf_next(p, tile, step) < p.num_tiles) issue_scores(it + 1);
       }
     }
   } else if (warp == 2 || warp == 3) {
     xf_regs_ctrl();
     {
       const bool leader = elect_one();
-      const int my_tiles = first < p.num_tiles ? (p.num_tiles - 1 - first) / step + 1 : 0;
+      int my_tiles = 0;
+      for (int tile = first; tile < p.num_tiles; tile = xf_next(p, tile, step)) ++my_tiles;
       const int jobs_per_tile = 2 * p.num_hc;
       const int J = my_tiles * jobs_per_tile;
+      int cur_ti = 0, cur_tile = first;
+      auto tile_at = [&](int ti, int& ci, int& ct) {
+        for (; ci < ti; ++ci) ct = xf_next(p, ct, step);
+        return ct;
+      };
       auto job_coords = [&](int j, int& seq, int& row, int& pass, int& hc) {
         const int ti = j / jobs_per_tile, r = j - ti * jobs_per_tile;
-        const int tile = first + ti * step;
+        const int tile = tile_at(ti, cur_ti, cur_tile);
         seq = tile / p.m_tiles;
         row = (tile - seq * p.m_tiles) * p.rt;
         pass = r / p.num_hc;
@@ -263,12 +281,13 @@
       if (warp == 2) {
         const int P0 = my_tiles * p.num_hc;
         int pf_next = 0;
+        int pf_ti = 0, pf_tile = first;
         auto prefetch_upto = [&](int limit) {
           if (p.pf_dist <= 0) return;
           limit = limit < P0 ? limit : P0;
           for (; pf_next < limit; ++pf_next) {
             const int ti = pf_next / p.num_hc, hc = pf_next - ti * p.num_hc;
-            const int tile = first + ti * step, seq = tile / p.m_tiles, row = (tile - seq * p.m_tiles) * p.rt;
+            const int tile = tile_at(ti, pf_ti, pf_tile), seq = tile / p.m_tiles, row = (tile - seq * p.m_tiles) * p.rt;
             if (leader && pf_next >= XF_NB) {
               tma_prefetch_4d(&tmap_h, hc * XF_HC, row, 0, seq);
               tma_prefetch_4d(&tmap_h, hc * XF_HC + 32, row, 0, seq);
@@ -329,7 +348,7 @@
     const int g = lane >> 2, q = lane & 3, q2 = q * 2;
     const bool writer = q == 0;
     uint32_t it = 0, oc = 0, job = 0;
-    for (int tile = first; tile < p.num_tiles; tile += step, ++it) {
+    for (int tile = first; tile < p.num_tiles; tile = xf_next(p, tile, step), ++it) {
       const int seq = tile / p.m_tiles;
       const uint32_t sb = it & 1u;
       if (sub < 2) {
@@ -649,8 +668,9 @@
   p.inv_h = 1.0f / static_cast<float>(q.H);
   p.pf_dist = g_opt.xf_prefetch > 0 ? std::min(g_opt.xf_prefetch, 2 * p.num_hc) : 0;
   p.ln_stat = q.ln_stat; p.ln_parts = q.ln_parts; p.ln_c = q.ln_c;
+  p.uni = q.uni;
   if (q.ln_stat != nullptr) DITTO_REQUIRE(q.ln_parts > 0 && q.ln_c != nullptr, DITTO_E_BADARG, "cross_fused: deferred LayerNorm arguments");
-  const double rows = static_cast<double>(q.n_seq) * q.T;
+  const double rows = static_cast<double>(q.n_seq - profiled_uniform_seqs(q.uni, q.n_seq, st)) * q.T;
   ProfScope prof(q.tag, st, 4.0 * rows * q.S * q.H, rows * q.H * 12.0);
   const int grid = static_cast<int>(std::min<int64_t>(sms, tiles));
   cross_fused_kernel<<<grid, XF_THREADS, XF_SMEM_BYTES, st>>>(mu, mk, mv, mh, mo, p);
diff --git a/ditto_tts_b200/csrc/elementwise.cu b/ditto_tts_b200/csrc/elementwise.cu
--- a/ditto_tts_b200/csrc/elementwise.cu
+++ b/ditto_tts_b200/csrc/elementwise.cu
@@ -532,6 +532,40 @@
                      cudaStream_t st) {
   const int64_t total = n * heads * Sp;
   fold_bias_kernel<<<static_cast<unsigned>(ceil_div(total, 8)), 256, 0, st>>>(kv, ld, bq, sb, total, S, Sp, heads, d, scale);
+  DITTO_LAUNCH_CHECK();
+  return 0;
+}
+
+__global__ void text_uniform_kernel(const float* __restrict__ text, int* __restrict__ uni, int S, int D) {
+  const uint32_t* row0 = reinterpret_cast<const uint32_t*>(text) + static_cast<int64_t>(blockIdx.x) * S * D;
+  int diff = 0;
+  for (int64_t i = D + threadIdx.x; i < static_cast<int64_t>(S) * D && !diff; i += blockDim.x) diff = row0[i] != row0[i % D];
+  diff = __syncthreads_or(diff);
+  if (threadIdx.x == 0) uni[blockIdx.x] = diff ? 0 : 1;
+}
+int launch_text_uniform(const float* text, int* uni, int64_t n, int S, int D, cudaStream_t st) {
+  text_uniform_kernel<<<static_cast<unsigned>(n), 256, 0, st>>>(text, uni, S, D);
+  DITTO_LAUNCH_CHECK();
+  return 0;
+}
+
+__global__ void cross_const_kernel(const bf16* __restrict__ vfold, int64_t vf_seq, const float* __restrict__ bo, float* __restrict__ c,
+                                   int64_t total, int H, bool perm4) {
+  const int64_t o = static_cast<int64_t>(blockIdx.x) * blockDim.x + threadIdx.x;
+  if (o >= total) return;
+  const int64_t seq = o / H;
+  const int r = static_cast<int>(o - seq * H);
+  int j = r;
+  if (perm4) {
+    const int blk = r / 64, cc = r % 64, kb = cc / 8, q = (cc % 8) / 2, e = cc % 2;
+    j = blk * 64 + 16 * (kb / 2) + 4 * q + 2 * (kb % 2) + e;
+  }
+  c[seq * H + j] = __bfloat162float(vfold[seq * vf_seq + r]) + bo[j];
+}
+int launch_cross_const(const bf16* vfold, int64_t vf_seq, const float* bo, float* c, int64_t n, int H, bool perm4, cudaStream_t st) {
+  DITTO_REQUIRE(!perm4 || H % 64 == 0, DITTO_E_UNSUPPORTED, "cross_const: perm4 needs H % 64 == 0");
+  const int64_t total = n * H;
+  cross_const_kernel<<<static_cast<unsigned>(ceil_div(total, 256)), 256, 0, st>>>(vfold, vf_seq, bo, c, total, H, perm4);
   DITTO_LAUNCH_CHECK();
   return 0;
 }
@@ -846,6 +880,18 @@
     }
   }
   if (RNG && advance) last_block_advances(rng, t, n_t, draw);
+}
+
+int64_t profiled_uniform_seqs(const int* uni, int64_t n, cudaStream_t st) {
+  cudaStreamCaptureStatus cs = cudaStreamCaptureStatusNone;
+  if (uni == nullptr || !g_prof_enabled || cudaStreamIsCapturing(st, &cs) != cudaSuccess || cs != cudaStreamCaptureStatusNone) return 0;
+  std::vector<int> h(static_cast<size_t>(n));
+  if (cudaMemcpyAsync(h.data(), uni, sizeof(int) * static_cast<size_t>(n), cudaMemcpyDeviceToHost, st) != cudaSuccess ||
+      cudaStreamSynchronize(st) != cudaSuccess)
+    return 0;
+  int64_t k = 0;
+  for (int v : h) k += v != 0;
+  return k;
 }
 
 static int64_t profiled_known_frames(const uint8_t* mask, int64_t n, cudaStream_t st) {
diff --git a/ditto_tts_b200/csrc/engine.cu b/ditto_tts_b200/csrc/engine.cu
--- a/ditto_tts_b200/csrc/engine.cu
+++ b/ditto_tts_b200/csrc/engine.cu
@@ -89,6 +89,7 @@
   bool fused_attn = false;
   bool fold_cross = false;
   bool defer_ln = false;
+  bool uniform_cross = true;
   int pv_transpose = 0;
   bool rope_table_in_epilogue = false;
   std::map<std::string, int64_t> expected;
@@ -183,6 +184,8 @@
   bf16 *kfold0 = nullptr, *vfold0 = nullptr;
   float *sbias0 = nullptr, *cvec0 = nullptr;
   size_t kfold_stride = 0, vfold_stride = 0, sbias_stride = 0;
+  int* uni = nullptr;
+  float* xconst0 = nullptr;
   size_t total = 0;
 };
 static bool fold_active(const ditto_engine* e, int64_t S) {
@@ -213,6 +216,10 @@
     c.vfold0 = a.take<bf16>(static_cast<int64_t>(c.vfold_stride) * e->L);
     c.sbias0 = a.take<float>(static_cast<int64_t>(c.sbias_stride) * e->L);
     if (e->defer_ln || e->defer_ln2) c.cvec0 = a.take<float>(static_cast<int64_t>(c.sbias_stride) * e->L);
+    if (e->heads == 1) {
+      c.uni = a.take<int>(n);
+      c.xconst0 = a.take<float>(n * e->H * e->L);
+    }
   }
   c.total = a.off + 256;
   return c;
@@ -512,11 +519,18 @@
         float* hg = w.h + grp.row0 * H;
         const bool dln2 = dln ? dln2_all : fold_ln_active(e, S) && do_self;
         float2* lnstat_g = w.lnstat ? w.lnstat + grp.row0 * std::max(w.ln_parts_h, w.ln_parts_attn) : nullptr;
+        const bool self768 = do_self && e->flash768 && !dln2 && flash768_supported(H, e->heads, static_cast<int>(T));
+        const bool uni_on = e->uniform_cross && c.uni != nullptr && do_cross && !dln && self768 &&
+                            (cross_flash_active(e, S) || fuse_cross_group(grp));
         if (!do_self) {
-        } else if (e->flash768 && !dln2 && flash768_supported(H, e->heads, static_cast<int>(T))) {
+        } else if (self768) {
           Flash768Params f;
           f.qkv = q; f.ld = 3 * H; f.n_seq = n; f.T = static_cast<int>(T); f.H = H; f.alpha = inv_sqrt_d; f.h = hg;
           f.gamma = e->LW(i, "norm2.weight"); f.beta = e->LW(i, "norm2.bias"); f.u_out = ug; f.tag = PC_FLASH768;
+          if (uni_on) {
+            f.uni = c.uni; f.cvec = c.xconst0 + n * H * i; f.cv_seq = H;
+            f.gamma3 = e->LW(i, "norm3.weight"); f.beta3 = e->LW(i, "norm3.bias");
+          }
           DITTO_TRY(launch_flash768(f, st));
         } else {
           DITTO_TRY(attention_bf16(e, wg, q, 3 * H, T * 3 * H, q + H, 3 * H, T * 3 * H, q + 2 * H, 3 * H, T * 3 * H, n, static_cast<int>(T),
@@ -537,6 +551,7 @@
             f.vf_rows = static_cast<int>(Sp); f.Tk = static_cast<int>(S); f.kbias = c.sbias0 + c.sbias_stride * i; f.kb_seq = Sp;
             f.out_bias = e->LW(i, "cross_attn.out_proj.bias");
             f.gamma = e->LW(i, "norm3.weight"); f.beta = e->LW(i, "norm3.bias"); f.u_out = ug; f.tag = PC_CROSS_FLASH;
+            if (uni_on) f.uni = c.uni;
             DITTO_TRY(launch_flash768_quad(f, st));
             continue;
           }
@@ -547,6 +562,7 @@
             f.h = hg; f.gamma = e->LW(i, "norm3.weight"); f.beta = e->LW(i, "norm3.bias"); f.u_out = ug;
             f.n_seq = n; f.T = T; f.S = S; f.Sp = Sp; f.H = H; f.alpha = sqrt_inv_d; f.tag = PC_TC_CROSS_FUSED;
             if (dln2) { f.ln_stat = lnstat_g; f.ln_parts = w.ln_parts_attn; f.ln_c = c.cvec0 + c.sbias_stride * i; }
+            if (uni_on) f.uni = c.uni;
             DITTO_TRY(launch_cross_fused(f, st));
             continue;
           }
@@ -799,6 +815,7 @@
     e->flash_attn = e->fused_attn;
     if (g_opt.no_flash) e->flash_attn = false;
     if (g_opt.no_fused_cross) e->fused_cross = false;
+    e->uniform_cross = !g_opt.no_uniform_cross;
     e->defer_ln2 = !e->defer_ln && e->fused_cross && e->bf16_mode && e->heads == 1 && g_opt.defer_ln2 != 0;
     e->pv_transpose = g_opt.pv_transpose != 0;
     e->rope_table_in_epilogue = g_opt.rope_table != 0;
@@ -1127,6 +1144,10 @@
                                    static_cast<int>(S), static_cast<int>(Sp), heads, d, sqrtf(1.0f / static_cast<float>(d)), st));
         if (fln)
           DITTO_TRY(launch_rowsum_bf16(kf, c.cvec0 + c.sbias_stride * i, n * heads, static_cast<int>(S), static_cast<int>(Sp), H, st));
+        if (c.uni) {
+          if (i == 0) DITTO_TRY(launch_text_uniform(text_emb, c.uni, n, static_cast<int>(S), Xd, st));
+          DITTO_TRY(launch_cross_const(vf, Sp * H, e->LW(i, "cross_attn.out_proj.bias"), c.xconst0 + n * H * i, n, H, cross_flash_active(e, S), st));
+        }
       }
     } else {
       DITTO_TRY(sgemm_nt(text_emb, Xd, e->LW(i, "cross_attn.in_proj_weight") + static_cast<int64_t>(H) * H, H, static_cast<float*>(kv),
@@ -1560,7 +1581,7 @@
       {"no_flash768", &g_opt.no_flash768}, {"no_fused_cross", &g_opt.no_fused_cross}, {"defer_ln2", &g_opt.defer_ln2},
       {"pv_transpose", &g_opt.pv_transpose}, {"rope_table", &g_opt.rope_table}, {"rope_generic", &g_opt.rope_generic},
       {"glu_generic", &g_opt.glu_generic}, {"no_rope_fast32", &g_opt.no_rope_fast32}, {"no_pv_perm4", &g_opt.no_pv_perm4},
-      {"side_streams", &g_opt.side_streams}, {"no_fused_ln", &g_opt.no_fused_ln}, {"flash768_quad", &g_opt.flash768_quad},
+      {"side_streams", &g_opt.side_streams}, {"no_fused_ln", &g_opt.no_fused_ln}, {"flash768_quad", &g_opt.flash768_quad}, {"no_uniform_cross", &g_opt.no_uniform_cross},
       {"no_fc2_ln", &g_opt.no_fc2_ln}, {"no_cross_flash", &g_opt.no_cross_flash}, {"dbg_nostore", &g_opt.dbg_nostore}};
   if (strcmp(name, "reset") == 0) { g_opt = DebugOptions(); return 0; }
   for (const Opt& o : opts)
diff --git a/ditto_tts_b200/csrc/flash_attn768.cu b/ditto_tts_b200/csrc/flash_attn768.cu
--- a/ditto_tts_b200/csrc/flash_attn768.cu
+++ b/ditto_tts_b200/csrc/flash_attn768.cu
@@ -64,6 +64,8 @@
   float* h;
   const float* gamma; const float* beta;
   bf16* u_out;
+  const int* uni; const float* cvec; long long cv_seq;
+  const float* gamma3; const float* beta3;
   int force_rescale;
   int dbg;
 };
@@ -556,6 +558,40 @@
         sweep1(cb + 1, f1);
         if (cb + 3 < F7_DH / 64) load_res(cb + 3, f1);
       }
+      const bool uni_item = p.uni != nullptr && __ldg(p.uni + seq) != 0;
+      if (uni_item) {
+        tmem_st_wait();
+        smA = sqA = smB = sqB = 0.f;
+        const float* cvp = p.cvec + seq * p.cv_seq + col_half + q * 4;
+#pragma unroll 1
+        for (int cb = 0; cb < F7_DH / 64; ++cb) {
+          uint32_t o[32];
+          tmem_ld_16x64(t_lane + cb * 64, o);
+          float4 cv[4];
+#pragma unroll
+          for (int jj = 0; jj < 4; ++jj) cv[jj] = __ldg(reinterpret_cast<const float4*>(cvp + cb * 64 + jj * 16));
+          tmem_ld_wait();
+#pragma unroll
+          for (int jj = 0; jj < 4; ++jj) {
+            const int k0 = 2 * jj, k1 = 2 * jj + 1;
+            const float4 vA = make_float4(__uint_as_float(o[4 * k0]) + cv[jj].x, __uint_as_float(o[4 * k0 + 1]) + cv[jj].y,
+                                          __uint_as_float(o[4 * k1]) + cv[jj].z, __uint_as_float(o[4 * k1 + 1]) + cv[jj].w);
+            const float4 vB = make_float4(__uint_as_float(o[4 * k0 + 2]) + cv[jj].x, __uint_as_float(o[4 * k0 + 3]) + cv[jj].y,
+                                          __uint_as_float(o[4 * k1 + 2]) + cv[jj].z, __uint_as_float(o[4 * k1 + 3]) + cv[jj].w);
+            if (okA && !(p.dbg & 4)) *reinterpret_cast<float4*>(hA + cb * 64 + jj * 16) = vA;
+            if (okB && !(p.dbg & 4)) *reinterpret_cast<float4*>(hB + cb * 64 + jj * 16) = vB;
+            smA += (vA.x + vA.y) + (vA.z + vA.w);
+            sqA = fmaf(vA.x, vA.x, fmaf(vA.y, vA.y, fmaf(vA.z, vA.z, fmaf(vA.w, vA.w, sqA))));
+            smB += (vB.x + vB.y) + (vB.z + vB.w);
+            sqB = fmaf(vB.x, vB.x, fmaf(vB.y, vB.y, fmaf(vB.z, vB.z, fmaf(vB.w, vB.w, sqB))));
+            o[4 * k0] = __float_as_uint(vA.x); o[4 * k0 + 1] = __float_as_uint(vA.y);
+            o[4 * k1] = __float_as_uint(vA.z); o[4 * k1 + 1] = __float_as_uint(vA.w);
+            o[4 * k0 + 2] = __float_as_uint(vB.x); o[4 * k0 + 3] = __float_as_uint(vB.y);
+            o[4 * k1 + 2] = __float_as_uint(vB.z); o[4 * k1 + 3] = __float_as_uint(vB.w);
+          }
+          tmem_st_16x64(t_lane + cb * 64, o);
+        }
+      }
       tr.ev(17, it);
       if (p.u_out != nullptr) {
         tmem_st_wait();
@@ -579,35 +615,39 @@
         const float rsB = rsqrtf(fmaxf(fmaf(-meanB, meanB, (sqB + xB.y) * inv_h), 0.f) + 1e-5f);
         bf16* uA = p.u_out + growA * F7_D + col_half + q * 4;
         bf16* uB = uA + 8 * F7_D;
-        const float* gp = p.gamma + col_half + q * 4;
-        const float* bp = p.beta + col_half + q * 4;
+        auto sweep2 = [&](const float* gp, const float* bp) {
+          gp += col_half + q * 4;
+          bp += col_half + q * 4;
 #pragma unroll 1
-        for (int cb = 0; cb < F7_DH / 64; ++cb) {
-          uint32_t o[32];
-          tmem_ld_16x64(t_lane + cb * 64, o);
-          float4 gm[4], bt[4];
-#pragma unroll
-          for (int jj = 0; jj < 4; ++jj) {
-            gm[jj] = __ldg(reinterpret_cast<const float4*>(gp + cb * 64 + jj * 16));
-            bt[jj] = __ldg(reinterpret_cast<const float4*>(bp + cb * 64 + jj * 16));
-          }
-          tmem_ld_wait();
-#pragma unroll
-          for (int jj = 0; jj < 4; ++jj) {
-            const int k0 = 2 * jj, k1 = 2 * jj + 1;
-            uint2 wA, wB;
-            wA.x = pack_bf16x2(fmaf((__uint_as_float(o[4 * k0]) - meanA) * rsA, gm[jj].x, bt[jj].x),
-                               fmaf((__uint_as_float(o[4 * k0 + 1]) - meanA) * rsA, gm[jj].y, bt[jj].y));
-            wA.y = pack_bf16x2(fmaf((__uint_as_float(o[4 * k1]) - meanA) * rsA, gm[jj].z, bt[jj].z),
-                               fmaf((__uint_as_float(o[4 * k1 + 1]) - meanA) * rsA, gm[jj].w, bt[jj].w));
-            wB.x = pack_bf16x2(fmaf((__uint_as_float(o[4 * k0 + 2]) - meanB) * rsB, gm[jj].x, bt[jj].x),
-                               fmaf((__uint_as_float(o[4 * k0 + 3]) - meanB) * rsB, gm[jj].y, bt[jj].y));
-            wB.y = pack_bf16x2(fmaf((__uint_as_float(o[4 * k1 + 2]) - meanB) * rsB, gm[jj].z, bt[jj].z),
-                               fmaf((__uint_as_float(o[4 * k1 + 3]) - meanB) * rsB, gm[jj].w, bt[jj].w));
-            if (okA && !(p.dbg & 8)) *reinterpret_cast<uint2*>(uA + cb * 64 + jj * 16) = wA;
-            if (okB && !(p.dbg & 8)) *reinterpret_cast<uint2*>(uB + cb * 64 + jj * 16) = wB;
-          }
-        }
+          for (int cb = 0; cb < F7_DH / 64; ++cb) {
+            uint32_t o[32];
+            tmem_ld_16x64(t_lane + cb * 64, o);
+            float4 gm[4], bt[4];
+#pragma unroll
+            for (int jj = 0; jj < 4; ++jj) {
+              gm[jj] = __ldg(reinterpret_cast<const float4*>(gp + cb * 64 + jj * 16));
+              bt[jj] = __ldg(reinterpret_cast<const float4*>(bp + cb * 64 + jj * 16));
+            }
+            tmem_ld_wait();
+#pragma unroll
+            for (int jj = 0; jj < 4; ++jj) {
+              const int k0 = 2 * jj, k1 = 2 * jj + 1;
+              uint2 wA, wB;
+              wA.x = pack_bf16x2(fmaf((__uint_as_float(o[4 * k0]) - meanA) * rsA, gm[jj].x, bt[jj].x),
+                                 fmaf((__uint_as_float(o[4 * k0 + 1]) - meanA) * rsA, gm[jj].y, bt[jj].y));
+              wA.y = pack_bf16x2(fmaf((__uint_as_float(o[4 * k1]) - meanA) * rsA, gm[jj].z, bt[jj].z),
+                                 fmaf((__uint_as_float(o[4 * k1 + 1]) - meanA) * rsA, gm[jj].w, bt[jj].w));
+              wB.x = pack_bf16x2(fmaf((__uint_as_float(o[4 * k0 + 2]) - meanB) * rsB, gm[jj].x, bt[jj].x),
+                                 fmaf((__uint_as_float(o[4 * k0 + 3]) - meanB) * rsB, gm[jj].y, bt[jj].y));
+              wB.y = pack_bf16x2(fmaf((__uint_as_float(o[4 * k1 + 2]) - meanB) * rsB, gm[jj].z, bt[jj].z),
+                                 fmaf((__uint_as_float(o[4 * k1 + 3]) - meanB) * rsB, gm[jj].w, bt[jj].w));
+              if (okA && !(p.dbg & 8)) *reinterpret_cast<uint2*>(uA + cb * 64 + jj * 16) = wA;
+              if (okB && !(p.dbg & 8)) *reinterpret_cast<uint2*>(uB + cb * 64 + jj * 16) = wB;
+            }
+          }
+        };
+        if (p.uni != nullptr && __ldg(p.uni + seq) != 0) sweep2(p.gamma3, p.beta3);
+        else sweep2(p.gamma, p.beta);
       }
       tcgen05_fence_before();
       __syncwarp();
@@ -631,6 +671,11 @@
 }
 
 bool flash768_supported(int H, int heads, int T) { return heads == 1 && H == F7_D && T >= 1; }
+
+bool flash768_uniform_args_ok(const Flash768Params& q) {
+  return q.kfold == nullptr && q.cvec && q.gamma3 && q.beta3 && q.u_out && q.cv_seq % 4 == 0 &&
+         (reinterpret_cast<uintptr_t>(q.cvec) & 15) == 0;
+}
 
 int launch_flash768(const Flash768Params& q, cudaStream_t st) {
   if (g_opt.flash768_quad != 1 && q.T >= 1 && (g_opt.flash768_quad == 2 || flash768_quad_preferred(q.T)) && flash768_quad_schedulable())
@@ -641,6 +686,7 @@
   DITTO_REQUIRE(q.u_out == nullptr || (q.gamma && q.beta), DITTO_E_BADARG, "flash768: LayerNorm output needs gamma and beta");
   DITTO_REQUIRE((reinterpret_cast<uintptr_t>(q.h) & 15) == 0 && (reinterpret_cast<uintptr_t>(q.u_out) & 7) == 0, DITTO_E_BADARG,
                 "flash768: h must be 16-byte, u 8-byte aligned");
+  DITTO_REQUIRE(q.uni == nullptr || flash768_uniform_args_ok(q), DITTO_E_BADARG, "flash768: uniform-text arguments");
   DeviceState* ds = device_state();
   if (ds == nullptr) return DITTO_E_CUDA;
   DITTO_REQUIRE(ds->num_sms >= 2, DITTO_E_UNSUPPORTED, "flash768: needs an SM pair");
@@ -665,6 +711,7 @@
   p.num_items = static_cast<int>(items);
   p.alpha2 = q.alpha * 1.4426950408889634f;
   p.h = q.h; p.gamma = q.gamma; p.beta = q.beta; p.u_out = q.u_out;
+  p.uni = q.uni; p.cvec = q.cvec; p.cv_seq = q.cv_seq; p.gamma3 = q.gamma3; p.beta3 = q.beta3;
   p.force_rescale = q.force_rescale ? 1 : 0;
   p.dbg = q.dbg;
   p.trace = DITTO_F7_TRACE ? tc_gemm_debug_counters() : nullptr;
diff --git a/ditto_tts_b200/csrc/flash_attn768q.cu b/ditto_tts_b200/csrc/flash_attn768q.cu
--- a/ditto_tts_b200/csrc/flash_attn768q.cu
+++ b/ditto_tts_b200/csrc/flash_attn768q.cu
@@ -68,9 +68,23 @@
   float* h;
   const float* gamma; const float* beta;
   bf16* u_out;
+  const int* uni; const float* cvec; long long cv_seq;
+  const float* gamma3; const float* beta3;
   int force_rescale;
   int dbg;
 };
+
+template <bool CROSS>
+__device__ __forceinline__ bool q7_skip(const Q7Dev& p, int item) { return CROSS && p.uni != nullptr && __ldg(p.uni + item / p.m_tiles) != 0; }
+template <bool CROSS>
+__device__ __forceinline__ int q7_next(const Q7Dev& p, int item, int stride) {
+  for (item += stride; item < p.num_items && q7_skip<CROSS>(p, item); item += stride) {}
+  return item;
+}
+template <bool CROSS>
+__device__ __forceinline__ int q7_first(const Q7Dev& p, int item, int stride) {
+  return item < p.num_items && q7_skip<CROSS>(p, item) ? q7_next<CROSS>(p, item, stride) : item;
+}
 
 __device__ __forceinline__ void q7_tmem_st_16x64(uint32_t taddr, const uint32_t (&r)[32]) {
   asm volatile(
@@ -139,7 +153,7 @@
   const int c = static_cast<int>(rank >> 1);
   const uint32_t peer = rank ^ 2u;
   const int num_clusters = gridDim.x >> 2;
-  const int first = blockIdx.x >> 2;
+  const int first = q7_first<CROSS>(p, static_cast<int>(blockIdx.x >> 2), num_clusters);
   const int KT = p.k_tiles;
 
   if (warp == 0 && lane == 0) {
@@ -186,7 +200,7 @@
     Q7Tr tr; tr.init(p.trace, rank, 2, first == 0 && leader, t_sync);
     int stage = 0;
     uint32_t phase = 0;
-    for (int item = first; item < p.num_items; item += num_clusters) {
+    for (int item = first; item < p.num_items; item = q7_next<CROSS>(p, item, num_clusters)) {
       const int qt = item % p.m_tiles, seq = item / p.m_tiles;
       const int q_row0 = qt * (2 * Q7_BM) + a * Q7_BM;
       auto load_s = [&](int j) {
@@ -313,7 +327,7 @@
         if (own) ++oc; else ++rc;
         ++pvi;
       };
-      for (int item = first; item < p.num_items; item += num_clusters, ++it) {
+      for (int item = first; item < p.num_items; item = q7_next<CROSS>(p, item, num_clusters), ++it) {
         if (c < KT) issue_s();
         for (int j = 0; j < KT; ++j) {
           if ((j & 1) == c && j + 2 < KT) issue_s();
@@ -329,7 +343,7 @@
     const bool leader = elect_one();
     const uint32_t dst = q7_mapa(smem_u32(p_land), peer), src = smem_u32(p_own), bar = q7_mapa(smem_u32(land_full), peer);
     uint32_t oc = 0;
-    for (int item = first; item < p.num_items; item += num_clusters)
+    for (int item = first; item < p.num_items; item = q7_next<CROSS>(p, item, num_clusters))
       for (int j = c; j < KT; j += 2, ++oc) {
         mbar_wait(p_ready, oc & 1u);
         if (leader) q7_bulk_copy_to_peer(dst, src, Q7_P_BYTES, bar);
@@ -338,7 +352,7 @@
   } else if (warp == 3) {
     regs_shrink_ctrl();
     uint32_t rc = 0;
-    for (int item = first; item < p.num_items; item += num_clusters)
+    for (int item = first; item < p.num_items; item = q7_next<CROSS>(p, item, num_clusters))
       for (int j = c ^ 1; j < KT; j += 2, ++rc) {
         if (lane == 0) {
           mbar_expect_tx(land_full, Q7_P_BYTES);
@@ -380,7 +394,7 @@
       q7_tmem_st_wait();
       tcgen05_fence_before();
     };
-    for (int item = first; item < p.num_items; item += num_clusters, ++it) {
+    for (int item = first; item < p.num_items; item = q7_next<CROSS>(p, item, num_clusters), ++it) {
       const int qt = item % p.m_tiles, seq = item / p.m_tiles;
       const int row0 = qt * (2 * Q7_BM) + a * Q7_BM;
       const int lrowA = row0 + rA;
@@ -613,6 +627,40 @@
       sweep1(3, f0);
       sweep1(4, f1);
       sweep1(5, f2);
+      const bool uni_item = !CROSS && p.uni != nullptr && __ldg(p.uni + seq) != 0;
+      if (uni_item) {
+        q7_tmem_st_wait();
+        smA = sqA = smB = sqB = 0.f;
+        const float* cvp = p.cvec + seq * p.cv_seq + col_half + q * 4;
+#pragma unroll 1
+        for (int cb = 0; cb < Q7_DH / 64; ++cb) {
+          uint32_t o[32];
+          tmem_ld_16x64(t_lane + cb * 64, o);
+          float4 cv[4];
+#pragma unroll
+          for (int jj = 0; jj < 4; ++jj) cv[jj] = __ldg(reinterpret_cast<const float4*>(cvp + cb * 64 + jj * 16));
+          tmem_ld_wait();
+#pragma unroll
+          for (int jj = 0; jj < 4; ++jj) {
+            const int k0 = 2 * jj, k1 = 2 * jj + 1;
+            const float4 vA = make_float4(__uint_as_float(o[4 * k0]) + cv[jj].x, __uint_as_float(o[4 * k0 + 1]) + cv[jj].y,
+                                          __uint_as_float(o[4 * k1]) + cv[jj].z, __uint_as_float(o[4 * k1 + 1]) + cv[jj].w);
+            const float4 vB = make_float4(__uint_as_float(o[4 * k0 + 2]) + cv[jj].x, __uint_as_float(o[4 * k0 + 3]) + cv[jj].y,
+                                          __uint_as_float(o[4 * k1 + 2]) + cv[jj].z, __uint_as_float(o[4 * k1 + 3]) + cv[jj].w);
+            if (okA && !(p.dbg & 4)) *reinterpret_cast<float4*>(hA + cb * 64 + jj * 16) = vA;
+            if (okB && !(p.dbg & 4)) *reinterpret_cast<float4*>(hB + cb * 64 + jj * 16) = vB;
+            smA += (vA.x + vA.y) + (vA.z + vA.w);
+            sqA = fmaf(vA.x, vA.x, fmaf(vA.y, vA.y, fmaf(vA.z, vA.z, fmaf(vA.w, vA.w, sqA))));
+            smB += (vB.x + vB.y) + (vB.z + vB.w);
+            sqB = fmaf(vB.x, vB.x, fmaf(vB.y, vB.y, fmaf(vB.z, vB.z, fmaf(vB.w, vB.w, sqB))));
+            o[4 * k0] = __float_as_uint(vA.x); o[4 * k0 + 1] = __float_as_uint(vA.y);
+            o[4 * k1] = __float_as_uint(vA.z); o[4 * k1 + 1] = __float_as_uint(vA.w);
+            o[4 * k0 + 2] = __float_as_uint(vB.x); o[4 * k0 + 3] = __float_as_uint(vB.y);
+            o[4 * k1 + 2] = __float_as_uint(vB.z); o[4 * k1 + 3] = __float_as_uint(vB.w);
+          }
+          q7_tmem_st_16x64(t_lane + cb * 64, o);
+        }
+      }
       tr.ev(17, it);
       if (p.u_out != nullptr) {
         q7_tmem_st_wait();
@@ -638,8 +686,8 @@
         const float2 aB2 = make_float2(rsB, rsB), cB2 = make_float2(-meanB * rsB, -meanB * rsB);
         bf16* uA = p.u_out + growA * Q7_D + col_half + q * 4;
         bf16* uB = uA + 8 * Q7_D;
-        const float* gp = p.gamma + col_half + q * 4;
-        const float* bp = p.beta + col_half + q * 4;
+        const float* gp = (uni_item ? p.gamma3 : p.gamma) + col_half + q * 4;
+        const float* bp = (uni_item ? p.beta3 : p.beta) + col_half + q * 4;
         auto sweep2 = [&](int cb, const uint32_t(&o)[32]) {
           float4 gm[4], bt[4];
 #pragma unroll
@@ -746,6 +794,7 @@
   DITTO_REQUIRE(q.u_out == nullptr || (q.gamma && q.beta), DITTO_E_BADARG, "flash768: LayerNorm output needs gamma and beta");
   DITTO_REQUIRE((reinterpret_cast<uintptr_t>(q.h) & 15) == 0 && (reinterpret_cast<uintptr_t>(q.u_out) & 7) == 0, DITTO_E_BADARG,
                 "flash768: h must be 16-byte, u 8-byte aligned");
+  DITTO_REQUIRE(q.uni == nullptr || cross || flash768_uniform_args_ok(q), DITTO_E_BADARG, "flash768: uniform-text arguments");
   DeviceState* ds = device_state();
   if (ds == nullptr) return DITTO_E_CUDA;
   cudaLaunchConfig_t cfg = {};
@@ -784,12 +833,14 @@
   p.num_items = static_cast<int>(items);
   p.alpha2 = q.alpha * 1.4426950408889634f;
   p.h = q.h; p.gamma = q.gamma; p.beta = q.beta; p.u_out = q.u_out;
+  p.uni = q.uni; p.cvec = q.cvec; p.cv_seq = q.cv_seq; p.gamma3 = q.gamma3; p.beta3 = q.beta3;
   p.force_rescale = q.force_rescale ? 1 : 0;
   p.dbg = q.dbg;
   p.trace = DITTO_F7_TRACE ? tc_gemm_debug_counters() : nullptr;
-  const double rows = static_cast<double>(q.n_seq) * q.T;
-  ProfScope prof(q.tag, st, 4.0 * q.T * static_cast<double>(p.Tk) * Q7_D * q.n_seq,
-                 rows * Q7_D * ((cross ? 2.0 : 6.0) + 8.0 + (q.u_out ? 2.0 : 0.0)) + (cross ? 4.0 * q.n_seq * static_cast<double>(p.Tk) * Q7_D : 0.0));
+  const double seqs = static_cast<double>(q.n_seq - (cross ? profiled_uniform_seqs(q.uni, q.n_seq, st) : 0));
+  const double rows = seqs * q.T;
+  ProfScope prof(q.tag, st, 4.0 * q.T * static_cast<double>(p.Tk) * Q7_D * seqs,
+                 rows * Q7_D * ((cross ? 2.0 : 6.0) + 8.0 + (q.u_out ? 2.0 : 0.0)) + (cross ? 4.0 * seqs * static_cast<double>(p.Tk) * Q7_D : 0.0));
   const int clusters = static_cast<int>(std::min<int64_t>(max_clusters, items));
   cfg.gridDim = dim3(static_cast<unsigned>(4 * clusters), 1, 1);
   void* args[4] = {&mq, &mk, &mv, &p};
diff --git a/ditto_tts_b200/csrc/kernels.cuh b/ditto_tts_b200/csrc/kernels.cuh
--- a/ditto_tts_b200/csrc/kernels.cuh
+++ b/ditto_tts_b200/csrc/kernels.cuh
@@ -14,6 +14,7 @@
   int flash768_quad = 0;
   int no_fc2_ln = 0;
   int no_cross_flash = 0;
+  int no_uniform_cross = 0;
 };
 extern DebugOptions g_opt;
 
@@ -44,6 +45,9 @@
 int launch_mean_silu(const float* text, float* out, int64_t n, int S, int D, cudaStream_t st);
 int launch_fold_bias(const bf16* kv, int64_t ld, const float* bq, float* sb, int64_t n, int S, int Sp, int heads, int d, float scale,
                      cudaStream_t st);
+int launch_text_uniform(const float* text, int* uni, int64_t n, int S, int D, cudaStream_t st);
+int64_t profiled_uniform_seqs(const int* uni, int64_t n, cudaStream_t st);
+int launch_cross_const(const bf16* vfold, int64_t vf_seq, const float* bo, float* c, int64_t n, int H, bool perm4, cudaStream_t st);
 int launch_transpose_v(const bf16* v, int64_t ld, bf16* vt, int64_t n_seq, int T, int Tp, int heads, int d, cudaStream_t st);
 int launch_cfg_ddpm_update(const float* eps_c, const float* eps_u, const float* x, const float* z, const int64_t* t,
                            const float* coef, int steps, float w, float* out, int64_t B, int64_t elems_per_seq,
@@ -144,6 +148,7 @@
   const float* gamma = nullptr; const float* beta = nullptr;
   bf16* u_out = nullptr;
   const float2* ln_stat = nullptr; int ln_parts = 0; const float* ln_c = nullptr;
+  const int* uni = nullptr;
   int64_t n_seq = 0, T = 0, S = 0, Sp = 0; int H = 0;
   float alpha = 1.f;
   int tag = PC_TC_OTHER;
@@ -174,11 +179,15 @@
   int Tk = 0;
   const float* kbias = nullptr; int64_t kb_seq = 0;
   const float* out_bias = nullptr;
+  const int* uni = nullptr;
+  const float* cvec = nullptr; int64_t cv_seq = 0;
+  const float* gamma3 = nullptr; const float* beta3 = nullptr;
   bool force_rescale = false;
   int dbg = 0;
   int tag = PC_TC_OTHER;
 };
 bool flash768_supported(int H, int heads, int T);
+bool flash768_uniform_args_ok(const Flash768Params& q);
 int launch_flash768(const Flash768Params& p, cudaStream_t st);
 bool flash768_quad_preferred(int T);
 bool flash768_quad_schedulable();
```
